# srinidhiPY/SSL_CR_Histo

Hardware: AMD Instinct MI355X
Metric: images/sec (ResNet18 SSL_CR step, 256x256 bf16 synthetic patches; whole job) (higher is better)
Workload: dtype bf16

## Files before the change

### include/sslcr.h

```cpp
#ifndef SSLCR_H_
#define SSLCR_H_
#include <stddef.h>
#include <stdint.h>

#ifdef __cplusplus
extern "C" {
#endif
#if defined(__GNUC__) || defined(__clang__)
#pragma GCC visibility push(default)
#endif

#define SSLCR_F32 0
#define SSLCR_BF16 1
#define SSLCR_FP8 2

int sslcr_version(void);
const char* sslcr_last_error(void);

typedef struct sslcr_conv_desc {
  const void* x;
  const void* w;
  void* y;
  const float* in_scale;
  const float* in_shift;
  const float* bias;
  const void* residual;
  float* stats;
  int N, H, W, C, K, R, S, stride, pad;
  int PH, PW;
  int OH, OW, osh;
  int transposed;
  int in_relu, relu, accumulate;
  int pix_mul, pix_off_h, pix_off_w;
  unsigned tap_mask;
  const void* mask_x; const float* mask_scale; const float* mask_shift; const float* mask_mean;
  int par4;
  int seg_images, seg_stride;
  const float* out_scale;
} sslcr_conv_desc;
int sslcr_conv2d(int dtype, const sslcr_conv_desc* d, void* stream);
int sslcr_conv2d_partial_rows(const sslcr_conv_desc* d);
int sslcr_conv2d_segments_ok(int dtype, const sslcr_conv_desc* d);
const char* sslcr_conv2d_kernel_name(int dtype, const sslcr_conv_desc* d);
int sslcr_conv2d_s2_pair(int dtype, const sslcr_conv_desc* c1, const sslcr_conv_desc* ds, void* stream);
int sslcr_conv2d_s2_pair_ok(int dtype, const sslcr_conv_desc* c1, const sslcr_conv_desc* ds);

typedef struct sslcr_fp8_desc {
  const uint8_t* w8;
  const float* w_dequant;
  float x_scale;
  const float* x_scale_dev;
  float* amax_out;
} sslcr_fp8_desc;
int sslcr_conv2d_fp8(const sslcr_conv_desc* d, const sslcr_fp8_desc* q, void* stream);
int sslcr_conv2d_fp8_partial_rows(const sslcr_conv_desc* d);
typedef struct sslcr_pack_fp8_desc {
  const float* w;
  uint8_t* w8;
  float* w_dequant;
  const float* gamma; const float* beta; const float* rmean; const float* rvar; float eps; float* bias_out;
  int K, C;
} sslcr_pack_fp8_desc;
int sslcr_pack_conv_fp8(const sslcr_pack_fp8_desc* d, void* stream);

typedef struct sslcr_wgrad_desc {
  const void* x;
  const void* dy;
  float* dw;
  const float* in_scale;
  const float* in_shift;
  int in_relu;
  int N, H, W, C, K, R, S, stride, pad, OH, OW;
  int seg_images;
  int seg_stride;
} sslcr_wgrad_desc;
int sslcr_conv2d_wgrad(int dtype, const sslcr_wgrad_desc* d, void* stream);
const char* sslcr_conv2d_wgrad_kernel_name(int dtype, const sslcr_wgrad_desc* d);

int sslcr_probe_tr16(const uint16_t* in, const int* byte_addr, uint16_t* out, void* stream);

typedef struct sslcr_stem_desc {
  const void* x;
  const void* w;
  void* y;
  const float* bias;
  float* stats;
  int N, H, W, OH, OW, in_f32, relu;
  const void* x2;
  int n_split;
  const float* out_scale;
} sslcr_stem_desc;
int sslcr_stem_conv(int dtype, const sslcr_stem_desc* d, void* stream);
int sslcr_stem_partial_rows(const sslcr_stem_desc* d);
int sslcr_stem_conv_pool(int dtype, const sslcr_stem_desc* d, int POH, int POW, void* stream);
typedef struct sslcr_stem_wgrad_desc {
  const void* x; const void* dy;
  float* dw;
  int N, H, W, OH, OW, in_f32;
  const void* x2; int n_split;
} sslcr_stem_wgrad_desc;
int sslcr_stem_wgrad(int dtype, const sslcr_stem_wgrad_desc* d, void* stream);

typedef struct sslcr_bn_finalize_desc {
  const float* partials;
  int rows, C;
  double count;
  const float* gamma; const float* beta;
  float* scale; float* shift; float* mean; float* invstd;
  float* running_mean; float* running_var; int64_t* num_batches_tracked;
  float momentum, eps; int replay;
  double* sums_out;
  const double* sums_in;
  double* stage;
  int nseg, seg_stride;
  int* tickets;
} sslcr_bn_finalize_desc;
int sslcr_bn_finalize(const sslcr_bn_finalize_desc* d, void* stream);

typedef struct sslcr_bn_act_desc {
  const void* x; const float* scale; const float* shift;
  const void* res; const float* rscale; const float* rshift;
  void* y; size_t pixels; int C; int relu;
  int nseg, seg_stride;
  uint8_t* ybits;
} sslcr_bn_act_desc;
int sslcr_bn_act(int dtype, const sslcr_bn_act_desc* d, void* stream);

typedef struct sslcr_pool_fwd_desc {
  const void* x; const float* scale; const float* shift; void* y; uint8_t* argmax; int N, H, W, C, OH, OW;
} sslcr_pool_fwd_desc;
int sslcr_bn_relu_maxpool(int dtype, const sslcr_pool_fwd_desc* d, void* stream);
typedef struct sslcr_pool_bwd_desc {
  const void* dy; const uint8_t* argmax; const void* x; const float* scale; const float* shift; void* dx; int N, H, W, C, OH, OW;
} sslcr_pool_bwd_desc;
int sslcr_maxpool_relu_bwd(int dtype, const sslcr_pool_bwd_desc* d, void* stream);

int sslcr_avgpool_fwd(int dtype, const void* x, float* y, int N, int HW, int C, void* stream);
int sslcr_avgpool_bwd(int dtype, const float* dy, void* dx, int N, int HW, int C, void* stream);

typedef struct sslcr_bn_bwd_desc {
  const void* dy; const void* x; const void* yact;
  const float* scale; const float* shift; const float* mean; const float* invstd;
  double* sums;
  void* dx; void* gout;
  size_t pixels; int C; int relu_from_x; double count;
  const void* pool_dy;
  const uint8_t* pool_argmax;
  int pH, pW, pOH, pOW;
  const void* pool_y;
  int g_in_reduce;
  float* dgamma; float* dbeta;
  float pg_scale;
  int nseg, seg_stride, sums_stride;
  const uint8_t* yact_bits;
} sslcr_bn_bwd_desc;
int sslcr_bn_bwd_reduce(int dtype, const sslcr_bn_bwd_desc* d, void* stream);
int sslcr_bn_bwd_apply(int dtype, const sslcr_bn_bwd_desc* d, void* stream);
int sslcr_bn_param_grads(const double* sums, const float* invstd, float* dgamma, float* dbeta, int C, void* stream);
int sslcr_stem_wgrad_pool(int dtype, const sslcr_stem_wgrad_desc* w, const sslcr_bn_bwd_desc* bn, void* stream);

int sslcr_linear_fwd(const float* x, const float* w, const float* b, float* y, int M, int N, int K, int relu, void* stream);
int sslcr_linear_bwd(const float* x, const float* w, const float* dy, const float* yact, float* dx, float* dw, float* db,
                     int M, int N, int K, int dx_accumulate, float* scratch, void* stream);
typedef struct sslcr_loss_desc {
  int kind;
  const float* logits; const float* logits_t;
  const float* target_f; const int64_t* target_i;
  float* dlogits;
  float* out;
  int nx, nu, C; float lambda_u;
  float inv_nx_global, inv_nu_global;
} sslcr_loss_desc;
int sslcr_loss(const sslcr_loss_desc* d, void* stream);
int sslcr_softmax_col(const float* logits, float* out, int n, int C, int col, void* stream);

typedef struct sslcr_tensor_desc {
  float* p; float* g; float* s1; float* s2;
  int n;
  int K, C, RS;
  void* w_fwd;
  void* w_dgrad;
  int pack_dtype;
  int dgrad_flip;
} sslcr_tensor_desc;
typedef struct sslcr_opt_desc {
  int kind;
  float lr, beta1, beta2, eps, wd, momentum;
  float bc1, bc2;
  int first_step;
  float grad_scale;
} sslcr_opt_desc;
int sslcr_optimizer_step(const sslcr_tensor_desc* device_descs, int ntensors, int max_n, const sslcr_opt_desc* o, void* stream);
int sslcr_axpby(float* p, float* q, size_t n, float alpha, int copy_back, void* stream);
int sslcr_fill(float* p, size_t n, float v, void* stream);

typedef struct sslcr_pack_desc {
  const float* w; void* w_fwd; void* w_dgrad;
  const float* gamma; const float* beta; const float* rmean; const float* rvar; float eps; float* bias_out;
  int K, C, R, S;
  int dgrad_flip;
  float* scale_out;
} sslcr_pack_desc;
int sslcr_pack_conv(int dtype, const sslcr_pack_desc* d, void* stream);
int sslcr_pack_stem(int dtype, const sslcr_pack_desc* d, void* stream);

typedef struct sslcr_weak_aug_desc {
  const uint8_t* src;
  uint8_t* dst;
  const int32_t* params;
  int N, SH, SW, OH, OW, src_hwc;
} sslcr_weak_aug_desc;
int sslcr_weak_augment(const sslcr_weak_aug_desc* d, void* stream);

typedef struct sslcr_colour_aug_desc {
  const uint8_t* src;
  uint8_t* dst;
  const double* shift;
  const uint8_t* apply;
  double hed_from_rgb[9];
  double rgb_from_hed[9];
  int N, H, W, hwc;
// ... 96 lines not shown
```

### ssl_cr_histo_amd/_lib.py

```python
import ctypes as C
import os

import torch

HERE = os.path.dirname(os.path.abspath(__file__))
LIB_PATH = os.path.join(HERE, "libsslcr.so")

vp, i32, f32, f64, sz = C.c_void_p, C.c_int, C.c_float, C.c_double, C.c_size_t


class SslcrError(RuntimeError):
    pass


def _S(name, fields):
    return type(name, (C.Structure,), {"_fields_": fields})


ConvDesc = _S("ConvDesc", [("x", vp), ("w", vp), ("y", vp), ("in_scale", vp), ("in_shift", vp), ("bias", vp),
                           ("residual", vp), ("stats", vp)] +
              [(k, i32) for k in ("N", "H", "W", "C", "K", "R", "S", "stride", "pad", "PH", "PW", "OH", "OW", "osh",
                                  "transposed", "in_relu", "relu", "accumulate", "pix_mul", "pix_off_h", "pix_off_w")] +
              [("tap_mask", C.c_uint), ("mask_x", vp), ("mask_scale", vp), ("mask_shift", vp), ("mask_mean", vp),
               ("par4", i32), ("seg_images", i32), ("seg_stride", i32), ("out_scale", vp)])
WgradDesc = _S("WgradDesc", [("x", vp), ("dy", vp), ("dw", vp), ("in_scale", vp), ("in_shift", vp), ("in_relu", i32)] +
               [(k, i32) for k in ("N", "H", "W", "C", "K", "R", "S", "stride", "pad", "OH", "OW", "seg_images", "seg_stride")])
StemDesc = _S("StemDesc", [("x", vp), ("w", vp), ("y", vp), ("bias", vp), ("stats", vp)] +
              [(k, i32) for k in ("N", "H", "W", "OH", "OW", "in_f32", "relu")] + [("x2", vp), ("n_split", i32), ("out_scale", vp)])
StemWgradDesc = _S("StemWgradDesc", [("x", vp), ("dy", vp), ("dw", vp)] +
                   [(k, i32) for k in ("N", "H", "W", "OH", "OW", "in_f32")] + [("x2", vp), ("n_split", i32)])
BnFinalizeDesc = _S("BnFinalizeDesc", [("partials", vp), ("rows", i32), ("C", i32), ("count", f64), ("gamma", vp),
                                       ("beta", vp), ("scale", vp), ("shift", vp), ("mean", vp), ("invstd", vp),
                                       ("running_mean", vp), ("running_var", vp), ("num_batches_tracked", vp),
                                       ("momentum", f32), ("eps", f32), ("replay", i32), ("sums_out", vp),
                                       ("sums_in", vp), ("stage", vp), ("nseg", i32), ("seg_stride", i32), ("tickets", vp)])
BnActDesc = _S("BnActDesc", [("x", vp), ("scale", vp), ("shift", vp), ("res", vp), ("rscale", vp), ("rshift", vp),
                             ("y", vp), ("pixels", sz), ("C", i32), ("relu", i32), ("nseg", i32), ("seg_stride", i32), ("ybits", vp)])
PoolFwdDesc = _S("PoolFwdDesc", [("x", vp), ("scale", vp), ("shift", vp), ("y", vp), ("argmax", vp)] +
                 [(k, i32) for k in ("N", "H", "W", "C", "OH", "OW")])
PoolBwdDesc = _S("PoolBwdDesc", [("dy", vp), ("argmax", vp), ("x", vp), ("scale", vp), ("shift", vp), ("dx", vp)] +
                 [(k, i32) for k in ("N", "H", "W", "C", "OH", "OW")])
BnBwdDesc = _S("BnBwdDesc", [("dy", vp), ("x", vp), ("yact", vp), ("scale", vp), ("shift", vp), ("mean", vp),
                             ("invstd", vp), ("sums", vp), ("dx", vp), ("gout", vp), ("pixels", sz), ("C", i32),
                             ("relu_from_x", i32), ("count", f64), ("pool_dy", vp), ("pool_argmax", vp), ("pH", i32),
                             ("pW", i32), ("pOH", i32), ("pOW", i32), ("pool_y", vp), ("g_in_reduce", i32), ("dgamma", vp), ("dbeta", vp),
                             ("pg_scale", f32), ("nseg", i32), ("seg_stride", i32), ("sums_stride", i32), ("yact_bits", vp)])
LossDesc = _S("LossDesc", [("kind", i32), ("logits", vp), ("logits_t", vp), ("target_f", vp), ("target_i", vp),
                           ("dlogits", vp), ("out", vp), ("nx", i32), ("nu", i32), ("C", i32), ("lambda_u", f32),
                           ("inv_nx_global", f32), ("inv_nu_global", f32)])
TensorDesc = _S("TensorDesc", [("p", vp), ("g", vp), ("s1", vp), ("s2", vp), ("n", i32), ("K", i32), ("C", i32),
                               ("RS", i32), ("w_fwd", vp), ("w_dgrad", vp), ("pack_dtype", i32), ("dgrad_flip", i32)])
OptDesc = _S("OptDesc", [("kind", i32), ("lr", f32), ("beta1", f32), ("beta2", f32), ("eps", f32), ("wd", f32),
                         ("momentum", f32), ("bc1", f32), ("bc2", f32), ("first_step", i32), ("grad_scale", f32)])
WeakAugDesc = _S("WeakAugDesc", [("src", vp), ("dst", vp), ("params", vp)] +
                 [(k, i32) for k in ("N", "SH", "SW", "OH", "OW", "src_hwc")])
ColourAugDesc = _S("ColourAugDesc", [("src", vp), ("dst", vp), ("shift", vp), ("apply", vp), ("hed_from_rgb", f64 * 9),
                                     ("rgb_from_hed", f64 * 9), ("N", i32), ("H", i32), ("W", i32), ("hwc", i32)])
BrightnessContrastDesc = _S("BrightnessContrastDesc", [("src", vp), ("dst", vp), ("alpha_beta", vp), ("apply", vp), ("stats", vp),
                                                       ("N", i32), ("H", i32), ("W", i32)])
PackDesc = _S("PackDesc", [("w", vp), ("w_fwd", vp), ("w_dgrad", vp), ("gamma", vp), ("beta", vp), ("rmean", vp),
                           ("rvar", vp), ("eps", f32), ("bias_out", vp)] + [(k, i32) for k in ("K", "C", "R", "S", "dgrad_flip")] + [("scale_out", vp)])

Fp8Desc = _S("Fp8Desc", [("w8", vp), ("w_dequant", vp), ("x_scale", f32), ("x_scale_dev", vp), ("amax_out", vp)])
PackFp8Desc = _S("PackFp8Desc", [("w", vp), ("w8", vp), ("w_dequant", vp), ("gamma", vp), ("beta", vp), ("rmean", vp), ("rvar", vp),
                                 ("eps", f32), ("bias_out", vp), ("K", i32), ("C", i32)])

P = C.POINTER
SIGNATURES = {
    "sslcr_version": (i32, []),
    "sslcr_last_error": (C.c_char_p, []),
    "sslcr_conv2d": (i32, [i32, P(ConvDesc), vp]),
    "sslcr_conv2d_partial_rows": (i32, [P(ConvDesc)]),
    "sslcr_conv2d_segments_ok": (i32, [i32, P(ConvDesc)]),
    "sslcr_conv2d_kernel_name": (C.c_char_p, [i32, P(ConvDesc)]),
    "sslcr_conv2d_s2_pair": (i32, [i32, P(ConvDesc), P(ConvDesc), vp]),
    "sslcr_conv2d_s2_pair_ok": (i32, [i32, P(ConvDesc), P(ConvDesc)]),
    "sslcr_conv2d_fp8": (i32, [P(ConvDesc), P(Fp8Desc), vp]),
    "sslcr_conv2d_fp8_partial_rows": (i32, [P(ConvDesc)]),
    "sslcr_pack_conv_fp8": (i32, [P(PackFp8Desc), vp]),
    "sslcr_conv2d_wgrad": (i32, [i32, P(WgradDesc), vp]),
    "sslcr_conv2d_wgrad_kernel_name": (C.c_char_p, [i32, P(WgradDesc)]),
    "sslcr_probe_tr16": (i32, [vp, vp, vp, vp]),
    "sslcr_stem_conv": (i32, [i32, P(StemDesc), vp]),
    "sslcr_stem_partial_rows": (i32, [P(StemDesc)]),
    "sslcr_stem_conv_pool": (i32, [i32, P(StemDesc), i32, i32, vp]),
    "sslcr_stem_wgrad": (i32, [i32, P(StemWgradDesc), vp]),
    "sslcr_stem_wgrad_pool": (i32, [i32, P(StemWgradDesc), P(BnBwdDesc), vp]),
    "sslcr_bn_finalize": (i32, [P(BnFinalizeDesc), vp]),
    "sslcr_bn_act": (i32, [i32, P(BnActDesc), vp]),
    "sslcr_bn_relu_maxpool": (i32, [i32, P(PoolFwdDesc), vp]),
    "sslcr_maxpool_relu_bwd": (i32, [i32, P(PoolBwdDesc), vp]),
    "sslcr_avgpool_fwd": (i32, [i32, vp, vp, i32, i32, i32, vp]),
    "sslcr_avgpool_bwd": (i32, [i32, vp, vp, i32, i32, i32, vp]),
    "sslcr_bn_bwd_reduce": (i32, [i32, P(BnBwdDesc), vp]),
    "sslcr_bn_bwd_apply": (i32, [i32, P(BnBwdDesc), vp]),
    "sslcr_bn_param_grads": (i32, [vp, vp, vp, vp, i32, vp]),
    "sslcr_linear_fwd": (i32, [vp, vp, vp, vp, i32, i32, i32, i32, vp]),
    "sslcr_linear_bwd": (i32, [vp, vp, vp, vp, vp, vp, vp, i32, i32, i32, i32, vp, vp]),
    "sslcr_loss": (i32, [P(LossDesc), vp]),
    "sslcr_softmax_col": (i32, [vp, vp, i32, i32, i32, vp]),
    "sslcr_optimizer_step": (i32, [vp, i32, i32, P(OptDesc), vp]),
    "sslcr_axpby": (i32, [vp, vp, sz, f32, i32, vp]),
    "sslcr_fill": (i32, [vp, sz, f32, vp]),
    "sslcr_pack_conv": (i32, [i32, P(PackDesc), vp]),
    "sslcr_pack_stem": (i32, [i32, P(PackDesc), vp]),
    "sslcr_weak_augment": (i32, [P(WeakAugDesc), vp]),
    "sslcr_hed_colour_augment": (i32, [P(ColourAugDesc), vp]),
    "sslcr_brightness_contrast": (i32, [P(BrightnessContrastDesc), vp]),
}

_lib = None


def lib():
    global _lib
    if _lib is None:
        if not os.path.exists(LIB_PATH):
            raise SslcrError(f"{LIB_PATH} not built: run `python -m ssl_cr_histo_amd.build` "
                             "(or __graft_entry__.build()); there is no CPU/PyTorch fallback")
        L = C.CDLL(LIB_PATH, mode=C.RTLD_GLOBAL)
        for name, (res, args) in SIGNATURES.items():
            fn = getattr(L, name)
            fn.restype = res
            fn.argtypes = args
        _lib = L
    return _lib


def check(rc):
    if rc != 0:
        raise SslcrError(lib().sslcr_last_error().decode())


def stream_ptr():
    return C.c_void_p(torch.cuda.current_stream().cuda_stream)


def ptr(t):
    return None if t is None else C.c_void_p(t.data_ptr())
```

### ssl_cr_histo_amd/csrc/bn_eltwise.hip

```cpp
#include <stdlib.h>

#include "kernels.hpp"

namespace sslcr {

__global__ __launch_bounds__(256) void bn_reduce_rows_kernel(const float* __restrict__ part, int rows, int C, double* __restrict__ out, int splits) {
  __shared__ double sm[2][8][32];
  const int c = blockIdx.x * 32 + (threadIdx.x & 31);
  const int rl = threadIdx.x >> 5;
  const int per = (rows + splits - 1) / splits;
  const int r0 = blockIdx.y * per, r1 = min(rows, r0 + per);
  part += (size_t)blockIdx.z * rows * 2 * C;
  out += (size_t)blockIdx.z * splits * 2 * C;
  double s = 0.0, ss = 0.0;
  if (c < C) {
    int r = r0 + rl;
    for (; r + 8 < r1; r += 16) {
      const float* p = part + (size_t)r * 2 * C;
      const float* q = p + (size_t)16 * C;
      const float a0 = p[c], a1 = p[C + c], b0 = q[c], b1 = q[C + c];
      s += (double)a0 + (double)b0;
      ss += (double)a1 + (double)b1;
    }
    for (; r < r1; r += 8) {
// ... 436 lines not shown
    float acc[EPC];
#pragma unroll
    for (int e = 0; e < EPC; ++e) acc[e] = 0.f;
    const int oh0 = h >> 1, ow0 = w >> 1;
#pragma unroll
    for (int dh = 0; dh < 2; ++dh) {
      const int oh = oh0 + dh;
      const int wi_h = h - (2 * oh - 1);
      if (oh >= a.OH || wi_h < 0 || wi_h > 2 || (dh == 1 && ((h & 1) == 0))) continue;
#pragma unroll
      for (int dw = 0; dw < 2; ++dw) {
        const int ow = ow0 + dw;
        const int wi_w = w - (2 * ow - 1);
        if (ow >= a.OW || wi_w < 0 || wi_w > 2 || (dw == 1 && ((w & 1) == 0))) continue;
        const int code = wi_h * 3 + wi_w;
        const size_t o = (((size_t)n * a.OH + oh) * a.OW + ow) * cols + col;
        float g[EPC];
        Elem<T>::unpack(ld16(dy + o * 16), g);
        uint32_t am[2];
        if (EPC == 8) { const u32x2_t v = *reinterpret_cast<const u32x2_t*>(a.argmax + o * EPC); am[0] = v[0]; am[1] = v[1]; }
        else { am[0] = *reinterpret_cast<const uint32_t*>(a.argmax + o * EPC); am[1] = 0; }
#pragma unroll
        for (int e = 0; e < EPC; ++e)
          if (((am[e >> 2] >> (8 * (e & 3))) & 0xffu) == (uint32_t)code) acc[e] += g[e];
      }
    }
    float f[EPC];
    Elem<T>::unpack(ld16_nt(x + i * 16), f);
#pragma unroll
    for (int e = 0; e < EPC; ++e)
      if (!(fmaf(f[e], a.scale[cb + e], a.shift[cb + e]) > 0.f)) acc[e] = 0.f;
    st16_nt(dx + i * 16, Elem<T>::pack(acc));
  }
}

hipError_t launch_maxpool_relu_bwd(int dtype, const PoolBwdArgs& a, hipStream_t st) {
  size_t px = (size_t)a.N * a.H * a.W;
  if (dtype == DT_BF16) {
    hipLaunchKernelGGL(maxpool_relu_bwd_kernel<bf16_t>, dim3(ew_grid(px * (a.C / 8))), dim3(256), 0, st, a);
  } else {
    hipLaunchKernelGGL(maxpool_relu_bwd_kernel<float>, dim3(ew_grid(px * (a.C / 4))), dim3(256), 0, st, a);
  }
  return hipGetLastError();
}

template <typename T>
__global__ __launch_bounds__(256) void avgpool_fwd_kernel(const void* xv, float* y, int N, int HW, int C) {
  constexpr int EPC = Elem<T>::EPC;
  __shared__ float sm[3][64][EPC + 1];
  const int cols = C / EPC;
  const int cl = threadIdx.x & 63, q = threadIdx.x >> 6;
  const int i = blockIdx.x * 64 + cl;
  const bool ok = i < N * cols;
  const int n = ok ? i / cols : 0, col = ok ? i - n * cols : 0;
  const char* x = reinterpret_cast<const char*>(xv) + ((size_t)n * HW * C) * sizeof(T) + (size_t)col * 16;
  float acc[EPC];
#pragma unroll
  for (int e = 0; e < EPC; ++e) acc[e] = 0.f;
  if (ok) {
#pragma unroll 4
    for (int p = q; p < HW; p += 4) {
      float f[EPC];
      Elem<T>::unpack(ld16(x + (size_t)p * C * sizeof(T)), f);
#pragma unroll
      for (int e = 0; e < EPC; ++e) acc[e] += f[e];
    }
  }
  if (q > 0) {
#pragma unroll
    for (int e = 0; e < EPC; ++e) sm[q - 1][cl][e] = acc[e];
  }
  __syncthreads();
  if (q > 0 || !ok) return;
#pragma unroll
  for (int w = 0; w < 3; ++w)
#pragma unroll
    for (int e = 0; e < EPC; ++e) acc[e] += sm[w][cl][e];
  const float inv = 1.f / (float)HW;
#pragma unroll
  for (int e = 0; e < EPC; ++e) y[(size_t)n * C + col * EPC + e] = acc[e] * inv;
}

template <typename T>
__global__ __launch_bounds__(256) void avgpool_bwd_kernel(const float* dy, void* dxv, int N, int HW, int C) {
  constexpr int EPC = Elem<T>::EPC;
  const int cols = C / EPC;
  const size_t total = (size_t)N * HW * cols;
  char* dx = reinterpret_cast<char*>(dxv);
  const float inv = 1.f / (float)HW;
  for (size_t i = (size_t)blockIdx.x * 256 + threadIdx.x; i < total; i += (size_t)gridDim.x * 256) {
    const int col = (int)(i % cols);
    const int n = (int)(i / ((size_t)HW * cols));
    float f[EPC];
#pragma unroll
    for (int e = 0; e < EPC; ++e) f[e] = dy[(size_t)n * C + col * EPC + e] * inv;
    st16_nt(dx + i * 16, Elem<T>::pack(f));
  }
}

hipError_t launch_avgpool_fwd(int dtype, const void* x, float* y, int N, int HW, int C, hipStream_t st) {
  if (dtype == DT_BF16) {
    hipLaunchKernelGGL(avgpool_fwd_kernel<bf16_t>, dim3(cdiv(N * (C / 8), 64)), dim3(256), 0, st, x, y, N, HW, C);
  } else {
    hipLaunchKernelGGL(avgpool_fwd_kernel<float>, dim3(cdiv(N * (C / 4), 64)), dim3(256), 0, st, x, y, N, HW, C);
  }
  return hipGetLastError();
}
hipError_t launch_avgpool_bwd(int dtype, const float* dy, void* dx, int N, int HW, int C, hipStream_t st) {
  if (dtype == DT_BF16) {
    hipLaunchKernelGGL(avgpool_bwd_kernel<bf16_t>, dim3(ew_grid((size_t)N * HW * (C / 8))), dim3(256), 0, st, dy, dx, N, HW, C);
  } else {
    hipLaunchKernelGGL(avgpool_bwd_kernel<float>, dim3(ew_grid((size_t)N * HW * (C / 4))), dim3(256), 0, st, dy, dx, N, HW, C);
  }
  return hipGetLastError();
}

template <typename T>
__device__ __forceinline__ void bn_bwd_g(const BnBwdArgs& a, size_t i, const float* rsc, const float* rsh, float* g, float* xf) {
  constexpr int EPC = Elem<T>::EPC;
  Elem<T>::unpack(ld16_nt(reinterpret_cast<const char*>(a.x) + i * 16), xf);
  if (a.pool_dy) {
    const int cols = a.C / EPC, col = (int)(i % cols);
    size_t pix = i / cols;
    const int w = (int)(pix % a.pW);
    pix /= a.pW;
    const int h = (int)(pix % a.pH), n = (int)(pix / a.pH);
#pragma unroll
    for (int e = 0; e < EPC; ++e) g[e] = 0.f;
    u32x4_t dv[4];
    uint32_t am[4][2];
    bool ok[4];
    int code[4];
#pragma unroll
    for (int k = 0; k < 4; ++k) {
      const int dh = k >> 1, dw = k & 1;
      const int oh = (h >> 1) + dh, ow = (w >> 1) + dw;
      ok[k] = (dh == 0 || (h & 1)) && (dw == 0 || (w & 1)) && oh < a.pOH && ow < a.pOW;
      code[k] = (h - (2 * oh - 1)) * 3 + (w - (2 * ow - 1));
      const int ohc = oh < a.pOH ? oh : a.pOH - 1, owc = ow < a.pOW ? ow : a.pOW - 1;
      const size_t o = (((size_t)n * a.pOH + ohc) * a.pOW + owc) * cols + col;
      dv[k] = ld16(reinterpret_cast<const char*>(a.pool_dy) + o * 16);
      if (EPC == 8) { const u32x2_t v = *reinterpret_cast<const u32x2_t*>(a.pool_argmax + o * EPC); am[k][0] = v[0]; am[k][1] = v[1]; }
      else { am[k][0] = *reinterpret_cast<const uint32_t*>(a.pool_argmax + o * EPC); am[k][1] = 0; }
    }
#pragma unroll
    for (int k = 0; k < 4; ++k) {
      float d[EPC];
      Elem<T>::unpack(dv[k], d);
#pragma unroll
      for (int e = 0; e < EPC; ++e)
        if (ok[k] && ((am[k][e >> 2] >> (8 * (e & 3))) & 0xffu) == (uint32_t)code[k]) g[e] += d[e];
    }
  } else {
    Elem<T>::unpack(ld16_nt(reinterpret_cast<const char*>(a.dy) + i * 16), g);
  }
  if (EPC == 8 && a.yact_bits) {
    const unsigned b = a.yact_bits[i];
#pragma unroll
    for (int e = 0; e < EPC; ++e)
      if (!((b >> e) & 1u)) g[e] = 0.f;
  } else if (a.yact) {
    float ya[EPC];
    Elem<T>::unpack(ld16_nt(reinterpret_cast<const char*>(a.yact) + i * 16), ya);
#pragma unroll
    for (int e = 0; e < EPC; ++e)
      if (!(ya[e] > 0.f)) g[e] = 0.f;
  } else if (a.relu_from_x) {
#pragma unroll
    for (int e = 0; e < EPC; ++e)
      if (!(fmaf(xf[e], rsc[e], rsh[e]) > 0.f)) g[e] = 0.f;
  }
}

__device__ __forceinline__ void bn_bwd_param_grads(const BnBwdArgs& a) {
  if (blockIdx.x != 0 || blockIdx.y != 0 || !a.dgamma || !a.dbeta) return;
  const int nseg = a.nseg > 1 ? a.nseg : 1;
  for (int c = threadIdx.x; c < a.C; c += 256) {
    float dg = a.dgamma[c], db = a.dbeta[c];
    for (int z = 0; z < nseg; ++z) {
      const double* sums = a.sums + (size_t)z * a.sums_stride;
      dg += (float)(sums[a.C + c] * (double)a.invstd[(size_t)z * a.seg_stride + c] * (double)a.pg_scale);
      db += (float)(sums[c] * (double)a.pg_scale);
    }
    a.dgamma[c] = dg;
    a.dbeta[c] = db;
  }
}
template <typename T>
__device__ __forceinline__ BnBwdArgs bn_bwd_segment(const BnBwdArgs& a) {
  BnBwdArgs b = a;
  if (a.nseg > 1) {
    const int z = blockIdx.y;
    b.pixels = a.pixels / a.nseg;
    const size_t off = (size_t)z * b.pixels * a.C * sizeof(T);
    if (a.dy) b.dy = reinterpret_cast<const char*>(a.dy) + off;
// ... 463 lines not shown
```

### ssl_cr_histo_amd/csrc/capi.cpp

```cpp
#include <stdarg.h>
#include <stdio.h>
#include <string.h>

#include "kernels.hpp"

namespace sslcr {
thread_local char g_err[512] = "";
int fail(const char* fmt, ...) {
  va_list ap;
  va_start(ap, fmt);
  vsnprintf(g_err, sizeof(g_err), fmt, ap);
  va_end(ap);
  return -1;
}
int check(hipError_t e, const char* what) {
  if (e == hipSuccess) return 0;
  return fail("%s: %s", what, hipGetErrorString(e));
}
}

using namespace sslcr;

#define NEED(cond, what) \
  do {                   \
    if (!(cond)) return fail("%s: invalid argument (%s)", __func__, what); \
  } while (0)
#define DT_OK(dt) NEED((dt) == SSLCR_F32 || (dt) == SSLCR_BF16, "dtype")

extern "C" {

int sslcr_version(void) { return 6; }
const char* sslcr_last_error(void) { return g_err; }

int sslcr_conv2d(int dtype, const sslcr_conv_desc* d, void* stream) {
  DT_OK(dtype);
  NEED(d && d->x && d->w && d->y, "null tensor");
  NEED(d->N > 0 && d->C > 0 && d->K > 0 && d->R > 0 && d->S > 0 && d->stride > 0, "shape");
  NEED(d->C % (dtype == SSLCR_BF16 ? 64 : 32) == 0, "C must be a multiple of the 128-byte channel slab");
  NEED(d->K % 64 == 0, "K % 64");
  NEED(d->osh >= 1 && d->PH > 0 && d->PW > 0, "pixel space");
  NEED(conv_segments_ok(dtype, *d), "seg_images: no segment form for this shape / dtype (sslcr_conv2d_segments_ok)");
  return check(launch_conv(dtype, *d, (hipStream_t)stream), "conv2d");
}
int sslcr_conv2d_partial_rows(const sslcr_conv_desc* d) { return d ? conv_partials_rows(*d) : -1; }
int sslcr_conv2d_segments_ok(int dtype, const sslcr_conv_desc* d) { return (d && (dtype == DT_F32 || dtype == DT_BF16) && conv_segments_ok(dtype, *d)) ? 1 : 0; }
const char* sslcr_conv2d_kernel_name(int dtype, const sslcr_conv_desc* d) { return d ? conv_kernel_name(dtype, *d) : ""; }
int sslcr_conv2d_s2_pair_ok(int dtype, const sslcr_conv_desc* c1, const sslcr_conv_desc* ds) {
  return (c1 && ds && conv_s2_pair_ok(dtype, *c1, *ds)) ? 1 : 0;
}
int sslcr_conv2d_s2_pair(int dtype, const sslcr_conv_desc* c1, const sslcr_conv_desc* ds, void* stream) {
  DT_OK(dtype);
  NEED(c1 && ds && c1->x && c1->w && c1->y && ds->w && ds->y, "null tensor");
  NEED(conv_s2_pair_ok(dtype, *c1, *ds), "pair not served (sslcr_conv2d_s2_pair_ok)");
  return check(launch_conv_s2(*c1, ds, (hipStream_t)stream), "conv2d_s2_pair");
}

int sslcr_conv2d_fp8(const sslcr_conv_desc* d, const sslcr_fp8_desc* q, void* stream) {
  NEED(d && q && d->x && d->y && q->w8 && q->w_dequant, "null tensor");
  NEED(q->x_scale > 0.f, "x_scale must be positive");
  NEED(conv_fp8_mode(*d) != 0, "shape not served by the fp8 kernel (3x3/1, C % 128, K % 128, 16x16-tileable or 8x8 with N % 4)");
  return check(launch_conv_fp8(*d, *q, (hipStream_t)stream), "conv2d_fp8");
}
int sslcr_conv2d_fp8_partial_rows(const sslcr_conv_desc* d) { return (d && conv_fp8_mode(*d)) ? conv_fp8_rows(*d) : 0; }
int sslcr_pack_conv_fp8(const sslcr_pack_fp8_desc* d, void* stream) {
  NEED(d && d->w && d->w8 && d->w_dequant && d->K > 0 && d->C > 0, "args");
  NEED(!d->gamma || (d->beta && d->rmean && d->rvar), "BatchNorm fold needs gamma, beta, running mean and var");
  return check(launch_pack_fp8(*d, (hipStream_t)stream), "pack_conv_fp8");
}

const char* sslcr_conv2d_wgrad_kernel_name(int dtype, const sslcr_wgrad_desc* d) { return d ? wgrad_kernel_name(dtype, *d) : ""; }
int sslcr_conv2d_wgrad(int dtype, const sslcr_wgrad_desc* d, void* stream) {
  DT_OK(dtype);
  NEED(d && d->x && d->dy && d->dw, "null tensor");
  NEED(d->C % 64 == 0 && d->K % 64 == 0, "C,K % 64");
  NEED((d->R == 3 && d->S == 3) || (d->R == 1 && d->S == 1), "3x3 or 1x1");
  return check(launch_wgrad(dtype, *d, (hipStream_t)stream), "conv2d_wgrad");
}

int sslcr_probe_tr16(const uint16_t* in, const int* byte_addr, uint16_t* out, void* stream) {
  NEED(in && byte_addr && out, "null");
  return check(launch_probe_tr16(in, byte_addr, out, (hipStream_t)stream), "probe_tr16");
}

int sslcr_stem_conv(int dtype, const sslcr_stem_desc* d, void* stream) {
  DT_OK(dtype);
  NEED(d && d->x && d->w && d->y, "null tensor");
  NEED(d->OH == (d->H + 6 - 7) / 2 + 1 && d->OW == (d->W + 6 - 7) / 2 + 1, "7x7/2 pad 3 output dims");
  NEED(!d->x2 || (d->n_split >= 0 && d->n_split <= d->N), "n_split outside the batch");
  return check(launch_stem(dtype, *d, (hipStream_t)stream), "stem_conv");
}
int sslcr_stem_conv_pool(int dtype, const sslcr_stem_desc* d, int POH, int POW, void* stream) {
  DT_OK(dtype);
  NEED(d && d->x && d->w && d->y, "null");
  NEED(stem_pool_ok(dtype, *d, POH, POW), "shape / mode not served by the fused stem + max-pool kernel");
  return check(launch_stem_pool(dtype, *d, POH, POW, (hipStream_t)stream), "stem_conv_pool");
}
int sslcr_stem_partial_rows(const sslcr_stem_desc* d) { return d ? stem_partials_rows(*d) : -1; }
int sslcr_stem_wgrad(int dtype, const sslcr_stem_wgrad_desc* d, void* stream) {
  DT_OK(dtype);
  NEED(d && d->x && d->dy && d->dw, "null tensor");
  NEED(!d->x2 || (d->n_split >= 0 && d->n_split <= d->N), "n_split outside the batch");
  return check(launch_stem_wgrad(dtype, *d, (hipStream_t)stream), "stem_wgrad");
}
int sslcr_stem_wgrad_pool(int dtype, const sslcr_stem_wgrad_desc* w, const sslcr_bn_bwd_desc* bn, void* stream) {
  DT_OK(dtype);
  NEED(w && w->x && w->dw && bn && bn->pool_dy && bn->pool_argmax && bn->x && bn->sums && bn->mean && bn->invstd && bn->scale && bn->shift, "null tensor");
  NEED(!w->x2 || (w->n_split >= 0 && w->n_split <= w->N), "n_split outside the batch");
  NEED(bn->C == 64 && bn->pH == w->OH && bn->pW == w->OW && bn->pixels == (size_t)w->N * w->OH * w->OW, "bn descriptor is not this stem's");
  NEED(!bn->g_in_reduce && !bn->gout, "pool form has no g output");
  return check(launch_stem_wgrad_pool(dtype, *w, *bn, (hipStream_t)stream), "stem_wgrad_pool");
}

int sslcr_bn_finalize(const sslcr_bn_finalize_desc* d, void* stream) {
  NEED(d && d->C > 0, "desc");
  NEED(d->sums_in || (d->partials && d->stage && d->rows > 0), "partials/stage");
  NEED(d->sums_out || (d->gamma && d->beta && d->scale && d->shift && d->count > 0), "finalize outputs");
  return check(launch_bn_finalize(*d, (hipStream_t)stream), "bn_finalize");
}
int sslcr_bn_act(int dtype, const sslcr_bn_act_desc* d, void* stream) {
  DT_OK(dtype);
  NEED(d && d->x && d->y && d->scale && d->shift, "null");
  NEED(d->C % 8 == 0, "C % 8");
  return check(launch_bn_act(dtype, *d, (hipStream_t)stream), "bn_act");
}
int sslcr_bn_relu_maxpool(int dtype, const sslcr_pool_fwd_desc* d, void* stream) {
  DT_OK(dtype);
  NEED(d && d->x && d->y, "null");
  if (!d->scale || !d->shift) {
    const int cols = d->C / (dtype == SSLCR_BF16 ? 8 : 4);
    NEED(!d->scale && !d->shift && !d->argmax, "plain max-pool (scale = shift = NULL) records no argmax");
    NEED(cols >= 1 && cols <= 256 && 256 % cols == 0 && d->C % (dtype == SSLCR_BF16 ? 8 : 4) == 0, "plain max-pool: unsupported channel count");
  }
  return check(launch_bn_relu_maxpool(dtype, *d, (hipStream_t)stream), "bn_relu_maxpool");
}
int sslcr_maxpool_relu_bwd(int dtype, const sslcr_pool_bwd_desc* d, void* stream) {
  DT_OK(dtype);
  NEED(d && d->x && d->dy && d->dx && d->argmax, "null");
  return check(launch_maxpool_relu_bwd(dtype, *d, (hipStream_t)stream), "maxpool_relu_bwd");
}
int sslcr_avgpool_fwd(int dtype, const void* x, float* y, int N, int HW, int C, void* stream) {
  DT_OK(dtype);
  NEED(x && y && N > 0 && HW > 0 && C % 8 == 0, "args");
  return check(launch_avgpool_fwd(dtype, x, y, N, HW, C, (hipStream_t)stream), "avgpool_fwd");
}
int sslcr_avgpool_bwd(int dtype, const float* dy, void* dx, int N, int HW, int C, void* stream) {
  DT_OK(dtype);
  NEED(dy && dx && N > 0 && HW > 0 && C % 8 == 0, "args");
  return check(launch_avgpool_bwd(dtype, dy, dx, N, HW, C, (hipStream_t)stream), "avgpool_bwd");
}
int sslcr_bn_bwd_reduce(int dtype, const sslcr_bn_bwd_desc* d, void* stream) {
  DT_OK(dtype);
  NEED(d && (d->dy || (d->pool_dy && d->pool_argmax)) && d->x && d->sums && d->mean, "null");
  NEED(!d->g_in_reduce || (d->yact && d->gout && d->dy && !d->pool_dy), "g_in_reduce needs dy, yact and gout");
  return check(launch_bn_bwd_reduce(dtype, *d, (hipStream_t)stream), "bn_bwd_reduce");
}
int sslcr_bn_bwd_apply(int dtype, const sslcr_bn_bwd_desc* d, void* stream) {
  DT_OK(dtype);
  NEED(d && (d->dy || (d->pool_dy && d->pool_argmax)) && d->x && d->sums && d->dx && d->mean && d->invstd && d->scale, "null");
  NEED(!d->g_in_reduce || (d->yact && d->gout && d->dy && !d->pool_dy), "g_in_reduce needs dy, yact and gout");
  return check(launch_bn_bwd_apply(dtype, *d, (hipStream_t)stream), "bn_bwd_apply");
}
int sslcr_bn_param_grads(const double* sums, const float* invstd, float* dgamma, float* dbeta, int C, void* stream) {
  NEED(sums && invstd && dgamma && dbeta, "null");
  return check(launch_bn_param_grads(sums, invstd, dgamma, dbeta, C, (hipStream_t)stream), "bn_param_grads");
}

int sslcr_linear_fwd(const float* x, const float* w, const float* b, float* y, int M, int N, int K, int relu, void* stream) {
  NEED(x && w && y && M > 0 && N > 0 && K > 0, "args");
  return check(launch_linear_fwd(x, w, b, y, M, N, K, relu, (hipStream_t)stream), "linear_fwd");
}
int sslcr_linear_bwd(const float* x, const float* w, const float* dy, const float* yact, float* dx, float* dw, float* db,
                     int M, int N, int K, int dx_accumulate, float* scratch, void* stream) {
  NEED(x && w && dy && scratch && M > 0 && N > 0 && K > 0, "args");
  return check(launch_linear_bwd(x, w, dy, yact, dx, dw, db, M, N, K, dx_accumulate, scratch, (hipStream_t)stream), "linear_bwd");
}
int sslcr_loss(const sslcr_loss_desc* d, void* stream) {
  NEED(d && d->logits && d->out && d->nx > 0 && d->C > 0 && d->C <= 64, "args");
  return check(launch_loss(*d, (hipStream_t)stream), "loss");
}

int sslcr_softmax_col(const float* logits, float* out, int n, int C, int col, void* stream) {
  NEED(logits && out && n > 0 && C > 0 && C <= 64 && col >= 0 && col < C, "args");
  return check(launch_softmax_col(logits, out, n, C, col, (hipStream_t)stream), "softmax_col");
}

int sslcr_optimizer_step(const sslcr_tensor_desc* device_descs, int ntensors, int max_n, const sslcr_opt_desc* o, void* stream) {
  NEED(device_descs && o && ntensors > 0 && max_n > 0, "args");
  return check(launch_optimizer(device_descs, ntensors, max_n, *o, (hipStream_t)stream), "optimizer_step");
}
int sslcr_axpby(float* p, float* q, size_t n, float alpha, int copy_back, void* stream) {
  NEED(p && q, "null");
  return check(launch_axpby(p, q, n, alpha, copy_back, (hipStream_t)stream), "axpby");
}
int sslcr_fill(float* p, size_t n, float v, void* stream) {
  NEED(p, "null");
  return check(launch_fill(p, n, v, (hipStream_t)stream), "fill");
}
int sslcr_pack_conv(int dtype, const sslcr_pack_desc* d, void* stream) {
  DT_OK(dtype);
  NEED(d && d->w && (d->w_fwd || d->w_dgrad), "null");
  return check(launch_pack_conv(dtype, *d, (hipStream_t)stream), "pack_conv");
}
int sslcr_weak_augment(const sslcr_weak_aug_desc* d, void* stream) {
  NEED(d && d->src && d->dst && d->params, "null");
  NEED(d->N > 0 && d->OH > 0 && d->OW > 0 && d->OH <= d->SH && d->OW <= d->SW, "crop larger than the source");
  return check(launch_weak_augment(*d, (hipStream_t)stream), "weak_augment");
}
int sslcr_hed_colour_augment(const sslcr_colour_aug_desc* d, void* stream) {
  NEED(d && d->src && d->dst && d->shift, "null");
  NEED(d->N > 0 && d->H > 0 && d->W > 0, "empty batch");
  return check(launch_hed_colour(*d, (hipStream_t)stream), "hed_colour_augment");
}
int sslcr_brightness_contrast(const sslcr_brightness_contrast_desc* d, void* stream) {
  NEED(d && d->src && d->dst && d->alpha_beta && d->stats, "null");
  NEED(d->N > 0 && d->H > 0 && d->W > 0, "empty batch");
  return check(launch_brightness_contrast(*d, (hipStream_t)stream), "brightness_contrast");
}
int sslcr_pack_stem(int dtype, const sslcr_pack_desc* d, void* stream) {
  DT_OK(dtype);
  NEED(d && d->w && d->w_fwd && d->K == 64 && d->C == 3 && d->R == 7 && d->S == 7, "stem shape");
  return check(launch_pack_stem(dtype, *d, (hipStream_t)stream), "pack_stem");
}

}
```

### ssl_cr_histo_amd/csrc/conv_h16.hip

```cpp
#include "kernels.hpp"

namespace sslcr {

template <typename T> struct MmaH;
template <> struct MmaH<bf16_t> {
  __device__ static __forceinline__ void run(const u32x4_t& a, const u32x4_t& b, f32x4_t& c) {
    c = __builtin_amdgcn_mfma_f32_16x16x32_bf16(__builtin_bit_cast(bf16x8_t, a), __builtin_bit_cast(bf16x8_t, b), c, 0, 0, 0);
  }
};
template <> struct MmaH<float> {
  __device__ static __forceinline__ void run(const u32x4_t& a, const u32x4_t& b, f32x4_t& c) {
#pragma unroll
    for (int e = 0; e < 4; ++e)
      c = __builtin_amdgcn_mfma_f32_16x16x4f32(__uint_as_float(a[e]), __uint_as_float(b[e]), c, 0, 0, 0);
  }
};

template <int TK>
__device__ __forceinline__ int wperm_inv(int rr) {
  constexpr int B = 16 * TK;
  const int blk = rr / B, x = rr - blk * B;
  const int t = x >> 4, q = (x >> 2) & 3, j = x & 3;
  return blk * B + q * (4 * TK) + t * 4 + j;
}

#define SSLCR_WAIT_VM0() __builtin_amdgcn_s_waitcnt(0x0f70)
#define SSLCR_BARE_BARRIER() asm volatile("s_barrier" ::: "memory")

#ifdef SSLCR_H16_PROF
__device__ unsigned long long g_h16_prof[16][8];
#define H16_T(v) const unsigned long long v = __builtin_readcyclecounter()
#define H16_ACC(i, d) h16_t[i] += (d)
#else
#define H16_T(v)
#define H16_ACC(i, d)
#endif

template <typename T, int BKO, int WK, bool XF, bool WR, bool RAW = false, int TW = 16>
__global__ __launch_bounds__(256 * WK, WK == 1 ? 1 : 2) void conv3x3_h16_kernel(const ConvArgs a, const int tiles_total, const int n_items, const int kshift,
                                                                                const int row0) {
  constexpr bool OSC = false;
#include "conv_h16_body.hpp"
}
template <typename T, int BKO, int WK, bool WR, int TW>
__global__ __launch_bounds__(256 * WK, WK == 1 ? 1 : 2) void conv3x3_h16s_kernel(const ConvArgs a, const int tiles_total, const int n_items, const int kshift,
                                                                                 const int row0) {
  constexpr bool OSC = true, XF = false, RAW = false;
#include "conv_h16_body.hpp"
}

static int h16_mode(int dtype, const ConvArgs& a) {
  const int q = conv_halo256_mode(dtype, a);
  if (q == 16 && conv_halo256_mode(DT_BF16, a) == 16) return 16;
  static const bool on8 = [] { const char* e = getenv("SSLCR_H16_TW8"); return !e || atoi(e) != 0; }();
  if (q == 8 && on8 && conv_halo256_mode(DT_BF16, a) == 8 && a.K % 128 == 0 && !a.mask_x && (a.seg_images <= 0 || a.seg_images % 4 == 0)) return 8;
  return 0;
}
bool conv_h16_ok(int dtype, const ConvArgs& a) {
  if (a.in_scale && a.residual) return false;
  if (a.mask_x) {
    if (!a.mask_scale || !a.mask_shift || !a.mask_mean || a.in_scale || a.bias || a.residual || a.relu || a.out_scale) return false;
    if (18 * 24 * 128 + 2 * 3 * (a.K % 128 == 0 ? 128 : 64) * 128 + 2 * a.C * 4 + 8 * 128 * 4 + 3 * a.K * 4 > 160 * 1024) return false;
  }
  if (a.out_scale) {
    if (a.in_scale || a.stats || !a.bias) return false;
    const int mode = h16_mode(dtype, a);
    if (mode == 0) return false;
    const int bko = a.K % 128 == 0 ? 128 : 64;
    if (!(a.C == 64 && a.K == 64) &&
        (mode == 16 ? 18 * 24 : 4 * 10 * 10) * 128 + 2 * 3 * bko * 128 + 2 * a.C * 4 + 8 * bko * 4 + 2 * a.K * 4 > 160 * 1024) return false;
  }
  return h16_mode(dtype, a) != 0;
}
static int h16_tiles(const ConvArgs& a, int nseg) {
  return a.H == 8 ? (a.N / nseg) / 4 : (a.N / nseg) * (a.H / 16) * (a.W / 16);
}
static int h16_grid(const ConvArgs& a, int bko) {
  const int nseg = a.seg_images > 0 ? a.N / a.seg_images : 1;
  const int n_items = h16_tiles(a, nseg) * (a.K / bko);
  const int per = device_cus() / nseg;
  return (n_items < per ? n_items : per) * nseg;
}
static int h16_tail8(const ConvArgs& a) {
  if (a.H != 8 || a.seg_images > 0) return 0;
  const int cus = device_cus(), tiles = a.N / 4, kb = a.K / 128, rem = (tiles * kb) % cus;
  if (rem == 0 || 2 * rem > cus || rem % kb != 0 || tiles <= rem / kb) return 0;
  return rem / kb;
}
static ConvArgs h16_head8(const ConvArgs& a, int tail) { ConvArgs h = a; h.N = a.N - 4 * tail; return h; }
static ConvArgs h16_tailargs8(const ConvArgs& a, int tail, int dtype) {
  ConvArgs t = a;
  const int n0 = a.N - 4 * tail;
  const size_t es = dtype == DT_BF16 ? 2 : 4, px = (size_t)n0 * a.H * a.W;
  t.N = 4 * tail;
  t.x = reinterpret_cast<const char*>(a.x) + px * a.C * es;
  t.y = reinterpret_cast<char*>(a.y) + px * a.K * es;
  if (a.residual) t.residual = reinterpret_cast<const char*>(a.residual) + px * a.K * es;
  return t;
}
int conv_h16_rows(const ConvArgs& a) {
  if (a.seg_images > 0 && conv_pp64_ok(DT_BF16, a)) return conv_pp64_rows(a);
  const int tail = h16_tail8(a);
  if (tail) return (h16_grid(h16_head8(a, tail), 128) + h16_grid(h16_tailargs8(a, tail, DT_BF16), 64)) * 4;
  return h16_grid(a, a.K % 128 == 0 ? 128 : 64) * 4;
}

static bool h16_resident(const ConvArgs& a) { return a.C == 64 && a.K == 64; }
static bool h16_raw(const ConvArgs& a) {
  static const bool on = [] { const char* e = getenv("SSLCR_H16_RAW"); return !e || atoi(e) != 0; }();
  return on && a.stats && !a.bias && !a.relu && !a.residual && !a.mask_x;
}

template <typename T, int BKO, int WK, bool XF, bool WR = false, bool RAW = false, int TW = 16, bool OSC = false>
static hipError_t launch_h(const ConvArgs& a, hipStream_t st, int row0 = 0) {
  const size_t lds = (TW == 16 ? 18 * 24 : 4 * 10 * 10) * 128 + (WR ? 3 : 2) * 3 * BKO * 128 + 2 * a.C * sizeof(float) + 8 * BKO * sizeof(float) +
                     (a.mask_x ? 3 : (a.out_scale ? 2 : 1)) * a.K * sizeof(float);
  if (lds > 160 * 1024) return hipErrorInvalidValue;
  static_assert(!OSC || (!XF && !RAW), "output scale: eval forms only");
  void (*kern)(const ConvArgs, const int, const int, const int, const int);
  if constexpr (OSC) kern = conv3x3_h16s_kernel<T, BKO, WK, WR, TW>;
  else kern = conv3x3_h16_kernel<T, BKO, WK, XF, WR, RAW, TW>;
  if (OSC != (a.out_scale != nullptr)) return hipErrorInvalidValue;
  static std::atomic<bool> attr_done{false};
  if (!attr_done) {
    hipError_t e = hipFuncSetAttribute(reinterpret_cast<const void*>(kern), hipFuncAttributeMaxDynamicSharedMemorySize, 160 * 1024);
    if (e != hipSuccess) return e;
    attr_done = true;
  }
  const int nseg = a.seg_images > 0 ? a.N / a.seg_images : 1;
  const int tiles = h16_tiles(a, nseg);
  const int n_items = tiles * (a.K / BKO);
  const int grid = h16_grid(a, BKO);
  const int kbn = a.K / BKO, gseg = grid / nseg;
  const int kshift = (kbn > 1 && (kbn & (kbn - 1)) == 0 && (gseg & (kbn - 1)) == 0) ? __builtin_ctz(kbn) : -1;
  hipLaunchKernelGGL(kern, dim3(grid), dim3(256 * WK), lds, st, a, tiles, n_items, kshift, row0);
  return hipGetLastError();
}

template <typename T>
static hipError_t launch_ht8(const ConvArgs& a, hipStream_t st) {
  const bool xf = a.in_scale != nullptr;
  auto wide = [&](const ConvArgs& q) {
    if (q.out_scale) return launch_h<T, 128, 2, false, false, false, 8, true>(q, st);
    if constexpr (sizeof(T) == 2)
      if (h16_raw(q)) return xf ? launch_h<T, 128, 2, true, false, true, 8>(q, st) : launch_h<T, 128, 2, false, false, true, 8>(q, st);
    return xf ? launch_h<T, 128, 2, true, false, false, 8>(q, st) : launch_h<T, 128, 2, false, false, false, 8>(q, st);
  };
  const int tail = h16_tail8(a);
  if (!tail) return wide(a);
  const ConvArgs head = h16_head8(a, tail), tl = h16_tailargs8(a, tail, Elem<T>::DT);
  hipError_t e = wide(head);
  if (e != hipSuccess) return e;
  const int row0 = h16_grid(head, 128) * 4;
  if (tl.out_scale) return launch_h<T, 64, 2, false, false, false, 8, true>(tl, st, row0);
  return xf ? launch_h<T, 64, 2, true, false, false, 8>(tl, st, row0) : launch_h<T, 64, 2, false, false, false, 8>(tl, st, row0);
}

template <typename T>
static hipError_t launch_ht(const ConvArgs& a, hipStream_t st) {
  const bool xf = a.in_scale != nullptr;
  if (h16_mode(Elem<T>::DT, a) == 8) return launch_ht8<T>(a, st);
  if (a.K % 128 == 0) {
    if (a.out_scale) return launch_h<T, 128, 2, false, false, false, 16, true>(a, st);
    if constexpr (sizeof(T) == 2)
      if (h16_raw(a)) return xf ? launch_h<T, 128, 2, true, false, true>(a, st) : launch_h<T, 128, 2, false, false, true>(a, st);
    return xf ? launch_h<T, 128, 2, true>(a, st) : launch_h<T, 128, 2, false>(a, st);
  }
  if constexpr (sizeof(T) == 2)
    if (h16_resident(a)) {
      if (conv_pp64_ok(DT_BF16, a)) return launch_conv_pp64(a, st);
      if (a.out_scale) return launch_h<T, 64, 2, false, true, false, 16, true>(a, st);
      return xf ? launch_h<T, 64, 2, true, true>(a, st) : launch_h<T, 64, 2, false, true>(a, st);
    }
  if (a.out_scale) return launch_h<T, 64, 2, false, false, false, 16, true>(a, st);
  return xf ? launch_h<T, 64, 2, true>(a, st) : launch_h<T, 64, 2, false>(a, st);
}

hipError_t launch_conv_h16(int dtype, const ConvArgs& a, hipStream_t st) {
  if (a.mask_x && !a.stats) return hipErrorInvalidValue;
  return dtype == DT_BF16 ? launch_ht<bf16_t>(a, st) : launch_ht<float>(a, st);
}

const char* conv_h16_name(int dtype, const ConvArgs& a) {
  const bool bf = dtype == DT_BF16, xf = a.in_scale != nullptr;
  if (a.out_scale) {
    if (h16_mode(dtype, a) == 8) return bf ? "sslcr::conv3x3_h16s_kernel<unsigned short, 128, 2, false, 8>" : "sslcr::conv3x3_h16s_kernel<float, 128, 2, false, 8>";
    if (a.K % 128 == 0) return bf ? "sslcr::conv3x3_h16s_kernel<unsigned short, 128, 2, false, 16>" : "sslcr::conv3x3_h16s_kernel<float, 128, 2, false, 16>";
    if (bf && h16_resident(a) && conv_pp64_ok(DT_BF16, a)) return conv_pp64_name(a);
    if (bf && h16_resident(a)) return "sslcr::conv3x3_h16s_kernel<unsigned short, 64, 2, true, 16>";
    return bf ? "sslcr::conv3x3_h16s_kernel<unsigned short, 64, 2, false, 16>" : "sslcr::conv3x3_h16s_kernel<float, 64, 2, false, 16>";
  }
  if (h16_mode(dtype, a) == 8) {
    if (!bf) return xf ? "sslcr::conv3x3_h16_kernel<float, 128, 2, true, false, false, 8>" : "sslcr::conv3x3_h16_kernel<float, 128, 2, false, false, false, 8>";
    if (h16_raw(a))
      return xf ? "sslcr::conv3x3_h16_kernel<unsigned short, 128, 2, true, false, true, 8>" : "sslcr::conv3x3_h16_kernel<unsigned short, 128, 2, false, false, true, 8>";
    return xf ? "sslcr::conv3x3_h16_kernel<unsigned short, 128, 2, true, false, false, 8>" : "sslcr::conv3x3_h16_kernel<unsigned short, 128, 2, false, false, false, 8>";
  }
  if (a.K % 128 == 0) {
    if (bf && h16_raw(a))
      return xf ? "sslcr::conv3x3_h16_kernel<unsigned short, 128, 2, true, false, true, 16>" : "sslcr::conv3x3_h16_kernel<unsigned short, 128, 2, false, false, true, 16>";
    if (bf) return xf ? "sslcr::conv3x3_h16_kernel<unsigned short, 128, 2, true, false, false, 16>" : "sslcr::conv3x3_h16_kernel<unsigned short, 128, 2, false, false, false, 16>";
    return xf ? "sslcr::conv3x3_h16_kernel<float, 128, 2, true, false, false, 16>" : "sslcr::conv3x3_h16_kernel<float, 128, 2, false, false, false, 16>";
  }
  if (bf && h16_resident(a) && conv_pp64_ok(DT_BF16, a)) return conv_pp64_name(a);
  if (bf && h16_resident(a))
    return xf ? "sslcr::conv3x3_h16_kernel<unsigned short, 64, 2, true, true, false, 16>" : "sslcr::conv3x3_h16_kernel<unsigned short, 64, 2, false, true, false, 16>";
  if (bf) return xf ? "sslcr::conv3x3_h16_kernel<unsigned short, 64, 2, true, false, false, 16>" : "sslcr::conv3x3_h16_kernel<unsigned short, 64, 2, false, false, false, 16>";
  return xf ? "sslcr::conv3x3_h16_kernel<float, 64, 2, true, false, false, 16>" : "sslcr::conv3x3_h16_kernel<float, 64, 2, false, false, false, 16>";
}

}
```

### ssl_cr_histo_amd/csrc/conv_h16_body.hpp

```cpp
  constexpr int NT = 256 * WK;
  constexpr int EPC = Elem<T>::EPC;
  constexpr int CE = 8 * EPC;
  static_assert(TW == 16 || (TW == 8 && !WR), "tile forms");
  constexpr int TH = TW, NI = 256 / (TW * TH), HH = TH + 2, HWD = TW + 2, PITCH = TW == 16 ? 24 : 10;
  constexpr int HP = TW == 16 ? HH * HWD : 256;
  constexpr int NLD = (HP * 8 + NT - 1) / NT;
  constexpr int TK = BKO / (16 * WK), TP = 4;
  constexpr int HBUF = NI * HH * PITCH * 128, WBUF = BKO * 128, TPB = 3;
  static_assert(NLD <= 16, "staging shape");
  extern __shared__ __attribute__((aligned(16))) char smem[];
  char* s_halo = smem;
  constexpr int NRING = WR ? 3 : 2;
  char* s_w = smem + HBUF;
  float* s_scale = reinterpret_cast<float*>(smem + HBUF + NRING * TPB * WBUF);
  float* s_shift = s_scale + a.C;
  float* s_stat = s_shift + a.C;

  const int tid = threadIdx.x, lane = tid & 63;
  const int wave = __builtin_amdgcn_readfirstlane(tid >> 6);
  const int g = lane >> 4, li = lane & 15;
  const int wp = wave & 3, wk = wave >> 2;
  const int tiles_w = TW == 16 ? a.W / TW : 1, tiles_h = TW == 16 ? a.H / TH : 1;
  const int nseg = a.seg_images > 0 ? a.N / a.seg_images : 1;
  const int G = gridDim.x / nseg;
  const int seg = nseg > 1 ? (int)blockIdx.x / G : 0, lb = (int)blockIdx.x - seg * G;
  const int seg_n0 = seg * a.seg_images;
  if (XF) {
    const float* isc = a.in_scale + (size_t)seg * a.seg_stride;
    const float* ish = a.in_shift + (size_t)seg * a.seg_stride;
    for (int c = tid; c < a.C; c += NT) { s_scale[c] = isc[c]; s_shift[c] = ish[c]; }
  }
  for (int i = tid; i < 8 * BKO; i += NT) s_stat[i] = 0.f;
  float* s_bias = s_stat + 8 * BKO;
  const bool mk = !OSC && !XF && !RAW && a.mask_x != nullptr;
  float* s_msh = s_bias + a.K;
  float* s_mmu = s_msh + a.K;
  float* s_osc = s_msh;
  for (int i = tid; i < a.K; i += NT) {
    const size_t mo = (size_t)seg * a.seg_stride + i;
    s_bias[i] = mk ? a.mask_scale[mo] : (a.bias ? a.bias[i] : 0.f);
    if (mk) { s_msh[i] = a.mask_shift[mo]; s_mmu[i] = a.mask_mean[mo]; }
    if constexpr (OSC) s_osc[i] = a.out_scale[i];
  }
  const float relu_lo = a.in_relu ? 0.f : -__builtin_inff();
  const float out_lo = a.relu ? 0.f : -__builtin_inff();

  const int first = (G & 7) ? lb : (lb & 7) * (G >> 3) + (lb >> 3);
  if (first >= n_items) return;

  const int chunk = tid & 7;
  int rel[NLD], st_off[NLD];
  unsigned long long edge = 0;
  unsigned hvalid = 0;
#pragma unroll
  for (int i = 0; i < NLD; ++i) {
    const int sp = (tid >> 3) + (NT / 8) * i;
    rel[i] = 0; st_off[i] = 0;
    if (TW == 8) {
      rel[i] = sp;
      const int hc = (sp & 7) + 1;
      const int hp = ((sp >> 6) * HH + ((sp >> 3) & 7) + 1) * PITCH + hc;
      st_off[i] = hp * 128 + ((chunk ^ (hc & 7)) << 4);
      hvalid |= 1u << i;
    } else if (sp < HP) {
      const int hr = sp / HWD, hc = sp - hr * HWD;
      rel[i] = (hr - 1) * a.W + hc - 1;
      const int hp = hr * PITCH + hc;
      st_off[i] = hp * 128 + ((chunk ^ (hp & 7)) << 4);
      hvalid |= 1u << i;
      edge |= (unsigned long long)((hr == 0) | ((hr == HH - 1) << 1) | ((hc == 0) << 2) | ((hc == HWD - 1) << 3)) << (4 * i);
    }
  }
  const bool loader = WK == 1 || wave >= 4;
  constexpr int WLI = BKO / 32;
  const int lw = wave & 3;
  constexpr int WROWS = BKO / WLI;
  int wsrc0;
  {
    const int rr = lw * 8 + (lane >> 3);
    const int krow = wperm_inv<TK>(rr);
    const int c16 = (lane & 7) ^ (rr & 7);
    wsrc0 = (int)(((size_t)krow * 9 * a.C + c16 * EPC) * sizeof(T));
  }
  int Bb[3][2], Ab[2];
#pragma unroll
  for (int kk = 0; kk < 2; ++kk) {
    const int ci = kk * 4 + g;
#pragma unroll
    for (int s = 0; s < 3; ++s)
      Bb[s][kk] = TW == 16 ? ((wp * 4) * PITCH + li + s) * 128 + ((ci ^ ((li + s) & 7)) << 4)
                           : ((wp * HH + (li >> 3)) * PITCH + (li & 7) + s) * 128 + ((ci ^ (((li & 7) + s) & 7)) << 4);
    Ab[kk] = (wk * (BKO / WK) + li) * 128 + ((ci ^ (li & 7)) << 4);
  }
  const char* xg = reinterpret_cast<const char*>(a.x) + (size_t)chunk * EPC * sizeof(T);
  const char* wg = reinterpret_cast<const char*>(a.w);
  const int nslabs = a.C / CE;

  const bool kfast = kshift >= 0;
  struct Geo { int origin, k0, tile, n0, h0, w0; unsigned long long out; };
  auto geom = [&](int item) {
    Geo q;
    const int kbi = kfast ? item & ((1 << kshift) - 1) : item / tiles_total;
    q.tile = kfast ? item >> kshift : item - kbi * tiles_total;
    q.k0 = kbi * BKO;
    int t = q.tile;
    const int tw_i = t % tiles_w; t /= tiles_w;
    const int th_i = t % tiles_h;
    q.n0 = (t / tiles_h) * NI + seg_n0;
    q.h0 = th_i * TH; q.w0 = tw_i * TW;
    q.origin = (q.n0 * a.H + q.h0) * a.W + q.w0;
    q.out = TW == 8 ? 0ull : (unsigned long long)((q.h0 == 0) | ((q.h0 + TH >= a.H) << 1) | ((q.w0 == 0) << 2) | ((q.w0 + TW >= a.W) << 3)) *
                             0x1111111111111111ull;
    return q;
  };

  u32x4_t hreg[NLD];
  unsigned hin = 0;
  auto load_halo = [&](const Geo& q, int slab) {
    const unsigned long long bad = edge & q.out;
    hin = 0;
// ... 2 lines not shown
      const bool ok = ((hvalid >> i) & 1u) && !((bad >> (4 * i)) & 0xfull);
      const int idx = q.origin + (ok ? rel[i] : 0);
      hreg[i] = ld16_nt(xg + ((size_t)idx * a.C + slab * CE) * sizeof(T));
      hin |= (ok ? 1u : 0u) << i;
    }
  };
  float sc[EPC], sh[EPC];
  auto load_affine = [&](int slab) {
    if (XF) {
      const int cb = slab * CE + chunk * EPC;
#pragma unroll
      for (int e = 0; e < EPC; ++e) { sc[e] = s_scale[cb + e]; sh[e] = s_shift[cb + e]; }
    }
  };
  auto xform_one = [&](int i) {
    u32x4_t v = hreg[i];
    if (XF) {
      float f[EPC];
      Elem<T>::unpack(v, f);
#pragma unroll
      for (int e = 0; e < EPC; ++e) f[e] = clamp_lo(fmaf(f[e], sc[e], sh[e]), relu_lo);
      v = PackH<T>::run(f);
    }
    const bool ok = (hin >> i) & 1u;
#pragma unroll
    for (int e = 0; e < 4; ++e) v[e] = ok ? v[e] : 0u;
    hreg[i] = v;
  };
  auto store_halo = [&]() {
#pragma unroll
    for (int i = 0; i < NLD; ++i)
      if ((hvalid >> i) & 1u) st16(s_halo + st_off[i], hreg[i]);
  };
  LdsDma wdma;
  wdma.init(wg, 0x7fffffffu);
  auto dma_w = [&](int k0, int slab, int tap0, int half) {
    if (!loader) return;
#pragma unroll
    for (int tt = 0; tt < TPB; ++tt) {
      const int soff = (int)(((size_t)k0 * 9 * a.C + (size_t)(tap0 + tt) * a.C + slab * CE) * sizeof(T));
#pragma unroll
      for (int i = 0; i < WLI; ++i) {
        char* dst = s_w + (half * TPB + tt) * WBUF + (i * WROWS + lw * 8) * 128;
        wdma.load16(dst, wsrc0, soff + wperm_inv<TK>(i * WROWS) * 9 * a.C * (int)sizeof(T));
      }
    }
  };

  f32x4_t acc[TK][TP];
#pragma unroll
  for (int t = 0; t < TK; ++t)
#pragma unroll
    for (int p = 0; p < TP; ++p) acc[t][p] = f32x4_t{0.f, 0.f, 0.f, 0.f};

  u32x4_t A[2][TK], B[2][TP];
  auto frags = [&](int buf, int step, const char* ringg) {
    const int tap = step >> 1, kk = step & 1;
    const int r = tap / 3, s = tap - 3 * r;
    A[buf][0] = ld16(ringg + Ab[kk] + s * WBUF);
#pragma unroll
    for (int p = 0; p < TP; ++p) B[buf][p] = ld16(s_halo + Bb[s][kk] + ((TW == 16 ? p : 2 * p) + r) * (PITCH * 128));
#pragma unroll
    for (int t = 1; t < TK; ++t) A[buf][t] = ld16(ringg + Ab[kk] + s * WBUF + t * 2048);
  };

  if (TW == 8) {
    for (int i = tid; i < HBUF / 16; i += NT) st16(s_halo + i * 16, u32x4_t{0u, 0u, 0u, 0u});
    __syncthreads();
  }
  Geo cur = geom(first);
  dma_w(cur.k0, 0, 0, 0);
  if constexpr (WR) { dma_w(cur.k0, 0, 3, 1); dma_w(cur.k0, 0, 6, 2); }
  load_halo(cur, 0);
  if (XF) __syncthreads();
  load_affine(0);
#pragma unroll
  for (int i = 0; i < NLD; ++i) xform_one(i);
  store_halo();
  SSLCR_WAIT_VM0();
  __syncthreads();
  frags(0, 0, s_w);

  char* yg = reinterpret_cast<char*>(a.y);
  const char* rg = (XF || RAW) ? nullptr : reinterpret_cast<const char*>(a.mask_x ? a.mask_x : a.residual);
  constexpr bool RPRE = sizeof(T) == 2 && !XF && !RAW;
  constexpr int RQ = 4 * TK / EPC;
  u32x4_t rres[RPRE ? TP : 1][RPRE ? RQ : 1];
  auto out_off = [&](const Geo& q, int p) {
    const int h = q.h0 + wp * 4 + p, w = q.w0 + li;
    const size_t pix = TW == 16 ? ((size_t)q.n0 * a.H + h) * a.W + w : (size_t)(q.n0 + wp) * 64 + p * 16 + li;
    return (pix * a.K + q.k0 + wk * (BKO / WK) + g * (4 * TK)) * sizeof(T);
  };
  int wb = 0, item = first, slab = 0;
  unsigned pub = 0;
#ifdef SSLCR_H16_PROF
  unsigned long long h16_t[8] = {0, 0, 0, 0, 0, 0, 0, 0};
  const unsigned long long h16_begin = __builtin_readcyclecounter();
#endif
  for (;;) {
    const bool last = slab + 1 == nslabs;
    const bool done = last && item + G >= n_items;
    const int nslab = last ? 0 : slab + 1;
    const Geo nxt = (last && !done) ? geom(item + G) : cur;
    const char* ring0 = s_w + wb * (TPB * WBUF);
    const char* ring1 = s_w + (wb ^ 1) * (TPB * WBUF);

    auto load_res = [&]() {
      if constexpr (RPRE) {
        if (rg && last) {
#pragma unroll
          for (int p = 0; p < TP; ++p)
#pragma unroll
            for (int q = 0; q < RQ; ++q) rres[p][q] = ld16(rg + out_off(cur, p) + q * 16);
        }
      }
    };
    if constexpr (WR) {
      load_res();
      load_halo(nxt, 0);
    } else {
      dma_w(cur.k0, slab, 3, wb ^ 1);
    }
    __builtin_amdgcn_sched_barrier(0);
#pragma unroll
    for (int i = 0; i < 18; ++i) {
      if (i < 17) frags((i + 1) & 1, i + 1, WR ? s_w + ((i + 1) / 6) * (TPB * WBUF) : ((((i + 1) / 6) & 1) ? ring1 : ring0));
      if (sizeof(T) != 2) __builtin_amdgcn_sched_barrier(0);
#pragma unroll
      for (int t = 0; t < TK; ++t)
#pragma unroll
        for (int p = 0; p < TP; ++p) MmaH<T>::run(A[i & 1][t], B[i & 1][p], acc[t][p]);
      if (i < 17 && sizeof(T) == 2) {
#pragma unroll
        for (int q = 0; q < TK + TP; ++q) {
          __builtin_amdgcn_sched_group_barrier(0x100, 1, 0);
          __builtin_amdgcn_sched_group_barrier(0x008, (TK * TP) / (TK + TP), 0);
        }
      }
      if (i >= 15) {
#pragma unroll
        for (int j = (i - 15); j < NLD; j += 3) xform_one(j);
      }
      __builtin_amdgcn_sched_barrier(0);
      if (WR && i == 14) {
        SSLCR_WAIT_VM0();
        __builtin_amdgcn_sched_barrier(0);
      }
      if (!WR && i % 6 == 2) {
        H16_T(tp0);
        SSLCR_WAIT_VM0();
        H16_T(tp1);
        SSLCR_BARE_BARRIER();
        H16_T(tp2);
        H16_ACC(0, tp1 - tp0); H16_ACC(1, tp2 - tp1);
        if (i == 8) {
          load_res();
          load_halo(nxt, nslab);
          load_affine(nslab);
        }
        __builtin_amdgcn_sched_barrier(0);
      }
      if (!WR && (i == 5 || i == 11)) {
        H16_T(tf0);
        SSLCR_BARE_BARRIER();
        H16_T(tf1);
        H16_ACC(2, tf1 - tf0);
        if (i == 5) dma_w(cur.k0, slab, 6, wb); else dma_w(nxt.k0, nslab, 0, wb ^ 1);
        __builtin_amdgcn_sched_barrier(0);
      }
    }
    H16_T(ts0);
    SSLCR_BARE_BARRIER();
    store_halo();
    __syncthreads();
    H16_T(ts1);
    H16_ACC(3, ts1 - ts0); H16_ACC(5, 1);
    wb ^= 1;
    frags(0, 0, WR ? s_w : s_w + wb * (TPB * WBUF));
    __builtin_amdgcn_sched_barrier(0);

    H16_T(te0);
    if (last) {
      const int kb = cur.k0 + wk * (BKO / WK) + g * (4 * TK);
      float s1[4 * TK], s2[4 * TK];
      if (mk) {
#pragma unroll
        for (int q = 0; q < 4 * TK / EPC; ++q) {
          float msc[EPC], msh[EPC], mmu[EPC], a1[EPC], a2[EPC];
#pragma unroll
          for (int e = 0; e < EPC; ++e) {
            msc[e] = s_bias[kb + q * EPC + e]; msh[e] = s_msh[kb + q * EPC + e]; mmu[e] = s_mmu[kb + q * EPC + e];
            a1[e] = 0.f; a2[e] = 0.f;
          }
#pragma unroll
          for (int p = 0; p < TP; ++p) {
            const size_t off = out_off(cur, p);
            float xr[EPC], vq[EPC];
            if constexpr (RPRE) Elem<T>::unpack(rres[p][q], xr);
            else Elem<T>::unpack(ld16(rg + off + q * 16), xr);
#pragma unroll
            for (int e = 0; e < EPC; ++e) {
              const int idx = q * EPC + e;
              const float y = acc[idx >> 2][p][idx & 3];
              const float gv = fmaf(xr[e], msc[e], msh[e]) > 0.f ? y : 0.f;
              vq[e] = gv;
              a1[e] += gv;
              a2[e] = fmaf(gv, xr[e] - mmu[e], a2[e]);
            }
            st16(yg + off + q * 16, PackH<T>::run(vq));
          }
#pragma unroll
          for (int e = 0; e < EPC; ++e) { s1[q * EPC + e] = a1[e]; s2[q * EPC + e] = a2[e]; }
        }
      } else {
      if constexpr (RAW) {
#pragma unroll
        for (int p = 0; p < TP; ++p) {
          const size_t off = out_off(cur, p);
#pragma unroll
          for (int q = 0; q < 4 * TK / EPC; ++q) {
            float vq[EPC];
#pragma unroll
            for (int e = 0; e < EPC; ++e) vq[e] = acc[(q * EPC + e) >> 2][p][(q * EPC + e) & 3];
            st16(yg + off + q * 16, PackH<T>::run(vq));
          }
        }
      } else if constexpr (OSC) {
#pragma unroll
      for (int q = 0; q < 4 * TK / EPC; ++q) {
        float bq[EPC], sq[EPC];
#pragma unroll
        for (int e = 0; e < EPC; ++e) { bq[e] = s_bias[kb + q * EPC + e]; sq[e] = s_osc[kb + q * EPC + e]; }
#pragma unroll
        for (int p = 0; p < TP; ++p) {
          const size_t off = out_off(cur, p);
          float vq[EPC];
#pragma unroll
          for (int e = 0; e < EPC; ++e) {
            const int idx = q * EPC + e;
            vq[e] = fmaf(acc[idx >> 2][p][idx & 3], sq[e], bq[e]);
          }
          if (rg) {
            float rr[EPC];
            if constexpr (RPRE) Elem<T>::unpack(rres[p][q], rr);
            else Elem<T>::unpack(ld16(rg + off + q * 16), rr);
#pragma unroll
            for (int e = 0; e < EPC; ++e) vq[e] += rr[e];
          }
#pragma unroll
          for (int e = 0; e < EPC; ++e) vq[e] = clamp_lo(vq[e], out_lo);
          st16(yg + off + q * 16, PackH<T>::run(vq));
        }
      }
      } else {
      float bias[4 * TK];
#pragma unroll
      for (int j = 0; j < 4 * TK; ++j) bias[j] = s_bias[kb + j];
#pragma unroll
      for (int p = 0; p < TP; ++p) {
        const size_t off = out_off(cur, p);
        float v[4 * TK];
#pragma unroll
        for (int t = 0; t < TK; ++t)
#pragma unroll
          for (int j = 0; j < 4; ++j) v[t * 4 + j] = acc[t][p][j] + bias[t * 4 + j];
#pragma unroll
        for (int q = 0; q < 4 * TK / EPC; ++q) {
          float* vq = v + q * EPC;
          if (rg) {
            float rr[EPC];
            if constexpr (RPRE) Elem<T>::unpack(rres[p][q], rr);
            else Elem<T>::unpack(ld16(rg + off + q * 16), rr);
#pragma unroll
            for (int e = 0; e < EPC; ++e) vq[e] += rr[e];
          }
#pragma unroll
          for (int e = 0; e < EPC; ++e) vq[e] = clamp_lo(vq[e], out_lo);
          st16(yg + off + q * 16, PackH<T>::run(vq));
        }
      }
      }
      if (a.stats) {
#pragma unroll
        for (int t = 0; t < TK; ++t)
#pragma unroll
          for (int j = 0; j < 4; ++j) {
            float x1 = 0.f, x2 = 0.f;
#pragma unroll
            for (int p = 0; p < TP; ++p) { float q = acc[t][p][j]; x1 += q; x2 = fmaf(q, q, x2); }
            s1[t * 4 + j] = x1;
            s2[t * 4 + j] = x2;
          }
      }
      }
      constexpr bool FOLD = (4 * TK) % 16 == 0;
      if (a.stats) {
        if constexpr (FOLD) {
#pragma unroll
          for (int f = 0; f < 4 * TK / 16; ++f) {
            row16_fold16(*reinterpret_cast<float (*)[16]>(s1 + 16 * f));
            row16_fold16(*reinterpret_cast<float (*)[16]>(s2 + 16 * f));
          }
          if ((li & 3) == 0) {
            float* sp = s_stat + (wp * 2) * BKO + wk * (BKO / WK) + g * (4 * TK) + (li >> 2) * 4;
#pragma unroll
            for (int h = 0; h < 2; ++h) {
#pragma unroll
              for (int f = 0; f < 4 * TK / 16; ++f) {
                const float* sv = (h ? s2 : s1) + 16 * f;
                f32x4_t* slot = reinterpret_cast<f32x4_t*>(sp + h * BKO + 16 * f);
                f32x4_t v = *slot;
#pragma unroll
                for (int e = 0; e < 4; ++e) v[e] += sv[e];
                *slot = v;
              }
            }
          }
        } else {
#pragma unroll
          for (int i = 0; i < 4 * TK; ++i) { s1[i] = row16_sum(s1[i]); s2[i] = row16_sum(s2[i]); }
        }
        if (!FOLD && li == 0) {
          float* sp = s_stat + (wp * 2) * BKO + wk * (BKO / WK) + g * (4 * TK);
#pragma unroll
          for (int h = 0; h < 2; ++h) {
            const float* sv = h ? s2 : s1;
#pragma unroll
            for (int c4 = 0; c4 < TK; ++c4) {
              f32x4_t* slot = reinterpret_cast<f32x4_t*>(sp + h * BKO + c4 * 4);
              f32x4_t v = *slot;
#pragma unroll
              for (int e = 0; e < 4; ++e) v[e] += sv[c4 * 4 + e];
              *slot = v;
            }
          }
        }
        if (done || nxt.k0 != cur.k0) {
          pub |= 1u << (cur.k0 / BKO);
          __syncthreads();
          for (int i = tid; i < 8 * BKO; i += NT) {
            const int rw = i / BKO, c = i - rw * BKO;
            a.stats[((size_t)(row0 + blockIdx.x * 4 + (rw >> 1)) * 2 + (rw & 1)) * a.K + cur.k0 + c] = s_stat[i];
            s_stat[i] = 0.f;
          }
          __syncthreads();
        }
      }
#ifdef SSLCR_H16_PROF
      { H16_T(te1); H16_ACC(4, te1 - te0); }
#endif
      if (done) break;
#pragma unroll
      for (int t = 0; t < TK; ++t)
#pragma unroll
        for (int p = 0; p < TP; ++p) acc[t][p] = f32x4_t{0.f, 0.f, 0.f, 0.f};
      item += G;
      cur = nxt;
    }
    slab = nslab;
  }
#ifdef SSLCR_H16_PROF
  if (blockIdx.x == 0 && lane == 0) {
    h16_t[6] = __builtin_readcyclecounter() - h16_begin;
    for (int i = 0; i < 8; ++i) g_h16_prof[wave][i] = h16_t[i];
  }
#endif
  if (a.stats) {
    for (int kbi = 0; kbi < a.K / BKO; ++kbi) {
      if ((pub >> kbi) & 1u) continue;
      for (int i = tid; i < 8 * BKO; i += NT) {
        const int rw = i / BKO, c = i - rw * BKO;
        a.stats[((size_t)(row0 + blockIdx.x * 4 + (rw >> 1)) * 2 + (rw & 1)) * a.K + kbi * BKO + c] = 0.f;
      }
    }
  }
```

### ssl_cr_histo_amd/csrc/conv_igemm.hip

```cpp
#include "kernels.hpp"

namespace sslcr {

template <typename T> struct Mma;
template <> struct Mma<bf16_t> {
  __device__ static __forceinline__ void run(const u32x4_t& a, const u32x4_t& b, f32x4_t& c) {
    c = __builtin_amdgcn_mfma_f32_16x16x32_bf16(__builtin_bit_cast(bf16x8_t, a), __builtin_bit_cast(bf16x8_t, b), c, 0, 0, 0);
  }
};
template <> struct Mma<float> {
  __device__ static __forceinline__ void run(const u32x4_t& a, const u32x4_t& b, f32x4_t& c) {
#pragma unroll
    for (int e = 0; e < 4; ++e)
      c = __builtin_amdgcn_mfma_f32_16x16x4f32(__uint_as_float(a[e]), __uint_as_float(b[e]), c, 0, 0, 0);
  }
};

template <typename T, int BP, int BKO>
__global__ __launch_bounds__(256) void conv_igemm_kernel(const ConvArgs a) {
  constexpr int EPC = Elem<T>::EPC;
  constexpr int CE = 8 * EPC;
  constexpr int TP = BP / 32;
  constexpr int TK = BKO / 32;
  constexpr int PR = BP / 32;
// ... 235 lines not shown
  if (q) return conv_halo256_tiles(a, q) * 4;
  const int tw = conv_halo_tw(g_conv_dtype_hint, a);
  if (tw) return conv_halo_tiles(a, tw) * 2;
  const int bp = conv_dma_bp(g_conv_dtype_hint, a);
  if (bp) return conv_dma_rows(a, bp);
  const int M = a.N * a.PH * a.PW;
  return cdiv(M, conv_tile_bp(a)) * 2;
}

int conv_tile_bp(const ConvArgs& a) {
  const int M = a.N * a.PH * a.PW;
  return M >= 128 * 512 ? 128 : 64;
}

template <typename T>
static hipError_t launch_t(const ConvArgs& a, hipStream_t st) {
  constexpr int CE = 8 * Elem<T>::EPC;
  if (a.C % CE != 0 || a.K % 64 != 0) return hipErrorInvalidValue;
  const int bp = conv_tile_bp(a);
  if (bp == 128) {
    if (a.K % 128 == 0) return launch_cfg<T, 128, 128>(a, st);
    return launch_cfg<T, 128, 64>(a, st);
  }
  return launch_cfg<T, 64, 64>(a, st);
}

const char* conv_kernel_name(int dtype, const ConvArgs& a) {
  const bool bf = dtype == DT_BF16;
  const bool wide = a.K % 128 == 0;
  if (conv_h16_ok(dtype, a)) return conv_h16_name(dtype, a);
  const int q = conv_halo256_mode(dtype, a);
  if (q && conv_halo256_mode(DT_BF16, a) == q) {
    const bool one = a.C == (bf ? 64 : 32);
    if (q == 16) {
      if (wide) return bf ? "sslcr::conv3x3_halo256_kernel<unsigned short, 16, 128, 2, false>" : "sslcr::conv3x3_halo256_kernel<float, 16, 128, 2, false>";
      if (one) return bf ? "sslcr::conv3x3_halo256_kernel<unsigned short, 16, 64, 1, true>" : "sslcr::conv3x3_halo256_kernel<float, 16, 64, 1, true>";
      return bf ? "sslcr::conv3x3_halo256_kernel<unsigned short, 16, 64, 2, false>" : "sslcr::conv3x3_halo256_kernel<float, 16, 64, 2, false>";
    }
    if (wide) return bf ? "sslcr::conv3x3_halo256_kernel<unsigned short, 8, 128, 2, false>" : "sslcr::conv3x3_halo256_kernel<float, 8, 128, 2, false>";
    if (one) return bf ? "sslcr::conv3x3_halo256_kernel<unsigned short, 8, 64, 1, true>" : "sslcr::conv3x3_halo256_kernel<float, 8, 64, 1, true>";
    return bf ? "sslcr::conv3x3_halo256_kernel<unsigned short, 8, 64, 2, false>" : "sslcr::conv3x3_halo256_kernel<float, 8, 64, 2, false>";
  }
  const int tw = q ? 0 : conv_halo_tw(dtype, a);
  if (tw && conv_halo_tw(DT_BF16, a) == tw) return bf ? "sslcr::conv3x3_halo_kernel<unsigned short, ...>" : "sslcr::conv3x3_halo_kernel<float, ...>";
  if (!q && !tw && conv_s2_ok(dtype, a)) return conv_s2_name(a, false);
  if (!q && !tw && conv_s2d_ok(dtype, a)) return conv_s2d_name();
  const int dbp = (q || tw) ? 0 : conv_dma_bp(dtype, a);
  if (dbp && conv_dma_bp(DT_BF16, a) == dbp) return conv_dma_name(dtype, dbp);
  const int bp = conv_tile_bp(a);
  if (bp == 128) {
    if (wide) return bf ? "sslcr::conv_igemm_kernel<unsigned short, 128, 128>" : "sslcr::conv_igemm_kernel<float, 128, 128>";
    return bf ? "sslcr::conv_igemm_kernel<unsigned short, 128, 64>" : "sslcr::conv_igemm_kernel<float, 128, 64>";
  }
  return bf ? "sslcr::conv_igemm_kernel<unsigned short, 64, 64>" : "sslcr::conv_igemm_kernel<float, 64, 64>";
}

int device_cus() {
  static const int cus = [] {
    int dev = 0, n = 0;
    if (hipGetDevice(&dev) != hipSuccess || hipDeviceGetAttribute(&n, hipDeviceAttributeMultiprocessorCount, dev) != hipSuccess || n <= 0) n = 256;
    return n;
  }();
  return cus;
}

bool conv_segments_ok(int dtype, const ConvArgs& a) {
  if (a.seg_images <= 0) return true;
  if (dtype != DT_BF16 || a.N % a.seg_images != 0 || a.transposed || a.par4) return false;
  const int nseg = a.N / a.seg_images;
  if (nseg > 8) return false;
  if (conv_h16_ok(dtype, a)) return true;
  if (a.mask_x) return false;
  const int q = conv_halo256_mode(dtype, a);
  if (q) return q == 16 || a.seg_images % 4 == 0;
  if (conv_halo_tw(dtype, a)) return false;
  const int bp = conv_dma_bp(dtype, a);
  if (bp) return !a.in_scale && ((long)a.seg_images * a.PH * a.PW) % bp == 0;
  return false;
}

hipError_t launch_conv(int dtype, const ConvArgs& a, hipStream_t st) {
  if (!conv_segments_ok(dtype, a)) return hipErrorInvalidValue;
  if (a.out_scale && (!a.bias || a.stats || a.mask_x)) return hipErrorInvalidValue;
  if (conv_h16_ok(dtype, a)) return launch_conv_h16(dtype, a, st);
  if (a.mask_x) return hipErrorInvalidValue;
  const int q = conv_halo256_mode(dtype, a);
  if (q && conv_halo256_mode(DT_BF16, a) == q) return launch_conv_halo256(dtype, a, q, st);
  const int tw = q ? 0 : conv_halo_tw(dtype, a);
  if (tw && conv_halo_tw(DT_BF16, a) == tw) return launch_conv_halo(dtype, a, tw, st);
  if (!q && !tw && conv_s2_ok(dtype, a)) return launch_conv_s2(a, nullptr, st);
  if (!q && !tw && conv_s2d_ok(dtype, a)) return launch_conv_s2d(a, st);
  const int dbp = (q || tw) ? 0 : conv_dma_bp(dtype, a);
  if (dbp && conv_dma_bp(DT_BF16, a) == dbp) return launch_conv_dma(dtype, a, dbp, st);
  if (a.par4) return hipErrorInvalidValue;
  return dtype == DT_BF16 ? launch_t<bf16_t>(a, st) : launch_t<float>(a, st);
}

}
```

### ssl_cr_histo_amd/csrc/conv_pp64.hip

```cpp
#include <stdlib.h>

#include "kernels.hpp"

namespace sslcr {

typedef const __attribute__((address_space(1))) void* gptr_pp;
typedef __attribute__((address_space(3))) void* lptr_pp;

#define SSLCR_PP_BAR() asm volatile("s_waitcnt lgkmcnt(0)\n\ts_barrier" ::: "memory")

#ifdef SSLCR_PP_PROF
__device__ unsigned long long g_pp_prof[8][8];
#define PP_T(v) const unsigned long long v = __builtin_readcyclecounter()
#define PP_ACC(i, d) pp_t[i] += (d)
#else
#define PP_T(v)
#define PP_ACC(i, d)
#endif

#define PP_CH(t, g, j) ((((t) >> 1) * 32) + ((g) * 8) + (((t) & 1) * 4) + (j))
__device__ __forceinline__ int pp_row_kout(int rr) {
  const int t = rr >> 4, gq = (rr >> 2) & 3, j = rr & 3;
  return PP_CH(t, gq, j);
}
// ... 66 lines not shown
    const int sp = (gtid >> 3) + (GT / 8) * i;
    role[i] = rel_bias;
    if (sp < HP) {
      const int hr = sp / HWD, hc = sp - hr * HWD;
      role[i] = ((hr - 1) * a.W + hc - 1 + rel_bias) | ((((hr * PITCH + hc) * 128 + ((chunk ^ (hc & 7)) << 4)) >> 4) << 16);
      hvalid |= 1u << i;
      edge |= (unsigned long long)((hr == 0) | ((hr == HH - 1) << 1) | ((hc == 0) << 2) | ((hc == HWD - 1) << 3)) << (4 * i);
    }
  }
  int Bb[3][2], Ab[2];
#pragma unroll
  for (int kk = 0; kk < 2; ++kk) {
    const int ci = kk * 4 + g;
#pragma unroll
    for (int s = 0; s < 3; ++s) Bb[s][kk] = ((wq * 4) * PITCH + li + s) * 128 + ((ci ^ ((li + s) & 7)) << 4);
    Ab[kk] = li * 128 + ((ci ^ (li & 7)) << 4);
  }
  const char* xg = reinterpret_cast<const char*>(a.x) + (size_t)chunk * EPC * sizeof(T);

  struct Geo { int origin, n0, h0, w0; unsigned long long out; };
  auto geom = [&](int tile) {
    Geo q;
    int t = tile;
    const int tw_i = t % tiles_w; t /= tiles_w;
    const int th_i = t % tiles_h;
    q.n0 = t / tiles_h + seg_n0;
    q.h0 = th_i * TH; q.w0 = tw_i * TW;
    q.origin = (q.n0 * a.H + q.h0) * a.W + q.w0;
    q.out = (unsigned long long)((q.h0 == 0) | ((q.h0 + TH >= a.H) << 1) | ((q.w0 == 0) << 2) | ((q.w0 + TW >= a.W) << 3)) *
            0x1111111111111111ull;
    return q;
  };
  auto tile_of = [&](int k, bool& live) {
    const int t = first0 + grp + k * 2 * G;
    live = t < tiles_total;
    return live ? t : tiles_total - 1;
  };

  u32x4_t hreg[NLD];
  unsigned hin = 0;
  auto load_halo = [&](const Geo& q) {
    const unsigned long long bad = edge & q.out;
    hin = 0;
#pragma unroll
    for (int i = 0; i < NLD; ++i) {
      const bool ok = ((hvalid >> i) & 1u) && !((bad >> (4 * i)) & 0xfull);
      int rl = role[i];
      asm volatile("" : "+v"(rl));
      const int idx = q.origin + (ok ? (rl & 0xffff) - rel_bias : 0);
      hreg[i] = ld16_nt(xg + (unsigned)idx * (unsigned)(64 * sizeof(T)));
      hin |= (ok ? 1u : 0u) << i;
    }
  };
  auto xform_store = [&]() {
    float sc[EPC], sh[EPC];
    if (XF) {
      const f32x4_t c0 = *reinterpret_cast<const f32x4_t*>(s_scale + chunk * EPC), c1 = *reinterpret_cast<const f32x4_t*>(s_scale + chunk * EPC + 4);
      const f32x4_t h0 = *reinterpret_cast<const f32x4_t*>(s_shift + chunk * EPC), h1 = *reinterpret_cast<const f32x4_t*>(s_shift + chunk * EPC + 4);
#pragma unroll
      for (int e = 0; e < 4; ++e) { sc[e] = c0[e]; sc[4 + e] = c1[e]; sh[e] = h0[e]; sh[4 + e] = h1[e]; }
    }
#pragma unroll
    for (int i = 0; i < NLD; ++i) {
      u32x4_t v = hreg[i];
      if (XF) {
        float f[EPC];
        Elem<T>::unpack(v, f);
#pragma unroll
        for (int e = 0; e < EPC; ++e) f[e] = __builtin_amdgcn_fmed3f(fmaf(f[e], sc[e], sh[e]), relu_lo, __builtin_inff());
        v = PackH<T>::run(f);
      }
      const bool ok = (hin >> i) & 1u;
#pragma unroll
      for (int e = 0; e < 4; ++e) v[e] = ok ? v[e] : 0u;
      int rl = role[i];
      asm volatile("" : "+v"(rl));
      if ((hvalid >> i) & 1u) st16(s_halo + ((rl >> 12) & 0xffff0), v);
    }
  };

  char* yg = reinterpret_cast<char*>(a.y);
  const char* rg = OP == 0 ? nullptr : reinterpret_cast<const char*>(OP == 2 ? a.mask_x : a.residual);
  u32x4_t rres[RPRE ? TP : 1][RPRE ? RQ : 1];
  auto out_off = [&](const Geo& q, int p) {
    const int h = q.h0 + wq * 4 + p, w = q.w0 + li;
    return (unsigned)(((q.n0 * a.H + h) * a.W + w) * 64 + g * 8) * (unsigned)sizeof(T);
  };
  auto load_res = [&](const Geo& q) {
    if constexpr (RPRE) {
#pragma unroll
      for (int p = 0; p < TP; ++p)
#pragma unroll
        for (int qq = 0; qq < RQ; ++qq) rres[p][qq] = ld16(rg + out_off(q, p) + qq * 64);
    }
  };

  f32x4_t acc[TK][TP];
  u32x4_t A[2][TK], B[2][TP];
  auto frags = [&](int buf, int step) {
    const int tap = step >> 1, kk = step & 1;
    const int r = tap / 3, s = tap - 3 * r;
#pragma unroll
    for (int t = 0; t < TK; ++t) A[buf][t] = ld16(s_w + Ab[kk] + tap * WBUF + t * 2048);
#pragma unroll
    for (int p = 0; p < TP; ++p) B[buf][p] = ld16(s_halo + Bb[s][kk] + (p + r) * (PITCH * 128));
  };

  bool live = false, live_n = false;
  Geo cur = geom(tile_of(0, live));
  load_halo(cur);
  __builtin_amdgcn_s_waitcnt(0x0f70);
  SSLCR_PP_BAR();
  xform_store();
  Geo nxt = geom(tile_of(1, live_n));
  load_halo(nxt);
  SSLCR_PP_BAR();
  if (grp == 1) SSLCR_PP_BAR();

#ifdef SSLCR_PP_PROF
  unsigned long long pp_t[8] = {0, 0, 0, 0, 0, 0, 0, 0};
#endif
  for (int st = 0; st < nst; ++st) {
    PP_T(t0);
    frags(0, 0);
    __builtin_amdgcn_sched_barrier(0);
#pragma unroll
    for (int i = 0; i < 18; ++i) {
      if (i < 17) frags((i + 1) & 1, i + 1);
#pragma unroll
      for (int t = 0; t < TK; ++t)
#pragma unroll
        for (int p = 0; p < TP; ++p) {
          const bf16x8_t av = __builtin_bit_cast(bf16x8_t, A[i & 1][t]), bv = __builtin_bit_cast(bf16x8_t, B[i & 1][p]);
          if (i == 0) acc[t][p] = __builtin_amdgcn_mfma_f32_16x16x32_bf16(av, bv, f32x4_t{0.f, 0.f, 0.f, 0.f}, 0, 0, 0);
          else acc[t][p] = __builtin_amdgcn_mfma_f32_16x16x32_bf16(av, bv, acc[t][p], 0, 0, 0);
        }
      if (i < 17) {
#pragma unroll
        for (int q = 0; q < TK + TP; ++q) {
          __builtin_amdgcn_sched_group_barrier(0x100, 1, 0);
          __builtin_amdgcn_sched_group_barrier(0x008, (TK * TP) / (TK + TP), 0);
        }
      }
      __builtin_amdgcn_sched_barrier(0);
    }
    PP_T(t1);
    SSLCR_PP_BAR();
    PP_T(t2);
    PP_ACC(0, t1 - t0); PP_ACC(1, t2 - t1);

    load_res(cur);
    xform_store();
    PP_T(ta);
    PP_ACC(4, ta - t2);
    {
      const int kb = g * 8;
      float s1[4 * TK], s2[4 * TK];
      if constexpr (mk) {
#pragma unroll
        for (int q = 0; q < RQ; ++q) {
          float msc[EPC], msh[EPC], mmu[EPC], a1[EPC], a2[EPC];
#pragma unroll
          for (int e = 0; e < EPC; ++e) {
            msc[e] = s_bias[kb + q * 32 + e]; msh[e] = s_msh[kb + q * 32 + e]; mmu[e] = s_mmu[kb + q * 32 + e];
            a1[e] = 0.f; a2[e] = 0.f;
          }
#pragma unroll
          for (int p = 0; p < TP; ++p) {
            float xr[EPC], vq[EPC];
            Elem<T>::unpack(rres[RPRE ? p : 0][RPRE ? q : 0], xr);
#pragma unroll
            for (int e = 0; e < EPC; ++e) {
              const int idx = q * EPC + e;
              const float y = acc[idx >> 2][p][idx & 3];
              const float gv = fmaf(xr[e], msc[e], msh[e]) > 0.f ? y : 0.f;
              vq[e] = gv;
              a1[e] += gv;
              a2[e] = fmaf(gv, xr[e] - mmu[e], a2[e]);
            }
            if (live) st16(yg + out_off(cur, p) + q * 64, PackH<T>::run(vq));
          }
#pragma unroll
          for (int e = 0; e < EPC; ++e) { s1[q * EPC + e] = a1[e]; s2[q * EPC + e] = a2[e]; }
        }
      } else {
        if (live) {
          if (OP == 0 && !a.bias && !a.relu) {
#pragma unroll
            for (int p = 0; p < TP; ++p)
#pragma unroll
              for (int q = 0; q < RQ; ++q) {
                float vq[EPC];
#pragma unroll
                for (int e = 0; e < EPC; ++e) vq[e] = acc[(q * EPC + e) >> 2][p][e & 3];
                st16(yg + out_off(cur, p) + q * 64, PackH<T>::run(vq));
              }
          } else {
            if (osc_on) {
#pragma unroll
              for (int j = 0; j < 4 * TK; ++j) {
                const float sj = s_msh[kb + (j >> 3) * 32 + (j & 7)];
#pragma unroll
                for (int p = 0; p < TP; ++p) acc[j >> 2][p][j & 3] *= sj;
              }
            }
            float bias[4 * TK];
#pragma unroll
            for (int j = 0; j < 4 * TK; ++j) bias[j] = s_bias[kb + (j >> 3) * 32 + (j & 7)];
            const float lo = a.relu ? 0.f : -__builtin_inff();
#pragma unroll
            for (int p = 0; p < TP; ++p)
#pragma unroll
              for (int q = 0; q < RQ; ++q) {
                float vq[EPC], rr[EPC];
                if constexpr (OP == 1) Elem<T>::unpack(rres[RPRE ? p : 0][RPRE ? q : 0], rr);
#pragma unroll
                for (int e = 0; e < EPC; ++e) {
                  float v = acc[(q * EPC + e) >> 2][p][e & 3] + bias[q * EPC + e];
                  if constexpr (OP == 1) v += rr[e];
                  vq[e] = __builtin_amdgcn_fmed3f(v, lo, __builtin_inff());
                }
                st16(yg + out_off(cur, p) + q * 64, PackH<T>::run(vq));
              }
          }
        }
        if (a.stats) {
#pragma unroll
          for (int t = 0; t < TK; ++t)
#pragma unroll
            for (int j = 0; j < 4; ++j) {
              float x1 = 0.f, x2 = 0.f;
#pragma unroll
              for (int p = 0; p < TP; ++p) { float q = acc[t][p][j]; x1 += q; x2 = fmaf(q, q, x2); }
              s1[t * 4 + j] = x1;
              s2[t * 4 + j] = x2;
            }
        }
      }
      if (a.stats) {
        row16_fold16(s1);
        row16_fold16(s2);
        if (live && (li & 3) == 0) {
          const int t = li >> 2;
          float* sp = s_stat + (wq * 2) * BKO + kb + (t >> 1) * 32 + (t & 1) * 4;
#pragma unroll
          for (int h = 0; h < 2; ++h) {
            const float* sv = h ? s2 : s1;
            f32x4_t* slot = reinterpret_cast<f32x4_t*>(sp + h * BKO);
            f32x4_t v = *slot;
#pragma unroll
            for (int e = 0; e < 4; ++e) v[e] += sv[e];
            *slot = v;
          }
        }
      }
    }
    PP_T(tb);
    PP_ACC(5, tb - ta);
    cur = nxt;
    live = live_n;
    nxt = geom(tile_of(st + 2, live_n));
    load_halo(nxt);
    PP_T(t3);
    if (!(grp == 1 && st == nst - 1)) SSLCR_PP_BAR();
    PP_T(t4);
    PP_ACC(2, t3 - t2); PP_ACC(3, t4 - t3);
  }
#ifdef SSLCR_PP_PROF
  if (blockIdx.x == 0 && lane == 0)
    for (int i = 0; i < 8; ++i) g_pp_prof[wave][i] = pp_t[i];
#endif
  SSLCR_PP_BAR();
  if (a.stats) {
    const int rw = tid >> 6, c = tid & 63;
    a.stats[((size_t)((int)blockIdx.x * 4 + (rw >> 1)) * 2 + (rw & 1)) * 64 + c] = s_f[320 + tid] + s_f[320 + 512 + tid];
    const int eb = (int)blockIdx.x + (int)gridDim.x;
    if (eb * 4 < rows_total) a.stats[((size_t)(eb * 4 + (rw >> 1)) * 2 + (rw & 1)) * 64 + c] = 0.f;
  }
}

static int pp64_grid(const ConvArgs& a) {
  const int nseg = a.seg_images > 0 ? a.N / a.seg_images : 1;
  const int tiles = (a.N / nseg) * (a.H / 16) * (a.W / 16);
  const int pairs = (tiles + 1) / 2, per = device_cus() / nseg;
  return (pairs < per ? pairs : per) * nseg;
}

bool conv_pp64_ok(int dtype, const ConvArgs& a) {
  static const bool on = [] { const char* e = getenv("SSLCR_PP64"); return !e || atoi(e) != 0; }();
  if ((size_t)a.N * a.H * a.W * 64 * 2 >= ((size_t)1 << 32)) return false;
  if (a.W > 2048) return false;
  return on && dtype == DT_BF16 && a.C == 64 && a.K == 64 && a.R == 3 && a.S == 3 && a.stride == 1 && a.pad == 1 && !a.transposed &&
         a.H % 16 == 0 && a.W % 16 == 0 && !(a.in_scale && (a.residual || a.mask_x)) &&
         !(a.out_scale && (a.in_scale || a.mask_x || a.stats || !a.bias));
}
int conv_pp64_rows(const ConvArgs& a) {
  if (a.seg_images > 0) return pp64_grid(a) * 4;
  const int tiles = a.N * (a.H / 16) * (a.W / 16);
  return (tiles < device_cus() ? tiles : device_cus()) * 4;
}

hipError_t launch_conv_pp64(const ConvArgs& a, hipStream_t st) {
  constexpr size_t lds = 9 * 64 * 128 + 2 * 18 * 18 * 128 + (320 + 1024) * sizeof(float);
  static std::atomic<bool> attr_done{false};
  if (!attr_done) {
    const void* ks[4] = {reinterpret_cast<const void*>(conv3x3_pp64_kernel<false, 0>), reinterpret_cast<const void*>(conv3x3_pp64_kernel<false, 1>),
                         reinterpret_cast<const void*>(conv3x3_pp64_kernel<false, 2>), reinterpret_cast<const void*>(conv3x3_pp64_kernel<true, 0>)};
    for (const void* k : ks) {
      hipError_t e = hipFuncSetAttribute(k, hipFuncAttributeMaxDynamicSharedMemorySize, 160 * 1024);
      if (e != hipSuccess) return e;
    }
    attr_done = true;
  }
  const int nseg = a.seg_images > 0 ? a.N / a.seg_images : 1;
  const int tiles = (a.N / nseg) * (a.H / 16) * (a.W / 16);
  const int grid = pp64_grid(a);
  if (a.mask_x && !a.stats) return hipErrorInvalidValue;
  const int rows = conv_pp64_rows(a);
  if (a.in_scale) hipLaunchKernelGGL((conv3x3_pp64_kernel<true, 0>), dim3(grid), dim3(512), lds, st, a, tiles, rows);
  else if (a.mask_x) hipLaunchKernelGGL((conv3x3_pp64_kernel<false, 2>), dim3(grid), dim3(512), lds, st, a, tiles, rows);
  else if (a.residual) hipLaunchKernelGGL((conv3x3_pp64_kernel<false, 1>), dim3(grid), dim3(512), lds, st, a, tiles, rows);
  else hipLaunchKernelGGL((conv3x3_pp64_kernel<false, 0>), dim3(grid), dim3(512), lds, st, a, tiles, rows);
  return hipGetLastError();
}

const char* conv_pp64_name(const ConvArgs& a) {
  if (a.in_scale) return "sslcr::conv3x3_pp64_kernel<true, 0>";
  return a.mask_x ? "sslcr::conv3x3_pp64_kernel<false, 2>" : (a.residual ? "sslcr::conv3x3_pp64_kernel<false, 1>" : "sslcr::conv3x3_pp64_kernel<false, 0>");
}

}
```

### ssl_cr_histo_amd/csrc/engine.cpp

```cpp
#include <rccl/rccl.h>
#include <stdio.h>
#include <stdlib.h>
#include <string.h>

#include <atomic>
#include <chrono>
#include <condition_variable>
#include <mutex>
#include <vector>

#include "kernels.hpp"

using namespace sslcr;

#define TRY(expr)                                   \
  do {                                              \
    hipError_t _e = (expr);                         \
    if (_e != hipSuccess) return check(_e, #expr);  \
  } while (0)
#define TRYI(expr)            \
  do {                        \
    int _r = (expr);          \
    if (_r != 0) return _r;   \
  } while (0)
// ... 1064 lines not shown
}
int wg_join(sslcr_ctx* c, hipStream_t waiter) {
  if (!c->wg_any) return 0;
  TRY(hipEventRecord(c->ev_wg_join, c->wg_stream));
  TRY(hipStreamWaitEvent(waiter, c->ev_wg_join, 0));
  return 0;
}

int wgrad_call(sslcr_net* n, const ConvL& L, const void* x, const void* dy, const BnSaved* pro, int N, int H, int W, int OH, int OW, hipStream_t st,
               int seg_images = 0, int seg_stride = 0, int kind = -1) {
  if (!n->rg[L.pidx]) return 0;
  sslcr_ctx* c = n->ctx;
  WgradArgs a;
  memset(&a, 0, sizeof(a));
  a.x = x; a.dy = dy; a.dw = (float*)n->grads.p + n->goff[L.pidx];
  if (pro) { a.in_scale = pro->scale; a.in_shift = pro->shift; a.in_relu = 1; }
  a.N = N; a.H = H; a.W = W; a.C = L.cin; a.K = L.cout; a.R = L.k; a.S = L.k; a.stride = L.stride; a.pad = L.pad; a.OH = OH; a.OW = OW;
  a.seg_images = seg_images; a.seg_stride = seg_stride;
  if (kind < 0 || !c->use_wg || c->prof.on) {
    TRY(prof_wgrad(c, c->dtype, a, st));
    return 0;
  }
  if (!c->wg_stream) {
    TRY(hipStreamCreateWithFlags(&c->wg_stream, hipStreamNonBlocking));
    for (int k = 0; k < 3; ++k) {
      TRY(hipEventCreateWithFlags(&c->ev_wg_in[k], hipEventDisableTiming));
      TRY(hipEventCreateWithFlags(&c->ev_wg_done[k], hipEventDisableTiming));
    }
    TRY(hipEventCreateWithFlags(&c->ev_wg_join, hipEventDisableTiming));
  }
  TRY(hipEventRecord(c->ev_wg_in[kind], st));
  TRY(hipStreamWaitEvent(c->wg_stream, c->ev_wg_in[kind], 0));
  TRY(prof_wgrad(c, c->dtype, a, c->wg_stream));
  TRY(hipEventRecord(c->ev_wg_done[kind], c->wg_stream));
  c->wg_pending[kind] = true;
  c->wg_any = true;
  return 0;
}

int launch_bucket_allreduce(sslcr_net* n, int bucket, size_t lo, size_t hi, hipStream_t st) {
  sslcr_ctx* c = n->ctx;
  if (!sharded(c) || hi <= lo) return 0;
  TRY(hipEventRecord(c->ev_ready[bucket], st));
  TRY(hipStreamWaitEvent(c->comm_stream, c->ev_ready[bucket], 0));
  TRYI(wg_join(c, c->comm_stream));
  float* g = (float*)n->grads.p + lo;
  TRYI(all_reduce(c, 1, g, hi - lo, false, c->comm_stream));
  return 0;
}

int lowest_trainable(const sslcr_net* n) {
  for (int i = 0; i < 60; ++i)
    if (n->rg[i]) return i;
  return 60;
}

int backbone_backward(sslcr_net* n, int npass, hipStream_t st) {
  sslcr_ctx* c = n->ctx;
  const int dt = c->dtype;
  const size_t es = c->esz();
  PassState* P = n->pass;
  const int N = P[0].N;
  const Dims d = make_dims(P[0].H, P[0].W);
  const int low = lowest_trainable(n);
  if (low >= 60) return 0;
  const size_t unit = (((size_t)N * d.ph * d.pw * 64 * es) + 255) & ~(size_t)255;
  const size_t stem_sz = (((size_t)N * d.oh0 * d.ow0 * 64 * es) + 255) & ~(size_t)255;
  TRYI(c->scratch.ensure(7 * npass * unit + stem_sz));
  char* S = (char*)c->scratch.p;
  auto buf = [&](int kind, int p, size_t bytes) { return S + (size_t)kind * npass * unit + (size_t)p * bytes; };
  int kOut = 0, kXin = 5;
  const int kG = 1, kRaw2 = 2, kAct1 = 3, kRaw1 = 4, kRawD = 6;
  char* dRaw0 = S + (size_t)7 * npass * unit;
  auto tap = [&](int blk, int slot, const void* src, int n_, int h_, int w_, int c_) -> int {
    if (!n->tap) return 0;
    const size_t bytes = (size_t)n_ * h_ * w_ * c_ * es;
    TRYI(n->tapbuf[blk][slot].ensure(bytes));
    TRY(hipMemcpyAsync(n->tapbuf[blk][slot].p, src, bytes, hipMemcpyDeviceToDevice, st));
    int* d4 = n->tapdims[blk][slot];
    d4[0] = n_; d4[1] = h_; d4[2] = w_; d4[3] = c_;
    return 0;
  };

  size_t hi_pending = n->goff[60];
  int bucket = 1;
  for (int p = 0; p < npass; ++p)
    TRY(launch_avgpool_bwd(dt, n->dE[p], buf(kOut, p, (size_t)N * d.lh[7] * d.lw[7] * 512 * es), N, d.lh[7] * d.lw[7], 512, st));
  for (int i = 7; i >= 0; --i) {
    BlockL& B = n->blocks[i];
    const int oh = d.lh[i], ow = d.lw[i];
    const int xh = i == 0 ? d.ph : d.lh[i - 1], xw = i == 0 ? d.pw : d.lw[i - 1];
    const size_t opix = (size_t)N * oh * ow;
    const bool need_dx = low < B.pstart;
    const size_t so = opix * B.c2.cout * es, si = (size_t)N * xh * xw * B.c1.cin * es;
    bool c2_batched = false;
    if (npass > 1) {
      WgradArgs q;
      memset(&q, 0, sizeof(q));
      q.N = N * npass; q.H = oh; q.W = ow; q.C = B.c2.cin; q.K = B.c2.cout; q.R = 3; q.S = 3; q.stride = 1; q.pad = 1; q.OH = oh; q.OW = ow;
      c2_batched = wgrad_halo_tw(q) != 0 && (wgrad_halo_tw(q) == 16 || N % 2 == 0);
    }
    ConvArgs seg_m;
    bool seg_dg = false;
    if (npass > 1 && segments_on() && !c->prof.on) {
      seg_m = conv_args(B.c2, nullptr, B.c2.w_dg, nullptr, N * npass, oh, ow);
      seg_m.C = B.c2.cout; seg_m.K = B.c2.cin; seg_m.transposed = 0; seg_m.PH = oh; seg_m.PW = ow; seg_m.OH = oh; seg_m.OW = ow;
      const BnSaved& s1 = P[0].bn[B.b1.bidx];
      seg_m.mask_x = P[0].blk[i].raw1; seg_m.mask_scale = s1.scale; seg_m.mask_shift = s1.shift; seg_m.mask_mean = s1.mean;
      seg_m.seg_images = N; seg_m.seg_stride = (int)(P[1].bn[B.b1.bidx].scale - s1.scale);
      seg_dg = conv_h16_ok(dt, seg_m) && conv_segments_ok(dt, seg_m) && conv_partials_rows(seg_m) % npass == 0;
    }
    const bool seg_bn = npass > 1 && segments_on() && !c->prof.on && !(sharded(c) && c->bn_sync) && c->bn_ring.p &&
                        c->bn_ring_i + 2 * npass <= sslcr_ctx::kBnRing;
    const int bn_stride = npass > 1 ? (int)(P[1].bn[0].scale - P[0].bn[0].scale) : 0;
    if (seg_bn) {
      char *dOut = buf(kOut, 0, so), *G = buf(kG, 0, so), *dRaw2 = buf(kRaw2, 0, so), *dRawD = buf(kRawD, 0, so);
      TRYI(wg_wait(c, 0, st));
      if (B.has_ds) TRYI(wg_wait(c, 2, st));
      const size_t apix = opix * npass;
      if (B.has_ds) {
        BnBwdArgs a2, ad;
        double* sums_2 = take_sums_n(c, npass);
        if (!sums_2) return fail("backbone_backward: ring slots");
        TRYI(bn_bwd_begin(n, B.b2, P[0].bn[B.b2.bidx], dOut, P[0].blk[i].raw2, P[0].blk[i].y, 0, dRaw2, G, apix, (double)opix, st, sums_2, &a2, nullptr, 1,
                          nullptr, 0, true, npass, bn_stride));
        TRYI(bn_bwd_begin(n, B.bd, P[0].bn[B.bd.bidx], G, P[0].blk[i].rawd, nullptr, 0, dRawD, nullptr, apix, (double)opix, st, sums_2 + 2 * B.b2.C, &ad,
                          nullptr, 0, nullptr, 0, true, npass, bn_stride));
        TRYI(bn_bwd_end(c, a2, st));
        TRYI(bn_bwd_end(c, ad, st));
      } else {
        TRYI(bn_backward(n, B.b2, P[0].bn[B.b2.bidx], dOut, P[0].blk[i].raw2, P[0].blk[i].y, 0, dRaw2, G, apix, (double)opix, st, nullptr, 1, nullptr, 0,
                         npass, bn_stride));
      }
      TRYI(tap(i, 0, G, N, oh, ow, B.c2.cout));
      TRYI(tap(i, 1, dRaw2, N, oh, ow, B.c2.cout));
      if (B.has_ds) TRYI(tap(i, 4, dRawD, N, oh, ow, B.ds.cout));
    }
    for (int p = 0; p < npass; ++p) {
      PassState& ps = P[p];
      char *dOut = buf(kOut, p, so), *G = buf(kG, p, so), *dRaw2 = buf(kRaw2, p, so), *dAct1 = buf(kAct1, p, so), *dRaw1 = buf(kRaw1, p, so),
           *dRawD = buf(kRawD, p, so);
      if (!seg_bn) {
      TRYI(wg_wait(c, 0, st));
      if (B.has_ds) TRYI(wg_wait(c, 2, st));
      if (B.has_ds) {
        BnBwdArgs a2, ad;
        double* ring = take_sums(c);
        double* sums_2 = ring ? ring : c->bn_sums;
        double* sums_d = sums_2 + 2 * B.b2.C;
        TRYI(bn_bwd_begin(n, B.b2, ps.bn[B.b2.bidx], dOut, ps.blk[i].raw2, ps.blk[i].y, 0, dRaw2, G, opix, (double)opix, st, sums_2, &a2, nullptr, 1,
                          nullptr, 0, ring != nullptr, 1, 0, true));
        TRYI(bn_bwd_begin(n, B.bd, ps.bn[B.bd.bidx], G, ps.blk[i].rawd, nullptr, 0, dRawD, nullptr, opix, (double)opix, st, sums_d, &ad, nullptr, 0,
                          nullptr, 0, ring != nullptr, 1, 0, true));
        const bool pair = bn_bwd_pair_ok(a2, ad);
        static const bool g_free = [] { const char* e = getenv("SSLCR_BN_PAIR_G"); return e && atoi(e) == 0; }();
        const int keep_g = (n->tap || !a2.yact_bits || !g_free) ? 1 : 0;
        if (pair) {
          TRY(launch_bn_bwd_reduce_pair(dt, a2, ad, keep_g, st));
        } else {
          TRY(launch_bn_bwd_reduce(dt, a2, st));
          TRY(launch_bn_bwd_reduce(dt, ad, st));
        }
        TRYI(bn_bwd_sync(c, sums_2, 4 * (size_t)B.b2.C, st));
        if (pair) {
          if (c->prof.on) {
            ProfRec r;
            r.e0 = c->prof.get(); r.e1 = c->prof.get();
            r.name = dt == DT_BF16 ? "sslcr::bn_bwd_apply_pair_kernel<unsigned short>" : "sslcr::bn_bwd_apply_pair_kernel<float>";
            r.flops = 0.0;
            r.bytes = (keep_g ? 5.0 : 5.0625) * (double)opix * B.b2.C * c->esz();
            (void)hipEventRecord(r.e0, st);
            hipError_t e = launch_bn_bwd_apply_pair(dt, a2, ad, keep_g, st);
            (void)hipEventRecord(r.e1, st);
            c->prof.rec[2].push_back(r);
            TRY(e);
          } else {
            TRY(launch_bn_bwd_apply_pair(dt, a2, ad, keep_g, st));
          }
        } else {
          TRYI(bn_bwd_end(c, a2, st));
          TRYI(bn_bwd_end(c, ad, st));
        }
      } else {
        TRYI(bn_backward(n, B.b2, ps.bn[B.b2.bidx], dOut, ps.blk[i].raw2, ps.blk[i].y, 0, dRaw2, G, opix, (double)opix, st, nullptr, 1));
      }
      if (p == 0) {
        TRYI(tap(i, 0, G, N, oh, ow, B.c2.cout));
        TRYI(tap(i, 1, dRaw2, N, oh, ow, B.c2.cout));
        if (B.has_ds) TRYI(tap(i, 4, dRawD, N, oh, ow, B.ds.cout));
      }
      }
      if (!c2_batched) TRYI(wgrad_call(n, B.c2, ps.blk[i].raw1, dRaw2, &ps.bn[B.b1.bidx], N, oh, ow, oh, ow, st, 0, 0, 0));
      if (seg_dg) continue;
      float* b1_rows = nullptr;
      int b1_nrows = 0;
      {
        ConvArgs a = conv_args(B.c2, dRaw2, B.c2.w_dg, dAct1, N, oh, ow);
        a.C = B.c2.cout; a.K = B.c2.cin; a.transposed = 0; a.PH = oh; a.PW = ow; a.OH = oh; a.OW = ow;
        ConvArgs m = a;
        const BnSaved& s1 = ps.bn[B.b1.bidx];
        m.mask_x = ps.blk[i].raw1; m.mask_scale = s1.scale; m.mask_shift = s1.shift; m.mask_mean = s1.mean;
        if (conv_h16_ok(dt, m)) {
          TRYI(ensure_partials(c, m, &b1_rows, &b1_nrows));
          m.stats = b1_rows;
          a = m;
        }
        TRY(prof_conv(c, dt,a, st));
        if (p == 0) {
          TRYI(tap(i, 2, dAct1, N, oh, ow, B.c2.cin));
          n->tap_flags[i] = b1_rows ? 1 : 0;
        }
      }
      TRYI(wg_wait(c, 1, st));
      TRYI(bn_backward(n, B.b1, ps.bn[B.b1.bidx], dAct1, ps.blk[i].raw1, nullptr, b1_rows ? 0 : 1, dRaw1, nullptr, opix, (double)opix, st,
                       nullptr, 0, b1_rows, b1_nrows));
      if (p == 0) TRYI(tap(i, 3, dRaw1, N, oh, ow, B.c1.cout));
    }
    if (seg_dg) {
      float* rows = nullptr;
      int nrows = 0;
      seg_m.x = buf(kRaw2, 0, so); seg_m.y = buf(kAct1, 0, so);
      TRYI(ensure_partials(c, seg_m, &rows, &nrows));
      seg_m.stats = rows;
      TRY(prof_conv(c, dt, seg_m, st));
      TRYI(tap(i, 2, buf(kAct1, 0, so), N, oh, ow, B.c2.cin));
      n->tap_flags[i] = 1;
      const int per = nrows / npass;
      if (seg_bn) {
        TRYI(wg_wait(c, 1, st));
        TRYI(bn_backward(n, B.b1, P[0].bn[B.b1.bidx], buf(kAct1, 0, so), P[0].blk[i].raw1, nullptr, 0, buf(kRaw1, 0, so), nullptr, opix * npass,
                         (double)opix, st, nullptr, 0, rows, nrows, npass, bn_stride));
        TRYI(tap(i, 3, buf(kRaw1, 0, so), N, oh, ow, B.c1.cout));
      }
      for (int p = 0; p < npass && !seg_bn; ++p) {
        PassState& ps = P[p];
        TRYI(wg_wait(c, 1, st));
        TRYI(bn_backward(n, B.b1, ps.bn[B.b1.bidx], buf(kAct1, p, so), ps.blk[i].raw1, nullptr, 0, buf(kRaw1, p, so), nullptr, opix, (double)opix, st,
                         nullptr, 0, rows + (size_t)p * per * 2 * B.b1.C, per));
        if (p == 0) TRYI(tap(i, 3, buf(kRaw1, 0, so), N, oh, ow, B.c1.cout));
      }
    }
    if (c2_batched)
      TRYI(wgrad_call(n, B.c2, P[0].blk[i].raw1, buf(kRaw2, 0, so), &P[0].bn[B.b1.bidx], N * npass, oh, ow, oh, ow, st, N,
                      (int)(P[1].bn[B.b1.bidx].scale - P[0].bn[B.b1.bidx].scale), 0));
    {
      const char* X0 = i == 0 ? P[0].pooled : P[0].blk[i - 1].y;
      TRYI(wgrad_call(n, B.c1, X0, buf(kRaw1, 0, so), nullptr, N * npass, xh, xw, oh, ow, st, 0, 0, 1));
      if (B.has_ds) TRYI(wgrad_call(n, B.ds, X0, buf(kRawD, 0, so), nullptr, N * npass, xh, xw, oh, ow, st, 0, 0, 2));
    }
    if (need_dx) {
      {
        const int NB = N * npass;
        char *G = buf(kG, 0, so), *dRaw1 = buf(kRaw1, 0, so), *dXin = buf(kXin, 0, si), *dRawD = buf(kRawD, 0, so);
        ConvArgs a = conv_args(B.c1, dRaw1, B.c1.w_dg, dXin, NB, oh, ow);
        a.C = B.c1.cout; a.K = B.c1.cin; a.transposed = (B.c1.stride == 1) ? 0 : 1; a.PH = xh; a.PW = xw; a.OH = xh; a.OW = xw;
        if (!B.has_ds) a.residual = G;
        if (B.c1.stride == 1) {
          TRY(prof_conv(c, dt,a, st));
        } else {
          ConvArgs q4 = a;
          q4.pix_mul = 2; q4.PH = xh / 2; q4.PW = xw / 2; q4.par4 = 1;
          const bool one = xh % 2 == 0 && xw % 2 == 0 && conv_dma_bp(dt, q4) != 0 && conv_dma_bp(DT_BF16, q4) == conv_dma_bp(dt, q4) &&
                           conv_halo_tw(dt, q4) == 0;
          if (one) TRY(prof_conv(c, dt, q4, st));
          for (int par = 0; par < (one ? 0 : 4); ++par) {
            ConvArgs q = a;
            const int ph_ = par >> 1, pw_ = par & 1;
            q.pix_mul = 2; q.pix_off_h = ph_; q.pix_off_w = pw_;
            q.PH = (xh - ph_ + 1) / 2; q.PW = (xw - pw_ + 1) / 2;
            if (q.PH <= 0 || q.PW <= 0) continue;
            unsigned m = 0;
            for (int r = 0; r < 3; ++r)
              for (int s2 = 0; s2 < 3; ++s2)
                if (((ph_ + 1 - r) & 1) == 0 && ((pw_ + 1 - s2) & 1) == 0) m |= 1u << (r * 3 + s2);
            q.tap_mask = m;
            TRY(prof_conv(c, dt,q, st));
          }
        }
        if (B.has_ds) {
          ConvArgs s = conv_args(B.ds, dRawD, B.ds.w_dg, dXin, NB, oh, ow);
          s.C = B.ds.cout; s.K = B.ds.cin; s.stride = 1; s.pad = 0; s.PH = oh; s.PW = ow; s.OH = xh; s.OW = xw; s.osh = B.ds.stride;
          s.accumulate = 1;
          TRY(prof_conv(c, dt,s, st));
        }
        TRYI(tap(i, 5, dXin, N, xh, xw, B.c1.cin));
      }
      const int t = kOut; kOut = kXin; kXin = t;
    }
    if (i == 6 || i == 4 || i == 2) {
      TRYI(launch_bucket_allreduce(n, bucket++, n->goff[B.pstart], hi_pending, st));
      hi_pending = n->goff[B.pstart];
    }
    if (!need_dx) break;
  }
  if (low < 3) {
    for (int p = 0; p < npass; ++p) {
      PassState& ps = P[p];
      PoolSrc pool{buf(kOut, p, (size_t)N * d.ph * d.pw * 64 * es), ps.argmax, d.oh0, d.ow0, d.ph, d.pw, ps.pooled};
      const size_t spix = (size_t)N * d.oh0 * d.ow0;
      StemWgradArgs w;
      memset(&w, 0, sizeof(w));
      w.x = ps.x; w.x2 = ps.x2; w.n_split = ps.n_split; w.dy = dRaw0; w.dw = (float*)n->grads.p + n->goff[0];
      w.N = N; w.H = ps.H; w.W = ps.W; w.OH = d.oh0; w.OW = d.ow0; w.in_f32 = ps.in_f32;
      if (n->rg[0] && c->fuse_stem_bwd) {
        BnBwdArgs a;
        double* ring = take_sums(c);
        double* sums0 = ring ? ring : c->bn_sums;
        TRYI(bn_bwd_begin(n, n->bn0, ps.bn[0], nullptr, ps.raw0, nullptr, 1, nullptr, nullptr, spix, (double)spix, st, sums0, &a, &pool, 0, nullptr, 0,
                          ring != nullptr));
        TRYI(bn_bwd_sync(c, sums0, 2 * 64, st));
        w.dy = nullptr;
        if (c->prof.on) {
          ProfRec r;
          r.e0 = c->prof.get(); r.e1 = c->prof.get();
          r.name = dt == DT_BF16 ? "sslcr::stem_wgrad_kernel<unsigned short, pool>" : "sslcr::stem_wgrad_kernel<float, pool>";
          r.flops = 0.0;
          const double t = (double)spix * 64 * c->esz();
          r.bytes = 0.25 * t + 0.25 * (double)spix * 64 + t + (double)N * 3 * ps.H * ps.W * (ps.in_f32 ? 4 : 1);
          (void)hipEventRecord(r.e0, st);
          hipError_t e = launch_stem_wgrad_pool(dt, w, a, st);
          (void)hipEventRecord(r.e1, st);
          c->prof.rec[2].push_back(r);
          TRY(e);
        } else {
          TRY(launch_stem_wgrad_pool(dt, w, a, st));
        }
        continue;
      }
      TRYI(bn_backward(n, n->bn0, ps.bn[0], nullptr, ps.raw0, nullptr, 1, dRaw0, nullptr, spix, (double)spix, st, &pool));
      if (n->rg[0]) TRY(launch_stem_wgrad(dt, w, st));
    }
  }
  TRYI(launch_bucket_allreduce(n, bucket, 0, hi_pending, st));
  return 0;
}

int net_forward(sslcr_net* n, int train, const void* const* xs, int in_f32, int N, int H, int W, float* feats, float* logits, hipStream_t st) {
  if (!(train ? n->packed_train : n->packed_eval)) TRYI(sslcr_net_pack(n, train ? 1 : 2, st));
  const int npass_ = n->triplet ? 3 : 1;
  if (n->n8 > 0 && !n->f8_cal[train ? 0 : 1]) {
    n->f8_calib_pass = true;
    TRYI(alloc_heads(n, N));
    int rc = 0;
    for (int i = 0; i < npass_ && rc == 0 && train; ++i)
      rc = backbone_forward_train(n, n->pass[i], xs[i], in_f32, N, H, W, n->triplet ? 1 : 3, st);
    if (!train) rc = backbone_forward_eval(n, xs, npass_, in_f32, N, H, W, n->dE, st);
    n->f8_calib_pass = false;
    if (rc) return rc;
    n->f8_cal[train ? 0 : 1] = true;
  }
  if (n->n8 > 0) TRY(launch_fp8_scale_update(n->f8slots, n->n8, st));
  if (train) n->packed_eval = false;
  const int npass = n->triplet ? 3 : 1;
  TRYI(alloc_heads(n, N));
  float* E[3] = {nullptr, nullptr, nullptr};
  const bool segs = train && npass == 3 && segments_servable(n, N, H, W);
  if (train) n->last_segments = segs;
  if (segs) {
    TRYI(backbone_forward_train_segments(n, xs, in_f32, N, H, W, st));
    for (int i = 0; i < npass; ++i) E[i] = n->pass[i].E;
  }
  for (int i = 0; i < npass && !segs && train; ++i) {
    TRYI(backbone_forward_train(n, n->pass[i], xs[i], in_f32, N, H, W, n->triplet ? 1 : 3, st));
    E[i] = n->pass[i].E;
  }
  if (!train) {
    for (int i = 0; i < npass; ++i) E[i] = n->dE[i];
    TRYI(backbone_forward_eval(n, xs, npass, in_f32, N, H, W, E, st));
  }
  TRYI(heads_forward(n, E, npass, N, st));
  if (feats) TRY(hipMemcpyAsync(feats, n->feats, (size_t)N * 768 * 4, hipMemcpyDeviceToDevice, st));
  if (logits) TRY(hipMemcpyAsync(logits, n->logits, (size_t)N * n->ncls * 4, hipMemcpyDeviceToDevice, st));
  n->last_N = N; n->last_npass = train ? npass : 0;
  return 0;
}

int net_backward(sslcr_net* n, const float* dlogits, hipStream_t st) {
  sslcr_ctx* c = n->ctx;
  if (n->last_npass == 0) return fail("sslcr_net_backward: no train-mode forward to differentiate");
  const int N = n->last_N, npass = n->last_npass;
  TRYI(n->grads.ensure(n->grad_count * sizeof(float)));
  TRY(hipMemsetAsync(n->grads.p, 0, n->grad_count * sizeof(float), st));
  const bool bb = lowest_trainable(n) < 60;
  if (bb) {
    TRYI(c->bn_ring.ensure((size_t)sslcr_ctx::kBnRing * sslcr_ctx::kBnSlot * sizeof(double)));
    c->bn_ring_i = 0;
  }
  TRYI(heads_backward(n, dlogits, npass, N, bb, st));
  TRYI(launch_bucket_allreduce(n, 0, n->goff[60], n->goff[n->nparams], st));
  if (bb) {
    TRYI(backbone_backward(n, npass, st));
  }
  if (sharded(c)) {
    TRY(hipEventRecord(c->ev_done, c->comm_stream));
    TRY(hipStreamWaitEvent(st, c->ev_done, 0));
  }
  TRYI(wg_join(c, st));
  c->wg_any = false;
  for (bool& pnd : c->wg_pending) pnd = false;
  return 0;
}

}

extern "C" {

int sslcr_create(sslcr_ctx** out, int device, int dtype) {
  if (!out || (dtype != SSLCR_F32 && dtype != SSLCR_BF16 && dtype != SSLCR_FP8)) return fail("sslcr_create: invalid argument");
  TRY(hipSetDevice(device));
  sslcr_ctx* c = new sslcr_ctx();
  c->device = device; c->dtype = dtype == SSLCR_FP8 ? SSLCR_BF16 : dtype; c->fp8 = dtype == SSLCR_FP8;
  if (const char* e = getenv("SSLCR_FUSE_STEM_BWD")) c->fuse_stem_bwd = atoi(e) != 0;
  if (c->small.ensure((size_t)kMaxSeg * 32 * 2 * 512 * sizeof(double) + 2 * 2 * 512 * sizeof(double) + 2 * 512 * sizeof(float) + 64 * sizeof(int)) != 0) { delete c; return -1; }
  c->bn_stage = (double*)c->small.p;
  c->bn_sums = c->bn_stage + (size_t)kMaxSeg * 32 * 2 * 512;
  c->ones = (float*)(c->bn_sums + 2 * 2 * 512);
  c->zeros = c->ones + 512;
  c->bn_tickets = (int*)(c->zeros + 512);
  TRY(hipMemset(c->bn_tickets, 0, 64 * sizeof(int)));
  TRY(launch_fill(c->ones, 512, 1.f, nullptr));
  TRY(launch_fill(c->zeros, 512, 0.f, nullptr));
  TRY(hipStreamSynchronize(nullptr));
  g_live_ctx.fetch_add(1);
  *out = c;
  return 0;
}

int sslcr_destroy(sslcr_ctx* c) {
  if (!c) return 0;
  (void)hipDeviceSynchronize();
  if (c->wg_stream) {
    (void)hipStreamDestroy(c->wg_stream);
    for (int k = 0; k < 3; ++k) { (void)hipEventDestroy(c->ev_wg_in[k]); (void)hipEventDestroy(c->ev_wg_done[k]); }
    (void)hipEventDestroy(c->ev_wg_join);
  }
  if (c->aux_stream) {
    (void)hipStreamDestroy(c->aux_stream);
    (void)hipEventDestroy(c->ev_aux_begin);
    (void)hipEventDestroy(c->ev_aux_end);
  }
  if (c->comm || c->vcomm) {
    if (c->comm) ncclCommDestroy(c->comm);
    if (c->comm_g) ncclCommDestroy(c->comm_g);
    (void)hipStreamDestroy(c->comm_stream);
    for (int i = 0; i < 8; ++i) (void)hipEventDestroy(c->ev_ready[i]);
    (void)hipEventDestroy(c->ev_done);
  }
  c->scratch.release(); c->partials.release(); c->small.release(); c->bn_ring.release();
  if (g_live_ctx.fetch_sub(1) == 1) stream_scratch_release();
  delete c;
  return 0;
}

int sslcr_profile(sslcr_ctx* c, int enable) {
  if (!c) return fail("sslcr_profile: null");
  c->prof.on = enable != 0;
  if (enable) {
    for (int w = 0; w < 3; ++w) {
      for (auto& r : c->prof.rec[w]) { c->prof.pool.push_back(r.e0); c->prof.pool.push_back(r.e1); }
      c->prof.rec[w].clear();
    }
  }
  return 0;
}

int sslcr_profile_dump(sslcr_ctx* c, char* buf, size_t n) {
  if (!c || !buf || n < 64) return fail("sslcr_profile_dump: invalid argument");
  TRY(hipDeviceSynchronize());
  struct Row { const char* name; double launches, ms, flops, bytes; };
  std::vector<Row> rows;
  for (int w = 0; w < 3; ++w)
    for (auto& r : c->prof.rec[w]) {
      float t = 0.f;
      TRY(hipEventElapsedTime(&t, r.e0, r.e1));
      Row* hit = nullptr;
      for (auto& q : rows)
        if (strcmp(q.name, r.name) == 0) { hit = &q; break; }
      if (!hit) { rows.push_back(Row{r.name, 0, 0, 0, 0}); hit = &rows.back(); }
      hit->launches += 1; hit->ms += t; hit->flops += r.flops; hit->bytes += r.bytes;
    }
  size_t off = 0;
  for (auto& q : rows) {
    int k = snprintf(buf + off, n - off, "%s|%.0f|%.6f|%.6e|%.6e\n", q.name, q.launches, q.ms, q.flops, q.bytes);
    if (k < 0 || (size_t)k >= n - off) return fail("sslcr_profile_dump: buffer too small");
    off += k;
  }
  buf[off] = 0;
  return 0;
}

int sslcr_profile_read(sslcr_ctx* c, int which, double* out4) {
// ... 406 lines not shown
```

### ssl_cr_histo_amd/csrc/kernels.hpp

```cpp
#pragma once
#include "common.hpp"
#include "../../include/sslcr.h"

namespace sslcr {

using ConvArgs = sslcr_conv_desc;
using WgradArgs = sslcr_wgrad_desc;
using StemArgs = sslcr_stem_desc;
using StemWgradArgs = sslcr_stem_wgrad_desc;
using BnFinalizeArgs = sslcr_bn_finalize_desc;
using BnActArgs = sslcr_bn_act_desc;
using PoolFwdArgs = sslcr_pool_fwd_desc;
using PoolBwdArgs = sslcr_pool_bwd_desc;
using BnBwdArgs = sslcr_bn_bwd_desc;
using LossArgs = sslcr_loss_desc;
using TensorDesc = sslcr_tensor_desc;
using OptArgs = sslcr_opt_desc;
using PackArgs = sslcr_pack_desc;
using Fp8Args = sslcr_fp8_desc;
using PackFp8Args = sslcr_pack_fp8_desc;

hipError_t launch_conv(int dtype, const ConvArgs& a, hipStream_t st);
int conv_tile_bp(const ConvArgs& a);
const char* conv_kernel_name(int dtype, const ConvArgs& a);
const char* wgrad_kernel_name(int dtype, const WgradArgs& a);
int conv_partials_rows(const ConvArgs& a);
bool conv_segments_ok(int dtype, const ConvArgs& a);
int device_cus();
int conv_halo_tw(int dtype, const ConvArgs& a);
int conv_halo_tiles(const ConvArgs& a, int tw);
hipError_t launch_conv_halo(int dtype, const ConvArgs& a, int tw, hipStream_t st);
int conv_halo256_mode(int dtype, const ConvArgs& a);
int conv_halo256_tiles(const ConvArgs& a, int mode);
hipError_t launch_conv_halo256(int dtype, const ConvArgs& a, int mode, hipStream_t st);
bool conv_h16_ok(int dtype, const ConvArgs& a);
int conv_h16_rows(const ConvArgs& a);
hipError_t launch_conv_h16(int dtype, const ConvArgs& a, hipStream_t st);
const char* conv_h16_name(int dtype, const ConvArgs& a);
bool conv_pp64_ok(int dtype, const ConvArgs& a);
hipError_t launch_conv_pp64(const ConvArgs& a, hipStream_t st);
const char* conv_pp64_name(const ConvArgs& a);
int conv_pp64_rows(const ConvArgs& a);
int conv_dma_bp(int dtype, const ConvArgs& a);
int conv_dma_rows(const ConvArgs& a, int bp);
hipError_t launch_conv_dma(int dtype, const ConvArgs& a, int bp, hipStream_t st);
const char* conv_dma_name(int dtype, int bp);
bool conv_s2_ok(int dtype, const ConvArgs& a);
bool conv_s2_pair_ok(int dtype, const ConvArgs& a, const ConvArgs& d);
int conv_s2_rows(const ConvArgs& a);
hipError_t launch_conv_s2(const ConvArgs& a, const ConvArgs* d, hipStream_t st);
const char* conv_s2_name(const ConvArgs& a, bool pair);
bool conv_s2d_ok(int dtype, const ConvArgs& a);
hipError_t launch_conv_s2d(const ConvArgs& a, hipStream_t st);
const char* conv_s2d_name();
int conv_fp8_mode(const ConvArgs& a);
int conv_fp8_rows(const ConvArgs& a);
const char* conv_fp8_name(const ConvArgs& a);
hipError_t launch_conv_fp8(const ConvArgs& a, const Fp8Args& q, hipStream_t st);
hipError_t launch_pack_fp8(const PackFp8Args& a, hipStream_t st);
hipError_t launch_fp8_scale_update(float* slots, int n, hipStream_t st);
hipError_t launch_wgrad(int dtype, const WgradArgs& a, hipStream_t st);
int wgrad_halo_tw(const WgradArgs& a);
void* stream_scratch(hipStream_t st, size_t bytes);
void stream_scratch_release();
hipError_t launch_wgrad_fold(const void* slabs, float* dw, int C, int gx, int gy, int splits, int taps, int kh_n, hipStream_t st);
hipError_t launch_stem_wgrad_fold(const void* slabs, float* dw, int nwg, hipStream_t st);
hipError_t launch_wgrad_halo(int dtype, const WgradArgs& a, int tw, hipStream_t st);
bool wgrad_dma_ok(int dtype, const WgradArgs& a, int splits);
bool wgrad_dma_used(int dtype, const WgradArgs& a);
hipError_t launch_wgrad_dma(const WgradArgs& a, int tw, int tps, int ntiles, int splits, void* slabs, hipStream_t st);
hipError_t launch_probe_tr16(const uint16_t* in, const int* byte_addr, uint16_t* out, hipStream_t st);
bool wgrad_s2_ok(int dtype, const WgradArgs& a);
hipError_t launch_wgrad_s2(const WgradArgs& a, hipStream_t st);
hipError_t launch_stem(int dtype, const StemArgs& a, hipStream_t st);
int stem_partials_rows(const StemArgs& a);
hipError_t launch_stem_wgrad(int dtype, const StemWgradArgs& a, hipStream_t st);
hipError_t launch_stem_wgrad_pool(int dtype, const StemWgradArgs& a, const sslcr_bn_bwd_desc& b, hipStream_t st);
bool stem_pool_ok(int dtype, const StemArgs& a, int POH, int POW);
hipError_t launch_stem_pool(int dtype, const StemArgs& a, int POH, int POW, hipStream_t st);
hipError_t launch_bn_finalize(const BnFinalizeArgs& a, hipStream_t st);
hipError_t launch_bn_act(int dtype, const BnActArgs& a, hipStream_t st);
hipError_t launch_bn_relu_maxpool(int dtype, const PoolFwdArgs& a, hipStream_t st);
hipError_t launch_maxpool_relu_bwd(int dtype, const PoolBwdArgs& a, hipStream_t st);
hipError_t launch_avgpool_fwd(int dtype, const void* x, float* y, int N, int HW, int C, hipStream_t st);
hipError_t launch_avgpool_bwd(int dtype, const float* dy, void* dx, int N, int HW, int C, hipStream_t st);
hipError_t launch_bn_bwd_reduce(int dtype, const BnBwdArgs& a, hipStream_t st);
hipError_t launch_bn_bwd_apply(int dtype, const BnBwdArgs& a, hipStream_t st);
bool bn_bwd_pair_ok(const BnBwdArgs& a, const BnBwdArgs& b);
hipError_t launch_bn_bwd_reduce_pair(int dtype, const BnBwdArgs& a, const BnBwdArgs& b, int keep_g, hipStream_t st);
hipError_t launch_bn_bwd_apply_pair(int dtype, const BnBwdArgs& a, const BnBwdArgs& b, int from_g, hipStream_t st);
hipError_t launch_bn_param_grads(const double* sums, const float* invstd, float* dgamma, float* dbeta, int C, hipStream_t st);
hipError_t launch_bn_param_grads_scaled(const double* sums, const float* invstd, float* dgamma, float* dbeta, int C, float scale, hipStream_t st);
hipError_t launch_linear_fwd(const float* x, const float* w, const float* b, float* y, int M, int N, int K, int relu, hipStream_t st);
hipError_t launch_linear_bwd(const float* x, const float* w, const float* dy, const float* yact, float* dx, float* dw, float* db,
                             int M, int N, int K, int dx_accumulate, float* scratch, hipStream_t st);
hipError_t launch_loss(const LossArgs& a, hipStream_t st);
hipError_t launch_softmax_col(const float* logits, float* out, int n, int C, int col, hipStream_t st);
hipError_t launch_weak_augment(const sslcr_weak_aug_desc& a, hipStream_t st);
hipError_t launch_hed_colour(const sslcr_colour_aug_desc& a, hipStream_t st);
hipError_t launch_brightness_contrast(const sslcr_brightness_contrast_desc& a, hipStream_t st);
hipError_t launch_optimizer(const TensorDesc* d_descs, int ntensors, int max_n, const OptArgs& o, hipStream_t st);
constexpr int OPT_CHUNK = 2048;
constexpr int OPT_TILE = 16 * 16 * 9;
hipError_t launch_optimizer_chunks(const TensorDesc* d_descs, const void* d_chunks , int nchunks,
                                   const OptArgs& o, hipStream_t st);
hipError_t launch_axpby(float* p, float* q, size_t n, float alpha, int copy_back, hipStream_t st);
hipError_t launch_fill(float* p, size_t n, float v, hipStream_t st);
hipError_t launch_pack_conv(int dtype, const PackArgs& a, hipStream_t st);
hipError_t launch_pack_stem(int dtype, const PackArgs& a, hipStream_t st);
hipError_t launch_copy2d(float* dst, long ldd, const float* src, long lds, int rows, int w, int accumulate, hipStream_t st);
hipError_t launch_copy2d_multi(float* dst, long ldd, int ndst, long dstep, const float* src, long lds, int nsrc, long sstep, int rows, int w,
                               hipStream_t st);
hipError_t launch_unpack_grad(const float* g, float* out, int K, int C, int RS, hipStream_t st);
int fail(const char* fmt, ...);
int check(hipError_t e, const char* what);

}
```

### ssl_cr_histo_amd/kernels.py

```python
import torch

from . import _lib as L

F32, BF16 = 0, 1


def tdtype(dtype):
    return torch.bfloat16 if dtype == BF16 else torch.float32


def _dt(t):
    if t.dtype == torch.bfloat16:
        return BF16
    if t.dtype == torch.float32:
        return F32
    raise TypeError(f"unsupported activation dtype {t.dtype}")


def _chk(*ts):
    for t in ts:
        if t is not None:
            if not t.is_cuda:
                raise L.SslcrError("sslcr kernels need device tensors (no CPU fallback)")
            if not t.is_contiguous():
                raise L.SslcrError("sslcr kernels need contiguous tensors")


last_conv_kernel = ""
last_wgrad_kernel = ""


def conv2d(x, w, stride, pad, *, in_scale=None, in_shift=None, in_relu=False, bias=None, residual=None, relu=False,
           want_stats=False, out=None, transposed=False, out_hw=None, osh=1, accumulate=False, pixel_hw=None,
           pix_mul=0, pix_off=(0, 0), tap_mask=0, mask=None, par4=False, seg_images=0, out_scale=None):
    _chk(x, w, in_scale, in_shift, bias, residual, out, out_scale)
    dt = _dt(x)
    N, H, W, C = x.shape
    K, R, S, C2 = w.shape
    assert C2 == C and w.dtype == x.dtype
    if transposed:
        PH, PW = pixel_hw
    else:
        PH, PW = (H + 2 * pad - R) // stride + 1, (W + 2 * pad - S) // stride + 1
    OH, OW = out_hw if out_hw is not None else (PH * osh, PW * osh)
    y = out if out is not None else torch.empty((N, OH, OW, K), dtype=x.dtype, device=x.device)
    d = L.ConvDesc(L.ptr(x), L.ptr(w), L.ptr(y), L.ptr(in_scale), L.ptr(in_shift), L.ptr(bias), L.ptr(residual), None,
                   N, H, W, C, K, R, S, stride, pad, PH, PW, OH, OW, osh, int(transposed), int(in_relu), int(relu),
                   int(accumulate), int(pix_mul), int(pix_off[0]), int(pix_off[1]), int(tap_mask))
    d.par4 = int(par4)
    d.out_scale = L.ptr(out_scale)
    if seg_images:
        d.seg_images = int(seg_images)
        d.seg_stride = int(in_scale.stride(0)) if in_scale is not None and in_scale.dim() == 2 else 0
        if not L.lib().sslcr_conv2d_segments_ok(dt, d):
            raise L.SslcrError("conv2d: no segment form for this shape / dtype")
    if mask is not None:
        _chk(*mask)
        d.mask_x, d.mask_scale, d.mask_shift, d.mask_mean = (L.ptr(t) for t in mask)
    stats = None
    if want_stats:
        rows = L.lib().sslcr_conv2d_partial_rows(d)
        stats = torch.full((rows, 2, K), float("nan"), dtype=torch.float32, device=x.device)
        d.stats = L.ptr(stats)
    global last_conv_kernel
    last_conv_kernel = L.lib().sslcr_conv2d_kernel_name(dt, d).decode()
    L.check(L.lib().sslcr_conv2d(dt, d, L.stream_ptr()))
    return (y, stats) if want_stats else y


def conv2d_s2_pair(x, w3, w1, *, bias3=None, bias1=None, relu3=False, want_stats=False, scale3=None, scale1=None):
    _chk(x, w3, w1, bias3, bias1, scale3, scale1)
    dt = _dt(x)
    N, H, W, C = x.shape
    K = w3.shape[0]
    assert w3.shape == (K, 3, 3, C) and w1.shape == (K, 1, 1, C)
    PH, PW = H // 2, W // 2
    y3 = torch.empty((N, PH, PW, K), dtype=x.dtype, device=x.device)
    yd = torch.empty_like(y3)
    d3 = L.ConvDesc(L.ptr(x), L.ptr(w3), L.ptr(y3), None, None, L.ptr(bias3), None, None,
                    N, H, W, C, K, 3, 3, 2, 1, PH, PW, PH, PW, 1, 0, 0, int(relu3), 0, 0, 0, 0, 0)
    d1 = L.ConvDesc(L.ptr(x), L.ptr(w1), L.ptr(yd), None, None, L.ptr(bias1), None, None,
                    N, H, W, C, K, 1, 1, 2, 0, PH, PW, PH, PW, 1, 0, 0, 0, 0, 0, 0, 0, 0)
    d3.out_scale, d1.out_scale = L.ptr(scale3), L.ptr(scale1)
    s3 = sd = None
    if want_stats:
        rows = L.lib().sslcr_conv2d_partial_rows(d3)
        s3 = torch.full((rows, 2, K), float("nan"), dtype=torch.float32, device=x.device)
        sd = torch.full((rows, 2, K), float("nan"), dtype=torch.float32, device=x.device)
        d3.stats, d1.stats = L.ptr(s3), L.ptr(sd)
    if not L.lib().sslcr_conv2d_s2_pair_ok(dt, d3, d1):
        raise L.SslcrError("conv2d_s2_pair: not served")
    L.check(L.lib().sslcr_conv2d_s2_pair(dt, d3, d1, L.stream_ptr()))
    return (y3, yd, s3, sd) if want_stats else (y3, yd)


def pack_conv_fp8(w_kcrs, *, bn=None, eps=1e-5):
    _chk(w_kcrs)
    K, C, R, S = w_kcrs.shape
    assert R == 3 and S == 3
    dev = w_kcrs.device
    w8 = torch.empty((K, 3, 3, C), dtype=torch.uint8, device=dev)
    dq = torch.empty(K, dtype=torch.float32, device=dev)
    bias = torch.empty(K, dtype=torch.float32, device=dev) if bn is not None else None
    g, b, rm, rv = bn if bn is not None else (None, None, None, None)
    d = L.PackFp8Desc(L.ptr(w_kcrs), L.ptr(w8), L.ptr(dq), L.ptr(g), L.ptr(b), L.ptr(rm), L.ptr(rv), eps, L.ptr(bias), K, C)
    L.check(L.lib().sslcr_pack_conv_fp8(d, L.stream_ptr()))
    return w8, dq, bias


def conv2d_fp8(x, w8, w_dequant, *, x_scale=1.0, in_scale=None, in_shift=None, in_relu=False, bias=None, residual=None, relu=False,
               want_stats=False, amax_out=None):
    _chk(x, w8, w_dequant, in_scale, in_shift, bias, residual)
    assert x.dtype == torch.bfloat16 and w8.dtype == torch.uint8
    N, H, W, C = x.shape
    K = w8.shape[0]
    y = torch.empty((N, H, W, K), dtype=torch.bfloat16, device=x.device)
    d = L.ConvDesc(L.ptr(x), None, L.ptr(y), L.ptr(in_scale), L.ptr(in_shift), L.ptr(bias), L.ptr(residual), None,
                   N, H, W, C, K, 3, 3, 1, 1, H, W, H, W, 1, 0, int(in_relu), int(relu), 0, 0, 0, 0, 0)
    q = L.Fp8Desc(L.ptr(w8), L.ptr(w_dequant), float(x_scale), None, L.ptr(amax_out))
    stats = None
    if want_stats:
        rows = L.lib().sslcr_conv2d_fp8_partial_rows(d)
        stats = torch.full((rows, 2, K), float("nan"), dtype=torch.float32, device=x.device)
        d.stats = L.ptr(stats)
    L.check(L.lib().sslcr_conv2d_fp8(d, q, L.stream_ptr()))
    return (y, stats) if want_stats else y


def conv2d_wgrad(x, dy, dw, R, S, stride, pad, *, in_scale=None, in_shift=None, in_relu=False, seg_images=0):
    _chk(x, dy, dw, in_scale, in_shift)
    N, H, W, C = x.shape
    _, OH, OW, K = dy.shape
    assert dw.shape == (K, R, S, C) and dw.dtype == torch.float32
# ... 87 lines not shown
    N, _, H, W = x_nchw.shape
    n_split = 0
    if x2 is not None:
        n_split, N = N, N + x2.shape[0]
    _, OH, OW, Cn = raw.shape
    pixels = raw.numel() // Cn
    sums = torch.zeros((2, Cn), dtype=torch.float64, device=raw.device)
    pdy, pam = pool[0], pool[1]
    _chk(pdy, pam)
    b = L.BnBwdDesc(None, L.ptr(raw), None, L.ptr(scale), L.ptr(shift), L.ptr(mean), L.ptr(invstd), L.ptr(sums),
                    None, None, pixels, Cn, 1, float(count if count is not None else pixels),
                    L.ptr(pdy), L.ptr(pam), OH, OW, pdy.shape[1], pdy.shape[2], None, 0)
    if len(pool) > 2 and pool[2] is not None:
        _chk(pool[2])
        b.pool_y = L.ptr(pool[2])
    if dgamma is not None:
        b.dgamma, b.dbeta, b.pg_scale = L.ptr(dgamma), L.ptr(dbeta), 1.0
    L.check(L.lib().sslcr_bn_bwd_reduce(_dt(raw), b, L.stream_ptr()))
    w = L.StemWgradDesc(L.ptr(x_nchw), None, L.ptr(dw), N, H, W, OH, OW, int(x_nchw.dtype == torch.float32),
                        L.ptr(x2), int(n_split))
    L.check(L.lib().sslcr_stem_wgrad_pool(_dt(raw), w, b, L.stream_ptr()))
    return sums


def bn_finalize(partials, count, gamma, beta, *, running_mean=None, running_var=None, nbt=None, momentum=0.1,
                eps=1e-5, replay=1, nseg=1, one_launch=True):
    _chk(partials, gamma, beta, running_mean, running_var, nbt)
    rows, _, Cn = partials.shape
    dev = partials.device
    shape = (nseg, Cn) if nseg > 1 else (Cn,)
    scale, shift, mean, invstd = (torch.empty(shape, dtype=torch.float32, device=dev) for _ in range(4))
    stage = torch.empty((max(nseg, 1), 32, 2, Cn), dtype=torch.float64, device=dev)
    tickets = torch.zeros((Cn + 31) // 32, dtype=torch.int32, device=dev) if one_launch else None
    d = L.BnFinalizeDesc(L.ptr(partials), rows, Cn, float(count), L.ptr(gamma), L.ptr(beta), L.ptr(scale), L.ptr(shift),
                         L.ptr(mean), L.ptr(invstd), L.ptr(running_mean), L.ptr(running_var), L.ptr(nbt), momentum, eps,
                         replay, None, None, L.ptr(stage), nseg if nseg > 1 else 0, Cn if nseg > 1 else 0, L.ptr(tickets))
    L.check(L.lib().sslcr_bn_finalize(d, L.stream_ptr()))
    return scale, shift, mean, invstd


def bn_act(x, scale, shift, *, res=None, rscale=None, rshift=None, relu=True, nseg=1, want_bits=False):
    _chk(x, scale, shift, res, rscale, rshift)
    y = torch.empty_like(x)
    Cn = x.shape[-1]
    d = L.BnActDesc(L.ptr(x), L.ptr(scale), L.ptr(shift), L.ptr(res), L.ptr(rscale), L.ptr(rshift), L.ptr(y),
                    x.numel() // Cn, Cn, int(relu), nseg if nseg > 1 else 0, Cn if nseg > 1 else 0)
    bits = None
    if want_bits:
        bits = torch.full((x.numel() // 8,), 0xa5, dtype=torch.uint8, device=x.device)
        d.ybits = L.ptr(bits)
    L.check(L.lib().sslcr_bn_act(_dt(x), d, L.stream_ptr()))
    return (y, bits) if want_bits else y


def bn_relu_maxpool(x, scale, shift):
    _chk(x, scale, shift)
    N, H, W, Cn = x.shape
    OH, OW = (H - 1) // 2 + 1, (W - 1) // 2 + 1
    y = torch.empty((N, OH, OW, Cn), dtype=x.dtype, device=x.device)
    am = torch.empty((N, OH, OW, Cn), dtype=torch.uint8, device=x.device) if scale is not None else None
    d = L.PoolFwdDesc(L.ptr(x), L.ptr(scale), L.ptr(shift), L.ptr(y), L.ptr(am), N, H, W, Cn, OH, OW)
    L.check(L.lib().sslcr_bn_relu_maxpool(_dt(x), d, L.stream_ptr()))
    return y, am


def maxpool_relu_bwd(dy, argmax, x, scale, shift):
    _chk(dy, argmax, x, scale, shift)
    N, H, W, Cn = x.shape
    _, OH, OW, _ = dy.shape
    dx = torch.empty_like(x)
    d = L.PoolBwdDesc(L.ptr(dy), L.ptr(argmax), L.ptr(x), L.ptr(scale), L.ptr(shift), L.ptr(dx), N, H, W, Cn, OH, OW)
    L.check(L.lib().sslcr_maxpool_relu_bwd(_dt(x), d, L.stream_ptr()))
    return dx


def avgpool_fwd(x):
    _chk(x)
    N, H, W, Cn = x.shape
    y = torch.empty((N, Cn), dtype=torch.float32, device=x.device)
    L.check(L.lib().sslcr_avgpool_fwd(_dt(x), L.ptr(x), L.ptr(y), N, H * W, Cn, L.stream_ptr()))
    return y


def avgpool_bwd(dy, shape, dtype):
    _chk(dy)
    N, H, W, Cn = shape
    dx = torch.empty(shape, dtype=tdtype(dtype), device=dy.device)
    L.check(L.lib().sslcr_avgpool_bwd(dtype, L.ptr(dy), L.ptr(dx), N, H * W, Cn, L.stream_ptr()))
    return dx


def bn_bwd(dy, x, scale, shift, mean, invstd, *, yact=None, relu_from_x=False, want_g=False, count=None, pool=None,
           g_in_reduce=False, nseg=1, dgamma=None, dbeta=None, yact_bits=None):
    _chk(x, scale, shift, mean, invstd, yact, dgamma, dbeta)
    if dy is not None:
        _chk(dy)
    Cn = x.shape[-1]
    pixels = x.numel() // Cn
    sums = torch.zeros((nseg, 2, Cn) if nseg > 1 else (2, Cn), dtype=torch.float64, device=x.device)
    dx = torch.empty_like(x)
    g = torch.empty_like(x) if want_g else None
    d = L.BnBwdDesc(L.ptr(dy), L.ptr(x), L.ptr(yact), L.ptr(scale), L.ptr(shift), L.ptr(mean), L.ptr(invstd), L.ptr(sums),
                    L.ptr(dx), L.ptr(g), pixels, Cn, int(relu_from_x), float(count if count is not None else pixels // nseg),
                    None, None, 0, 0, 0, 0, None, int(g_in_reduce))
    if dgamma is not None:
        d.dgamma, d.dbeta, d.pg_scale = L.ptr(dgamma), L.ptr(dbeta), 1.0
    if yact_bits is not None:
        _chk(yact_bits)
        d.yact_bits = L.ptr(yact_bits)
    if nseg > 1:
        d.nseg, d.seg_stride, d.sums_stride = nseg, Cn, 2 * Cn
    if pool is not None:
        pdy, pam = pool[0], pool[1]
        _chk(pdy, pam)
        d.pool_dy, d.pool_argmax = L.ptr(pdy), L.ptr(pam)
        if len(pool) > 2 and pool[2] is not None:
            _chk(pool[2])
            d.pool_y = L.ptr(pool[2])
        d.pH, d.pW, d.pOH, d.pOW = x.shape[1], x.shape[2], pdy.shape[1], pdy.shape[2]
    L.check(L.lib().sslcr_bn_bwd_reduce(_dt(x), d, L.stream_ptr()))
    L.check(L.lib().sslcr_bn_bwd_apply(_dt(x), d, L.stream_ptr()))
    return dx, sums, g


def bn_param_grads(sums, invstd, dgamma, dbeta):
    _chk(sums, invstd, dgamma, dbeta)
    L.check(L.lib().sslcr_bn_param_grads(L.ptr(sums), L.ptr(invstd), L.ptr(dgamma), L.ptr(dbeta), invstd.numel(),
                                         L.stream_ptr()))


def linear_fwd(x, w, b, relu=False):
    _chk(x, w, b)
    M, K = x.shape
    N = w.shape[0]
    y = torch.empty((M, N), dtype=torch.float32, device=x.device)
    L.check(L.lib().sslcr_linear_fwd(L.ptr(x), L.ptr(w), L.ptr(b), L.ptr(y), M, N, K, int(relu), L.stream_ptr()))
    return y


def linear_bwd(x, w, dy, *, yact=None, dw=None, db=None, want_dx=True, dx=None, dx_accumulate=False):
    _chk(x, w, dy, yact, dw, db, dx)
    M, K = x.shape
    N = w.shape[0]
    if want_dx and dx is None:
        dx = torch.empty((M, K), dtype=torch.float32, device=x.device)
    scratch = torch.empty((M, N), dtype=torch.float32, device=x.device)
    L.check(L.lib().sslcr_linear_bwd(L.ptr(x), L.ptr(w), L.ptr(dy), L.ptr(yact), L.ptr(dx) if want_dx else None,
                                     L.ptr(dw), L.ptr(db), M, N, K, int(dx_accumulate), L.ptr(scratch), L.stream_ptr()))
    return dx


def loss(kind, logits, *, logits_t=None, target_f=None, target_i=None, nx, lambda_u=1.0, want_grad=True,
         nx_global=None, nu_global=None):
    _chk(logits, logits_t, target_f, target_i)
    Ns, Cn = logits.shape
    nu = Ns - nx
    dl = torch.zeros_like(logits) if want_grad else None
    out = torch.zeros(4, dtype=torch.float32, device=logits.device)
    d = L.LossDesc(kind, L.ptr(logits), L.ptr(logits_t), L.ptr(target_f), L.ptr(target_i), L.ptr(dl), L.ptr(out), nx, nu,
                   Cn, lambda_u, 1.0 / (nx_global or nx), 1.0 / max(1, (nu_global or nu)))
    L.check(L.lib().sslcr_loss(d, L.stream_ptr()))
    return out, dl


def softmax_col(logits, col=-1):
    _chk(logits)
    n, c = logits.shape
    out = torch.empty(n, dtype=torch.float32, device=logits.device)
    L.check(L.lib().sslcr_softmax_col(L.ptr(logits), L.ptr(out), n, c, col % c, L.stream_ptr()))
    return out
```

Measured before the change: 72520.

## Fuse ReLU-mask application into dgrad conv epilogue and masked avgpool backward

The stride-1 dgrad conv epilogue can now apply the next block's output ReLU bitmask while it adds the residual, writing the masked skip gradient directly. The backward BN of the following block then takes that gradient as given instead of rebuilding G from the saved activation. The avgpool backward can also apply the mask bits. This removes a separate read of the activation tensor and the recomputation of G. In exchange it adds new kernel instantiations and extra eligibility checks, and it falls back to the old path when a shape is not eligible.

```diff
diff --git a/include/sslcr.h b/include/sslcr.h
--- a/include/sslcr.h
+++ b/include/sslcr.h
@@ -37,6 +37,7 @@
   int par4;
   int seg_images, seg_stride;
   const float* out_scale;
+  const uint8_t* out_bits;
 } sslcr_conv_desc;
 int sslcr_conv2d(int dtype, const sslcr_conv_desc* d, void* stream);
 int sslcr_conv2d_partial_rows(const sslcr_conv_desc* d);
@@ -137,6 +138,7 @@
 
 int sslcr_avgpool_fwd(int dtype, const void* x, float* y, int N, int HW, int C, void* stream);
 int sslcr_avgpool_bwd(int dtype, const float* dy, void* dx, int N, int HW, int C, void* stream);
+int sslcr_avgpool_bwd_masked(int dtype, const float* dy, void* dx, const uint8_t* bits, int N, int HW, int C, void* stream);
 
 typedef struct sslcr_bn_bwd_desc {
   const void* dy; const void* x; const void* yact;
diff --git a/ssl_cr_histo_amd/_lib.py b/ssl_cr_histo_amd/_lib.py
--- a/ssl_cr_histo_amd/_lib.py
+++ b/ssl_cr_histo_amd/_lib.py
@@ -22,7 +22,7 @@
               [(k, i32) for k in ("N", "H", "W", "C", "K", "R", "S", "stride", "pad", "PH", "PW", "OH", "OW", "osh",
                                   "transposed", "in_relu", "relu", "accumulate", "pix_mul", "pix_off_h", "pix_off_w")] +
               [("tap_mask", C.c_uint), ("mask_x", vp), ("mask_scale", vp), ("mask_shift", vp), ("mask_mean", vp),
-               ("par4", i32), ("seg_images", i32), ("seg_stride", i32), ("out_scale", vp)])
+               ("par4", i32), ("seg_images", i32), ("seg_stride", i32), ("out_scale", vp), ("out_bits", vp)])
 WgradDesc = _S("WgradDesc", [("x", vp), ("dy", vp), ("dw", vp), ("in_scale", vp), ("in_shift", vp), ("in_relu", i32)] +
                [(k, i32) for k in ("N", "H", "W", "C", "K", "R", "S", "stride", "pad", "OH", "OW", "seg_images", "seg_stride")])
 StemDesc = _S("StemDesc", [("x", vp), ("w", vp), ("y", vp), ("bias", vp), ("stats", vp)] +
@@ -92,6 +92,7 @@
     "sslcr_maxpool_relu_bwd": (i32, [i32, P(PoolBwdDesc), vp]),
     "sslcr_avgpool_fwd": (i32, [i32, vp, vp, i32, i32, i32, vp]),
     "sslcr_avgpool_bwd": (i32, [i32, vp, vp, i32, i32, i32, vp]),
+    "sslcr_avgpool_bwd_masked": (i32, [i32, vp, vp, vp, i32, i32, i32, vp]),
     "sslcr_bn_bwd_reduce": (i32, [i32, P(BnBwdDesc), vp]),
     "sslcr_bn_bwd_apply": (i32, [i32, P(BnBwdDesc), vp]),
     "sslcr_bn_param_grads": (i32, [vp, vp, vp, vp, i32, vp]),
diff --git a/ssl_cr_histo_amd/csrc/bn_eltwise.hip b/ssl_cr_histo_amd/csrc/bn_eltwise.hip
--- a/ssl_cr_histo_amd/csrc/bn_eltwise.hip
+++ b/ssl_cr_histo_amd/csrc/bn_eltwise.hip
@@ -542,7 +542,7 @@
 }
 
 template <typename T>
-__global__ __launch_bounds__(256) void avgpool_bwd_kernel(const float* dy, void* dxv, int N, int HW, int C) {
+__global__ __launch_bounds__(256) void avgpool_bwd_kernel(const float* dy, void* dxv, int N, int HW, int C, const uint8_t* __restrict__ bits) {
   constexpr int EPC = Elem<T>::EPC;
   const int cols = C / EPC;
   const size_t total = (size_t)N * HW * cols;
@@ -554,6 +554,12 @@
     float f[EPC];
 #pragma unroll
     for (int e = 0; e < EPC; ++e) f[e] = dy[(size_t)n * C + col * EPC + e] * inv;
+    if (EPC == 8 && bits) {
+      const unsigned b = bits[i];
+#pragma unroll
+      for (int e = 0; e < EPC; ++e)
+        if (!((b >> e) & 1u)) f[e] = 0.f;
+    }
     st16_nt(dx + i * 16, Elem<T>::pack(f));
   }
 }
@@ -566,11 +572,12 @@
   }
   return hipGetLastError();
 }
-hipError_t launch_avgpool_bwd(int dtype, const float* dy, void* dx, int N, int HW, int C, hipStream_t st) {
+hipError_t launch_avgpool_bwd(int dtype, const float* dy, void* dx, int N, int HW, int C, hipStream_t st, const uint8_t* bits) {
+  if (bits && dtype != DT_BF16) return hipErrorInvalidValue;
   if (dtype == DT_BF16) {
-    hipLaunchKernelGGL(avgpool_bwd_kernel<bf16_t>, dim3(ew_grid((size_t)N * HW * (C / 8))), dim3(256), 0, st, dy, dx, N, HW, C);
+    hipLaunchKernelGGL(avgpool_bwd_kernel<bf16_t>, dim3(ew_grid((size_t)N * HW * (C / 8))), dim3(256), 0, st, dy, dx, N, HW, C, bits);
   } else {
-    hipLaunchKernelGGL(avgpool_bwd_kernel<float>, dim3(ew_grid((size_t)N * HW * (C / 4))), dim3(256), 0, st, dy, dx, N, HW, C);
+    hipLaunchKernelGGL(avgpool_bwd_kernel<float>, dim3(ew_grid((size_t)N * HW * (C / 4))), dim3(256), 0, st, dy, dx, N, HW, C, bits);
   }
   return hipGetLastError();
 }
diff --git a/ssl_cr_histo_amd/csrc/capi.cpp b/ssl_cr_histo_amd/csrc/capi.cpp
--- a/ssl_cr_histo_amd/csrc/capi.cpp
+++ b/ssl_cr_histo_amd/csrc/capi.cpp
@@ -1,4 +1,5 @@
 #include <stdarg.h>
+#include <stdint.h>
 #include <stdio.h>
 #include <string.h>
 
@@ -29,7 +30,7 @@
 
 extern "C" {
 
-int sslcr_version(void) { return 6; }
+int sslcr_version(void) { return 7; }
 const char* sslcr_last_error(void) { return g_err; }
 
 int sslcr_conv2d(int dtype, const sslcr_conv_desc* d, void* stream) {
@@ -40,6 +41,11 @@
   NEED(d->K % 64 == 0, "K % 64");
   NEED(d->osh >= 1 && d->PH > 0 && d->PW > 0, "pixel space");
   NEED(conv_segments_ok(dtype, *d), "seg_images: no segment form for this shape / dtype (sslcr_conv2d_segments_ok)");
+  if (d->out_bits) {
+    NEED(((uintptr_t)d->out_bits & 1) == 0, "out_bits must be 2-byte aligned");
+    NEED(conv_out_bits_ok(dtype, *d), "out_bits: the skip-gradient form only (residual; no in_scale / bias / relu / stats / mask_x / out_scale / "
+                                      "accumulate / segments), bf16, on a shape the 16x16-tile kernels serve");
+  }
   return check(launch_conv(dtype, *d, (hipStream_t)stream), "conv2d");
 }
 int sslcr_conv2d_partial_rows(const sslcr_conv_desc* d) { return d ? conv_partials_rows(*d) : -1; }
@@ -148,6 +154,11 @@
   NEED(dy && dx && N > 0 && HW > 0 && C % 8 == 0, "args");
   return check(launch_avgpool_bwd(dtype, dy, dx, N, HW, C, (hipStream_t)stream), "avgpool_bwd");
 }
+int sslcr_avgpool_bwd_masked(int dtype, const float* dy, void* dx, const uint8_t* bits, int N, int HW, int C, void* stream) {
+  NEED(dtype == SSLCR_BF16, "dtype (the mask bits exist in bf16 only)");
+  NEED(dy && dx && bits && N > 0 && HW > 0 && C % 8 == 0, "args");
+  return check(launch_avgpool_bwd(dtype, dy, dx, N, HW, C, (hipStream_t)stream, bits), "avgpool_bwd_masked");
+}
 int sslcr_bn_bwd_reduce(int dtype, const sslcr_bn_bwd_desc* d, void* stream) {
   DT_OK(dtype);
   NEED(d && (d->dy || (d->pool_dy && d->pool_argmax)) && d->x && d->sums && d->mean, "null");
diff --git a/ssl_cr_histo_amd/csrc/conv_h16.hip b/ssl_cr_histo_amd/csrc/conv_h16.hip
--- a/ssl_cr_histo_amd/csrc/conv_h16.hip
+++ b/ssl_cr_histo_amd/csrc/conv_h16.hip
@@ -39,13 +39,19 @@
 template <typename T, int BKO, int WK, bool XF, bool WR, bool RAW = false, int TW = 16>
 __global__ __launch_bounds__(256 * WK, WK == 1 ? 1 : 2) void conv3x3_h16_kernel(const ConvArgs a, const int tiles_total, const int n_items, const int kshift,
                                                                                 const int row0) {
-  constexpr bool OSC = false;
+  constexpr bool OSC = false, RO = false;
 #include "conv_h16_body.hpp"
 }
 template <typename T, int BKO, int WK, bool WR, int TW>
 __global__ __launch_bounds__(256 * WK, WK == 1 ? 1 : 2) void conv3x3_h16s_kernel(const ConvArgs a, const int tiles_total, const int n_items, const int kshift,
                                                                                  const int row0) {
-  constexpr bool OSC = true, XF = false, RAW = false;
+  constexpr bool OSC = true, RO = false, XF = false, RAW = false;
+#include "conv_h16_body.hpp"
+}
+template <typename T, int BKO, int WK, int TW>
+__global__ __launch_bounds__(256 * WK, WK == 1 ? 1 : 2) void conv3x3_h16r_kernel(const ConvArgs a, const int tiles_total, const int n_items, const int kshift,
+                                                                                 const int row0) {
+  constexpr bool OSC = false, RO = true, XF = false, WR = false, RAW = false;
 #include "conv_h16_body.hpp"
 }
 
@@ -96,6 +102,7 @@
   t.x = reinterpret_cast<const char*>(a.x) + px * a.C * es;
   t.y = reinterpret_cast<char*>(a.y) + px * a.K * es;
   if (a.residual) t.residual = reinterpret_cast<const char*>(a.residual) + px * a.K * es;
+  if (a.out_bits) t.out_bits = a.out_bits + px * a.K / 8;
   return t;
 }
 int conv_h16_rows(const ConvArgs& a) {
@@ -111,16 +118,19 @@
   return on && a.stats && !a.bias && !a.relu && !a.residual && !a.mask_x;
 }
 
-template <typename T, int BKO, int WK, bool XF, bool WR = false, bool RAW = false, int TW = 16, bool OSC = false>
+template <typename T, int BKO, int WK, bool XF, bool WR = false, bool RAW = false, int TW = 16, bool OSC = false, bool RO = false>
 static hipError_t launch_h(const ConvArgs& a, hipStream_t st, int row0 = 0) {
   const size_t lds = (TW == 16 ? 18 * 24 : 4 * 10 * 10) * 128 + (WR ? 3 : 2) * 3 * BKO * 128 + 2 * a.C * sizeof(float) + 8 * BKO * sizeof(float) +
                      (a.mask_x ? 3 : (a.out_scale ? 2 : 1)) * a.K * sizeof(float);
   if (lds > 160 * 1024) return hipErrorInvalidValue;
   static_assert(!OSC || (!XF && !RAW), "output scale: eval forms only");
+  static_assert(!RO || (!OSC && !XF && !WR && !RAW && sizeof(T) == 2), "mask bits: the bf16 skip-gradient form only");
   void (*kern)(const ConvArgs, const int, const int, const int, const int);
-  if constexpr (OSC) kern = conv3x3_h16s_kernel<T, BKO, WK, WR, TW>;
+  if constexpr (RO) kern = conv3x3_h16r_kernel<T, BKO, WK, TW>;
+  else if constexpr (OSC) kern = conv3x3_h16s_kernel<T, BKO, WK, WR, TW>;
   else kern = conv3x3_h16_kernel<T, BKO, WK, XF, WR, RAW, TW>;
   if (OSC != (a.out_scale != nullptr)) return hipErrorInvalidValue;
+  if (RO != (a.out_bits != nullptr) || (RO && !a.residual)) return hipErrorInvalidValue;
   static std::atomic<bool> attr_done{false};
   if (!attr_done) {
     hipError_t e = hipFuncSetAttribute(reinterpret_cast<const void*>(kern), hipFuncAttributeMaxDynamicSharedMemorySize, 160 * 1024);
@@ -141,6 +151,8 @@
 static hipError_t launch_ht8(const ConvArgs& a, hipStream_t st) {
   const bool xf = a.in_scale != nullptr;
   auto wide = [&](const ConvArgs& q) {
+    if constexpr (sizeof(T) == 2)
+      if (q.out_bits) return launch_h<T, 128, 2, false, false, false, 8, false, true>(q, st);
     if (q.out_scale) return launch_h<T, 128, 2, false, false, false, 8, true>(q, st);
     if constexpr (sizeof(T) == 2)
       if (h16_raw(q)) return xf ? launch_h<T, 128, 2, true, false, true, 8>(q, st) : launch_h<T, 128, 2, false, false, true, 8>(q, st);
@@ -152,6 +164,8 @@
   hipError_t e = wide(head);
   if (e != hipSuccess) return e;
   const int row0 = h16_grid(head, 128) * 4;
+  if constexpr (sizeof(T) == 2)
+    if (tl.out_bits) return launch_h<T, 64, 2, false, false, false, 8, false, true>(tl, st, row0);
   if (tl.out_scale) return launch_h<T, 64, 2, false, false, false, 8, true>(tl, st, row0);
   return xf ? launch_h<T, 64, 2, true, false, false, 8>(tl, st, row0) : launch_h<T, 64, 2, false, false, false, 8>(tl, st, row0);
 }
@@ -161,6 +175,8 @@
   const bool xf = a.in_scale != nullptr;
   if (h16_mode(Elem<T>::DT, a) == 8) return launch_ht8<T>(a, st);
   if (a.K % 128 == 0) {
+    if constexpr (sizeof(T) == 2)
+      if (a.out_bits) return launch_h<T, 128, 2, false, false, false, 16, false, true>(a, st);
     if (a.out_scale) return launch_h<T, 128, 2, false, false, false, 16, true>(a, st);
     if constexpr (sizeof(T) == 2)
       if (h16_raw(a)) return xf ? launch_h<T, 128, 2, true, false, true>(a, st) : launch_h<T, 128, 2, false, false, true>(a, st);
@@ -176,13 +192,26 @@
   return xf ? launch_h<T, 64, 2, true>(a, st) : launch_h<T, 64, 2, false>(a, st);
 }
 
+bool conv_out_bits_ok(int dtype, const ConvArgs& a) {
+  if (dtype != DT_BF16 || !a.residual || a.in_scale || a.bias || a.relu || a.stats || a.mask_x || a.out_scale || a.accumulate || a.seg_images > 0)
+    return false;
+  if (!conv_h16_ok(dtype, a)) return false;
+  return a.K % 128 == 0 || (h16_resident(a) && conv_pp64_ok(DT_BF16, a));
+}
+
 hipError_t launch_conv_h16(int dtype, const ConvArgs& a, hipStream_t st) {
   if (a.mask_x && !a.stats) return hipErrorInvalidValue;
+  if (a.out_bits && !conv_out_bits_ok(dtype, a)) return hipErrorInvalidValue;
   return dtype == DT_BF16 ? launch_ht<bf16_t>(a, st) : launch_ht<float>(a, st);
 }
 
 const char* conv_h16_name(int dtype, const ConvArgs& a) {
   const bool bf = dtype == DT_BF16, xf = a.in_scale != nullptr;
+  if (a.out_bits && conv_out_bits_ok(dtype, a)) {
+    if (h16_mode(dtype, a) == 8) return "sslcr::conv3x3_h16r_kernel<unsigned short, 128, 2, 8>";
+    if (a.K % 128 == 0) return "sslcr::conv3x3_h16r_kernel<unsigned short, 128, 2, 16>";
+    return conv_pp64_name(a);
+  }
   if (a.out_scale) {
     if (h16_mode(dtype, a) == 8) return bf ? "sslcr::conv3x3_h16s_kernel<unsigned short, 128, 2, false, 8>" : "sslcr::conv3x3_h16s_kernel<float, 128, 2, false, 8>";
     if (a.K % 128 == 0) return bf ? "sslcr::conv3x3_h16s_kernel<unsigned short, 128, 2, false, 16>" : "sslcr::conv3x3_h16s_kernel<float, 128, 2, false, 16>";
diff --git a/ssl_cr_histo_amd/csrc/conv_h16_body.hpp b/ssl_cr_histo_amd/csrc/conv_h16_body.hpp
--- a/ssl_cr_histo_amd/csrc/conv_h16_body.hpp
+++ b/ssl_cr_histo_amd/csrc/conv_h16_body.hpp
@@ -32,10 +32,11 @@
   }
   for (int i = tid; i < 8 * BKO; i += NT) s_stat[i] = 0.f;
   float* s_bias = s_stat + 8 * BKO;
-  const bool mk = !OSC && !XF && !RAW && a.mask_x != nullptr;
+  const bool mk = !OSC && !RO && !XF && !RAW && a.mask_x != nullptr;
   float* s_msh = s_bias + a.K;
   float* s_mmu = s_msh + a.K;
   float* s_osc = s_msh;
+  if constexpr (!RO)
   for (int i = tid; i < a.K; i += NT) {
     const size_t mo = (size_t)seg * a.seg_stride + i;
     s_bias[i] = mk ? a.mask_scale[mo] : (a.bias ? a.bias[i] : 0.f);
@@ -204,10 +205,12 @@
   frags(0, 0, s_w);
 
   char* yg = reinterpret_cast<char*>(a.y);
-  const char* rg = (XF || RAW) ? nullptr : reinterpret_cast<const char*>(a.mask_x ? a.mask_x : a.residual);
+  const char* rg = (XF || RAW) ? nullptr : reinterpret_cast<const char*>((!RO && a.mask_x) ? a.mask_x : a.residual);
   constexpr bool RPRE = sizeof(T) == 2 && !XF && !RAW;
   constexpr int RQ = 4 * TK / EPC;
   u32x4_t rres[RPRE ? TP : 1][RPRE ? RQ : 1];
+  static_assert(!RO || (RPRE && (4 * TK == 16 || 4 * TK == 8)), "mask bits: one 16-bit or 8-bit load per pixel");
+  unsigned rbits[RO ? TP : 1];
   auto out_off = [&](const Geo& q, int p) {
     const int h = q.h0 + wp * 4 + p, w = q.w0 + li;
     const size_t pix = TW == 16 ? ((size_t)q.n0 * a.H + h) * a.W + w : (size_t)(q.n0 + wp) * 64 + p * 16 + li;
@@ -234,6 +237,13 @@
           for (int p = 0; p < TP; ++p)
 #pragma unroll
             for (int q = 0; q < RQ; ++q) rres[p][q] = ld16(rg + out_off(cur, p) + q * 16);
+          if constexpr (RO) {
+#pragma unroll
+            for (int p = 0; p < TP; ++p) {
+              const uint8_t* bp = a.out_bits + (out_off(cur, p) >> 4);
+              rbits[p] = 4 * TK == 16 ? (unsigned)*reinterpret_cast<const unsigned short*>(bp) : (unsigned)*bp;
+            }
+          }
         }
       }
     };
@@ -305,7 +315,23 @@
     if (last) {
       const int kb = cur.k0 + wk * (BKO / WK) + g * (4 * TK);
       float s1[4 * TK], s2[4 * TK];
-      if (mk) {
+      if constexpr (RO) {
+#pragma unroll
+        for (int p = 0; p < TP; ++p) {
+          const size_t off = out_off(cur, p);
+#pragma unroll
+          for (int q = 0; q < 4 * TK / EPC; ++q) {
+            float vq[EPC], rr[EPC];
+            Elem<T>::unpack(rres[RPRE ? p : 0][RPRE ? q : 0], rr);
+#pragma unroll
+            for (int e = 0; e < EPC; ++e) {
+              const int idx = q * EPC + e;
+              vq[e] = ((rbits[RO ? p : 0] >> idx) & 1u) ? acc[idx >> 2][p][idx & 3] + rr[e] : 0.f;
+            }
+            st16(yg + off + q * 16, PackH<T>::run(vq));
+          }
+        }
+      } else if (mk) {
 #pragma unroll
         for (int q = 0; q < 4 * TK / EPC; ++q) {
           float msc[EPC], msh[EPC], mmu[EPC], a1[EPC], a2[EPC];
@@ -416,7 +442,7 @@
       }
       }
       constexpr bool FOLD = (4 * TK) % 16 == 0;
-      if (a.stats) {
+      if (!RO && a.stats) {
         if constexpr (FOLD) {
 #pragma unroll
           for (int f = 0; f < 4 * TK / 16; ++f) {
@@ -487,7 +513,7 @@
     for (int i = 0; i < 8; ++i) g_h16_prof[wave][i] = h16_t[i];
   }
 #endif
-  if (a.stats) {
+  if (!RO && a.stats) {
     for (int kbi = 0; kbi < a.K / BKO; ++kbi) {
       if ((pub >> kbi) & 1u) continue;
       for (int i = tid; i < 8 * BKO; i += NT) {
diff --git a/ssl_cr_histo_amd/csrc/conv_igemm.hip b/ssl_cr_histo_amd/csrc/conv_igemm.hip
--- a/ssl_cr_histo_amd/csrc/conv_igemm.hip
+++ b/ssl_cr_histo_amd/csrc/conv_igemm.hip
@@ -341,6 +341,7 @@
 hipError_t launch_conv(int dtype, const ConvArgs& a, hipStream_t st) {
   if (!conv_segments_ok(dtype, a)) return hipErrorInvalidValue;
   if (a.out_scale && (!a.bias || a.stats || a.mask_x)) return hipErrorInvalidValue;
+  if (a.out_bits && !conv_out_bits_ok(dtype, a)) return hipErrorInvalidValue;
   if (conv_h16_ok(dtype, a)) return launch_conv_h16(dtype, a, st);
   if (a.mask_x) return hipErrorInvalidValue;
   const int q = conv_halo256_mode(dtype, a);
diff --git a/ssl_cr_histo_amd/csrc/conv_pp64.hip b/ssl_cr_histo_amd/csrc/conv_pp64.hip
--- a/ssl_cr_histo_amd/csrc/conv_pp64.hip
+++ b/ssl_cr_histo_amd/csrc/conv_pp64.hip
@@ -172,6 +172,7 @@
   char* yg = reinterpret_cast<char*>(a.y);
   const char* rg = OP == 0 ? nullptr : reinterpret_cast<const char*>(OP == 2 ? a.mask_x : a.residual);
   u32x4_t rres[RPRE ? TP : 1][RPRE ? RQ : 1];
+  unsigned rbits[OP == 3 ? TP : 1][OP == 3 ? RQ : 1];
   auto out_off = [&](const Geo& q, int p) {
     const int h = q.h0 + wq * 4 + p, w = q.w0 + li;
     return (unsigned)(((q.n0 * a.H + h) * a.W + w) * 64 + g * 8) * (unsigned)sizeof(T);
@@ -182,6 +183,12 @@
       for (int p = 0; p < TP; ++p)
 #pragma unroll
         for (int qq = 0; qq < RQ; ++qq) rres[p][qq] = ld16(rg + out_off(q, p) + qq * 64);
+    }
+    if constexpr (OP == 3) {
+#pragma unroll
+      for (int p = 0; p < TP; ++p)
+#pragma unroll
+        for (int qq = 0; qq < RQ; ++qq) rbits[p][qq] = a.out_bits[(out_off(q, p) >> 4) + qq * 4];
     }
   };
 
@@ -273,6 +280,20 @@
 #pragma unroll
           for (int e = 0; e < EPC; ++e) { s1[q * EPC + e] = a1[e]; s2[q * EPC + e] = a2[e]; }
         }
+      } else if constexpr (OP == 3) {
+        if (live) {
+#pragma unroll
+          for (int p = 0; p < TP; ++p)
+#pragma unroll
+            for (int q = 0; q < RQ; ++q) {
+              float vq[EPC], rr[EPC];
+              Elem<T>::unpack(rres[RPRE ? p : 0][RPRE ? q : 0], rr);
+              const unsigned b = rbits[OP == 3 ? p : 0][OP == 3 ? q : 0];
+#pragma unroll
+              for (int e = 0; e < EPC; ++e) vq[e] = ((b >> e) & 1u) ? acc[(q * EPC + e) >> 2][p][e & 3] + rr[e] : 0.f;
+              st16(yg + out_off(cur, p) + q * 64, PackH<T>::run(vq));
+            }
+        }
       } else {
         if (live) {
           if (OP == 0 && !a.bias && !a.relu) {
@@ -327,7 +348,7 @@
             }
         }
       }
-      if (a.stats) {
+      if (OP != 3 && a.stats) {
         row16_fold16(s1);
         row16_fold16(s2);
         if (live && (li & 3) == 0) {
@@ -361,7 +382,7 @@
     for (int i = 0; i < 8; ++i) g_pp_prof[wave][i] = pp_t[i];
 #endif
   SSLCR_PP_BAR();
-  if (a.stats) {
+  if (OP != 3 && a.stats) {
     const int rw = tid >> 6, c = tid & 63;
     a.stats[((size_t)((int)blockIdx.x * 4 + (rw >> 1)) * 2 + (rw & 1)) * 64 + c] = s_f[320 + tid] + s_f[320 + 512 + tid];
     const int eb = (int)blockIdx.x + (int)gridDim.x;
@@ -394,8 +415,9 @@
   constexpr size_t lds = 9 * 64 * 128 + 2 * 18 * 18 * 128 + (320 + 1024) * sizeof(float);
   static std::atomic<bool> attr_done{false};
   if (!attr_done) {
-    const void* ks[4] = {reinterpret_cast<const void*>(conv3x3_pp64_kernel<false, 0>), reinterpret_cast<const void*>(conv3x3_pp64_kernel<false, 1>),
-                         reinterpret_cast<const void*>(conv3x3_pp64_kernel<false, 2>), reinterpret_cast<const void*>(conv3x3_pp64_kernel<true, 0>)};
+    const void* ks[5] = {reinterpret_cast<const void*>(conv3x3_pp64_kernel<false, 0>), reinterpret_cast<const void*>(conv3x3_pp64_kernel<false, 1>),
+                         reinterpret_cast<const void*>(conv3x3_pp64_kernel<false, 2>), reinterpret_cast<const void*>(conv3x3_pp64_kernel<true, 0>),
+                         reinterpret_cast<const void*>(conv3x3_pp64_kernel<false, 3>)};
     for (const void* k : ks) {
       hipError_t e = hipFuncSetAttribute(k, hipFuncAttributeMaxDynamicSharedMemorySize, 160 * 1024);
       if (e != hipSuccess) return e;
@@ -407,7 +429,9 @@
   const int grid = pp64_grid(a);
   if (a.mask_x && !a.stats) return hipErrorInvalidValue;
   const int rows = conv_pp64_rows(a);
-  if (a.in_scale) hipLaunchKernelGGL((conv3x3_pp64_kernel<true, 0>), dim3(grid), dim3(512), lds, st, a, tiles, rows);
+  if (a.out_bits && (!a.residual || a.in_scale || a.mask_x || a.bias || a.relu || a.stats || a.out_scale || nseg > 1)) return hipErrorInvalidValue;
+  if (a.out_bits) hipLaunchKernelGGL((conv3x3_pp64_kernel<false, 3>), dim3(grid), dim3(512), lds, st, a, tiles, rows);
+  else if (a.in_scale) hipLaunchKernelGGL((conv3x3_pp64_kernel<true, 0>), dim3(grid), dim3(512), lds, st, a, tiles, rows);
   else if (a.mask_x) hipLaunchKernelGGL((conv3x3_pp64_kernel<false, 2>), dim3(grid), dim3(512), lds, st, a, tiles, rows);
   else if (a.residual) hipLaunchKernelGGL((conv3x3_pp64_kernel<false, 1>), dim3(grid), dim3(512), lds, st, a, tiles, rows);
   else hipLaunchKernelGGL((conv3x3_pp64_kernel<false, 0>), dim3(grid), dim3(512), lds, st, a, tiles, rows);
@@ -415,6 +439,7 @@
 }
 
 const char* conv_pp64_name(const ConvArgs& a) {
+  if (a.out_bits) return "sslcr::conv3x3_pp64_kernel<false, 3>";
   if (a.in_scale) return "sslcr::conv3x3_pp64_kernel<true, 0>";
   return a.mask_x ? "sslcr::conv3x3_pp64_kernel<false, 2>" : (a.residual ? "sslcr::conv3x3_pp64_kernel<false, 1>" : "sslcr::conv3x3_pp64_kernel<false, 0>");
 }
diff --git a/ssl_cr_histo_amd/csrc/engine.cpp b/ssl_cr_histo_amd/csrc/engine.cpp
--- a/ssl_cr_histo_amd/csrc/engine.cpp
+++ b/ssl_cr_histo_amd/csrc/engine.cpp
@@ -1170,10 +1170,17 @@
     return 0;
   };
 
+  static const bool dout_mask_on = [] { const char* e = getenv("SSLCR_DOUT_MASK"); return !e || atoi(e) != 0; }();
+  const bool mask_dout = dout_mask_on && !n->tap && dt == DT_BF16 && npass == 1;
+  auto bits_for = [&](int blk) -> const uint8_t* { return (mask_dout && blk >= 0) ? ybits_of(n, P[0].blk[blk].y) : nullptr; };
+  bool g_given = false;
   size_t hi_pending = n->goff[60];
   int bucket = 1;
-  for (int p = 0; p < npass; ++p)
-    TRY(launch_avgpool_bwd(dt, n->dE[p], buf(kOut, p, (size_t)N * d.lh[7] * d.lw[7] * 512 * es), N, d.lh[7] * d.lw[7], 512, st));
+  for (int p = 0; p < npass; ++p) {
+    const uint8_t* bits = bits_for(7);
+    TRY(launch_avgpool_bwd(dt, n->dE[p], buf(kOut, p, (size_t)N * d.lh[7] * d.lw[7] * 512 * es), N, d.lh[7] * d.lw[7], 512, st, bits));
+    g_given = bits != nullptr;
+  }
   for (int i = 7; i >= 0; --i) {
     BlockL& B = n->blocks[i];
     const int oh = d.lh[i], ow = d.lw[i];
@@ -1236,13 +1243,17 @@
         double* ring = take_sums(c);
         double* sums_2 = ring ? ring : c->bn_sums;
         double* sums_d = sums_2 + 2 * B.b2.C;
-        TRYI(bn_bwd_begin(n, B.b2, ps.bn[B.b2.bidx], dOut, ps.blk[i].raw2, ps.blk[i].y, 0, dRaw2, G, opix, (double)opix, st, sums_2, &a2, nullptr, 1,
-                          nullptr, 0, ring != nullptr, 1, 0, true));
-        TRYI(bn_bwd_begin(n, B.bd, ps.bn[B.bd.bidx], G, ps.blk[i].rawd, nullptr, 0, dRawD, nullptr, opix, (double)opix, st, sums_d, &ad, nullptr, 0,
+        char* Gb = g_given ? dOut : G;
+        TRYI(bn_bwd_begin(n, B.b2, ps.bn[B.b2.bidx], dOut, ps.blk[i].raw2, g_given ? nullptr : ps.blk[i].y, 0, dRaw2, Gb, opix, (double)opix, st, sums_2, &a2,
+                          nullptr, 1, nullptr, 0, ring != nullptr, 1, 0, true));
+        if (g_given) a2.g_in_reduce = 1;
+        TRYI(bn_bwd_begin(n, B.bd, ps.bn[B.bd.bidx], Gb, ps.blk[i].rawd, nullptr, 0, dRawD, nullptr, opix, (double)opix, st, sums_d, &ad, nullptr, 0,
                           nullptr, 0, ring != nullptr, 1, 0, true));
         const bool pair = bn_bwd_pair_ok(a2, ad);
+        if (g_given && !pair) { a2.g_in_reduce = 0; a2.gout = nullptr; }
         static const bool g_free = [] { const char* e = getenv("SSLCR_BN_PAIR_G"); return e && atoi(e) == 0; }();
-        const int keep_g = (n->tap || !a2.yact_bits || !g_free) ? 1 : 0;
+        const int keep_g = g_given ? 0 : ((n->tap || !a2.yact_bits || !g_free) ? 1 : 0);
+        const int from_g = g_given ? 1 : keep_g;
         if (pair) {
           TRY(launch_bn_bwd_reduce_pair(dt, a2, ad, keep_g, st));
         } else {
@@ -1256,21 +1267,22 @@
             r.e0 = c->prof.get(); r.e1 = c->prof.get();
             r.name = dt == DT_BF16 ? "sslcr::bn_bwd_apply_pair_kernel<unsigned short>" : "sslcr::bn_bwd_apply_pair_kernel<float>";
             r.flops = 0.0;
-            r.bytes = (keep_g ? 5.0 : 5.0625) * (double)opix * B.b2.C * c->esz();
+            r.bytes = (from_g ? 5.0 : 5.0625) * (double)opix * B.b2.C * c->esz();
             (void)hipEventRecord(r.e0, st);
-            hipError_t e = launch_bn_bwd_apply_pair(dt, a2, ad, keep_g, st);
+            hipError_t e = launch_bn_bwd_apply_pair(dt, a2, ad, from_g, st);
             (void)hipEventRecord(r.e1, st);
             c->prof.rec[2].push_back(r);
             TRY(e);
           } else {
-            TRY(launch_bn_bwd_apply_pair(dt, a2, ad, keep_g, st));
+            TRY(launch_bn_bwd_apply_pair(dt, a2, ad, from_g, st));
           }
         } else {
           TRYI(bn_bwd_end(c, a2, st));
           TRYI(bn_bwd_end(c, ad, st));
         }
       } else {
-        TRYI(bn_backward(n, B.b2, ps.bn[B.b2.bidx], dOut, ps.blk[i].raw2, ps.blk[i].y, 0, dRaw2, G, opix, (double)opix, st, nullptr, 1));
+        if (g_given) TRYI(bn_backward(n, B.b2, ps.bn[B.b2.bidx], dOut, ps.blk[i].raw2, nullptr, 0, dRaw2, nullptr, opix, (double)opix, st));
+        else TRYI(bn_backward(n, B.b2, ps.bn[B.b2.bidx], dOut, ps.blk[i].raw2, ps.blk[i].y, 0, dRaw2, G, opix, (double)opix, st, nullptr, 1));
       }
       if (p == 0) {
         TRYI(tap(i, 0, G, N, oh, ow, B.c2.cout));
@@ -1339,11 +1351,17 @@
     if (need_dx) {
       {
         const int NB = N * npass;
-        char *G = buf(kG, 0, so), *dRaw1 = buf(kRaw1, 0, so), *dXin = buf(kXin, 0, si), *dRawD = buf(kRawD, 0, so);
+        char *G = g_given ? buf(kOut, 0, so) : buf(kG, 0, so), *dRaw1 = buf(kRaw1, 0, so), *dXin = buf(kXin, 0, si), *dRawD = buf(kRawD, 0, so);
+        bool next_given = false;
         ConvArgs a = conv_args(B.c1, dRaw1, B.c1.w_dg, dXin, NB, oh, ow);
         a.C = B.c1.cout; a.K = B.c1.cin; a.transposed = (B.c1.stride == 1) ? 0 : 1; a.PH = xh; a.PW = xw; a.OH = xh; a.OW = xw;
         if (!B.has_ds) a.residual = G;
         if (B.c1.stride == 1) {
+          if (a.residual && i > 0) {
+            a.out_bits = bits_for(i - 1);
+            if (a.out_bits && !conv_out_bits_ok(dt, a)) a.out_bits = nullptr;
+            next_given = a.out_bits != nullptr;
+          }
           TRY(prof_conv(c, dt,a, st));
         } else {
           ConvArgs q4 = a;
@@ -1372,6 +1390,7 @@
           TRY(prof_conv(c, dt,s, st));
         }
         TRYI(tap(i, 5, dXin, N, xh, xw, B.c1.cin));
+        g_given = next_given;
       }
       const int t = kOut; kOut = kXin; kXin = t;
     }
@@ -1493,8 +1512,23 @@
 
 extern "C" {
 
+static void warn_measurement_knobs() {
+  static const bool once = [] {
+    const char* r = getenv("SSLCR_BN_REPEAT");
+    const char* u = getenv("SSLCR_UNFOLD_EVAL");
+    const char* b = getenv("SSLCR_POOL_BANDS");
+    const bool ra = r && atoi(r) > 1, ua = u && atoi(u) == 0, ba = b && atoi(b) != 0;
+    if (ra || ua || ba)
+      fprintf(stderr, "sslcr: measurement knob active:%s%s%s%s%s%s -- not the default step\n", ra ? " SSLCR_BN_REPEAT=" : "", ra ? r : "",
+              ua ? " SSLCR_UNFOLD_EVAL=" : "", ua ? u : "", ba ? " SSLCR_POOL_BANDS=" : "", ba ? b : "");
+    return true;
+  }();
+  (void)once;
+}
+
 int sslcr_create(sslcr_ctx** out, int device, int dtype) {
   if (!out || (dtype != SSLCR_F32 && dtype != SSLCR_BF16 && dtype != SSLCR_FP8)) return fail("sslcr_create: invalid argument");
+  warn_measurement_knobs();
   TRY(hipSetDevice(device));
   sslcr_ctx* c = new sslcr_ctx();
   c->device = device; c->dtype = dtype == SSLCR_FP8 ? SSLCR_BF16 : dtype; c->fp8 = dtype == SSLCR_FP8;
diff --git a/ssl_cr_histo_amd/csrc/kernels.hpp b/ssl_cr_histo_amd/csrc/kernels.hpp
--- a/ssl_cr_histo_amd/csrc/kernels.hpp
+++ b/ssl_cr_histo_amd/csrc/kernels.hpp
@@ -37,6 +37,7 @@
 int conv_h16_rows(const ConvArgs& a);
 hipError_t launch_conv_h16(int dtype, const ConvArgs& a, hipStream_t st);
 const char* conv_h16_name(int dtype, const ConvArgs& a);
+bool conv_out_bits_ok(int dtype, const ConvArgs& a);
 bool conv_pp64_ok(int dtype, const ConvArgs& a);
 hipError_t launch_conv_pp64(const ConvArgs& a, hipStream_t st);
 const char* conv_pp64_name(const ConvArgs& a);
@@ -83,7 +84,7 @@
 hipError_t launch_bn_relu_maxpool(int dtype, const PoolFwdArgs& a, hipStream_t st);
 hipError_t launch_maxpool_relu_bwd(int dtype, const PoolBwdArgs& a, hipStream_t st);
 hipError_t launch_avgpool_fwd(int dtype, const void* x, float* y, int N, int HW, int C, hipStream_t st);
-hipError_t launch_avgpool_bwd(int dtype, const float* dy, void* dx, int N, int HW, int C, hipStream_t st);
+hipError_t launch_avgpool_bwd(int dtype, const float* dy, void* dx, int N, int HW, int C, hipStream_t st, const uint8_t* bits = nullptr);
 hipError_t launch_bn_bwd_reduce(int dtype, const BnBwdArgs& a, hipStream_t st);
 hipError_t launch_bn_bwd_apply(int dtype, const BnBwdArgs& a, hipStream_t st);
 bool bn_bwd_pair_ok(const BnBwdArgs& a, const BnBwdArgs& b);
diff --git a/ssl_cr_histo_amd/kernels.py b/ssl_cr_histo_amd/kernels.py
--- a/ssl_cr_histo_amd/kernels.py
+++ b/ssl_cr_histo_amd/kernels.py
@@ -32,8 +32,8 @@
 
 def conv2d(x, w, stride, pad, *, in_scale=None, in_shift=None, in_relu=False, bias=None, residual=None, relu=False,
            want_stats=False, out=None, transposed=False, out_hw=None, osh=1, accumulate=False, pixel_hw=None,
-           pix_mul=0, pix_off=(0, 0), tap_mask=0, mask=None, par4=False, seg_images=0, out_scale=None):
-    _chk(x, w, in_scale, in_shift, bias, residual, out, out_scale)
+           pix_mul=0, pix_off=(0, 0), tap_mask=0, mask=None, par4=False, seg_images=0, out_scale=None, out_bits=None):
+    _chk(x, w, in_scale, in_shift, bias, residual, out, out_scale, out_bits)
     dt = _dt(x)
     N, H, W, C = x.shape
     K, R, S, C2 = w.shape
@@ -49,6 +49,7 @@
                    int(accumulate), int(pix_mul), int(pix_off[0]), int(pix_off[1]), int(tap_mask))
     d.par4 = int(par4)
     d.out_scale = L.ptr(out_scale)
+    d.out_bits = L.ptr(out_bits)
     if seg_images:
         d.seg_images = int(seg_images)
         d.seg_stride = int(in_scale.stride(0)) if in_scale is not None and in_scale.dim() == 2 else 0
@@ -302,11 +303,14 @@
     return y
 
 
-def avgpool_bwd(dy, shape, dtype):
-    _chk(dy)
+def avgpool_bwd(dy, shape, dtype, bits=None):
+    _chk(dy, bits)
     N, H, W, Cn = shape
     dx = torch.empty(shape, dtype=tdtype(dtype), device=dy.device)
-    L.check(L.lib().sslcr_avgpool_bwd(dtype, L.ptr(dy), L.ptr(dx), N, H * W, Cn, L.stream_ptr()))
+    if bits is not None:
+        L.check(L.lib().sslcr_avgpool_bwd_masked(dtype, L.ptr(dy), L.ptr(dx), L.ptr(bits), N, H * W, Cn, L.stream_ptr()))
+    else:
+        L.check(L.lib().sslcr_avgpool_bwd(dtype, L.ptr(dy), L.ptr(dx), N, H * W, Cn, L.stream_ptr()))
     return dx
 
 
```

Measured after the change: 72900 (median of 6 runs). About the same (+0.5%).
